# aleju/face-generator

Measured on NVIDIA H100. Metric: 32x32 GAN train images/sec (1 D-iter + 1 G-iter per batch, batch 256/GPU), higher is better.
Workload: dtype f32

## Files before the change

### face_generator_b200/csrc/convl.cu

```cuda
#include "convl.h"

#include "k_conv_tc.h"
#include "k_misc.h"

int convl_dalloc(ConvLEnv& e, float** p, size_t elems) { return fg_dalloc(e.c, *e.allocs, p, elems); }

int ScalePairs::alloc(fg_ctx* c, std::vector<void*>& allocs, int pairs) {
  n = pairs;
  used = 0;
  return fg_dalloc(c, allocs, &base, 2 * (size_t)pairs);
}
int ScalePairs::take(float** pair) {
  if (used == n) {
    fg_set_error("a block of %d FP16 scale pairs is full", n);
    return FG_ERR_UNSUPPORTED;
  }
  *pair = base + 2 * used++;
  return FG_OK;
}
int ScalePairs::reset(fg_ctx* c) const {
  if (!tc_f16(c)) return FG_OK;
  FG_CUDA(cudaMemset2DAsync(base, 2 * sizeof(float), 0, sizeof(float), n, c->stream));
  return FG_OK;
}

namespace {
inline bool tc_f(const fg_ctx* c, const ConvL& L, int B) { return c->conv_impl != FG_CONV_SIMT && tc_conv_eligible(L.geom_k(B)); }
inline bool tc_d(const fg_ctx* c, const ConvL& L, int B) { return c->conv_impl != FG_CONV_SIMT && tc_conv_eligible(L.geom_d(B)); }
inline bool tc_w(const fg_ctx* c, const ConvL& L, int B) { return tc_f(c, L, B) && L.Cout % 128 == 0 && L.geom_k(B).Cin % 64 == 0; }
}

bool convl_tc_fwd(const fg_ctx* c, const ConvL& L) { return tc_f(c, L, 1); }
bool convl_tc_bwd(const fg_ctx* c, const ConvL& L) { return tc_f(c, L, 1) && tc_d(c, L, 1); }

int tc_op_split(fg_ctx* c, TcOp& op, const float* x, int64_t n, bool f16) {
  if (!f16) {
    if (op.split_ready) {
      op.split_ready = false;
      return FG_OK;
    }
    return tc_split(c, x, op.hi, op.lo, n);
  }
  if (op.amax_ready) op.amax_ready = false;
  else FG_TRY(tc_amax(c, x, n, op.s));
  return tc_split_h(c, x, op.hi, op.lo, n, op.s);
}

int convl_alloc(ConvLEnv& e, ConvL& L) {
  const size_t nw = (size_t)L.k * L.k * L.Cout * L.Cin;
  FG_TRY(convl_dalloc(e, &L.Wp, nw));
  FG_TRY(convl_dalloc(e, &L.Wpd, nw));
  if (L.nA) FG_TRY(convl_dalloc(e, &L.bp, L.Cout));
  if (!L.x.s) FG_TRY(convl_dalloc(e, &L.x.s, 2));
  if (!e.dy.s) FG_TRY(convl_dalloc(e, &e.dy.s, 2));
  if (tc_conv_eligible(L.geom_k(e.maxB))) {
    const int K = L.geom_k(e.maxB).Cin;
    const size_t nk = (size_t)L.k * L.k * L.Cout * K, nx = (size_t)e.maxB * L.H * L.H * K;
    FG_TRY(convl_dalloc(e, &L.Wf_hi, nk));
    FG_TRY(convl_dalloc(e, &L.Wf_lo, nk));
    FG_TRY(convl_dalloc(e, &L.x.hi, nx));
    FG_TRY(convl_dalloc(e, &L.x.lo, nx));
    if (L.kpad) {
      FG_TRY(convl_dalloc(e, &L.Wpad, nk));
      FG_TRY(convl_dalloc(e, &L.xpad, nx));
    }
  }
  if (L.need_dgrad && tc_conv_eligible(L.geom_d(e.maxB))) {
    FG_TRY(convl_dalloc(e, &L.Wd_hi, nw));
    FG_TRY(convl_dalloc(e, &L.Wd_lo, nw));
  }
  const int B = e.maxB;
  if (L.pad_out && !(tc_conv_eligible(ConvGeom{B, L.H, L.H, L.Cin, L.pad_out, L.k, 1}) &&
                     tc_conv_eligible(ConvGeom{B, L.H, L.H, L.pad_out, L.Cin, L.k, 1}) && L.Cin % 128 == 0))
    L.pad_out = 0;
  if (L.pad_dy && !(L.x.hi && tc_conv_eligible(ConvGeom{B, L.H, L.H, L.Cin, L.pad_dy, L.k, 1}) && L.Cin % 64 == 0))
    L.pad_dy = 0;
  if (L.pad_out) {
    const size_t nq = (size_t)L.k * L.k * L.pad_out * L.Cin;
    FG_TRY(convl_dalloc(e, &L.Wq_hi, nq));
    FG_TRY(convl_dalloc(e, &L.Wq_lo, nq));
    const size_t nx = (size_t)B * L.H * L.H * L.Cin;
    FG_TRY(convl_dalloc(e, &L.x.hi, nx));
    FG_TRY(convl_dalloc(e, &L.x.lo, nx));
  }
  return FG_OK;
}

int convl_pack(fg_ctx* c, ConvL& L, const float* P) {
  const int KK = L.k * L.k;
  const bool tc_on = c->conv_impl != FG_CONV_SIMT;
  const bool h = tc_on && tc_f16(c) && L.geom_k(1).Cin % 64 == 0 && (L.Cout % 64 == 0 || L.pad_out);
  L.packed_f16 = h;
  if (KK > 1 && tc_on && !L.nA && !L.cA && !L.pad_out && !L.kpad && L.Wf_hi && (L.Wd_hi || !L.need_dgrad) && tc_f(c, L, 1) &&
      (!L.need_dgrad || tc_d(c, L, 1))) {
    if (h) return tc_pack_split_h(c, P + L.w_off, L.Wf_hi, L.Wf_lo, L.Wd_hi, L.Wd_lo, L.Cout, L.Cin, KK);
    return tc_pack_split(c, P + L.w_off, L.Wf_hi, L.Wf_lo, L.Wd_hi, L.Wd_lo, L.Cout, L.Cin, KK);
  }
  FG_TRY(k_pack_weights(c, P + L.w_off, L.Wp, L.need_dgrad ? L.Wpd : nullptr, L.Cout, L.Cin, KK, L.nA, L.nS, L.cA, L.cS));
  if (L.bp) FG_TRY(k_pack_weights(c, P + L.b_off, L.bp, nullptr, L.Cout, 1, 1, L.nA, L.nS, 0, 0));
  if (!tc_on) return FG_OK;
  if (L.kpad && L.Wf_hi) {
    FG_CUDA(cudaMemcpy2DAsync(L.Wpad, L.kpad * sizeof(float), L.Wp, L.Cin * sizeof(float), L.Cin * sizeof(float), L.Cout,
                              cudaMemcpyDeviceToDevice, c->stream));
    if (h) return tc_split_h(c, L.Wpad, L.Wf_hi, L.Wf_lo, (int64_t)L.Cout * L.kpad);
    return tc_split(c, L.Wpad, L.Wf_hi, L.Wf_lo, (int64_t)L.Cout * L.kpad);
  }
  const int64_t nw = (int64_t)KK * L.Cout * L.Cin;
  if (h) {
    if (L.Wf_hi) FG_TRY(tc_split_h(c, L.Wp, L.Wf_hi, L.Wf_lo, nw));
    if (L.Wd_hi) FG_TRY(tc_split_h(c, L.Wpd, L.Wd_hi, L.Wd_lo, nw));
    if (L.pad_out) FG_TRY(k_pack_pad_split_h(c, P + L.w_off, L.Wq_hi, L.Wq_lo, L.Cout, L.pad_out, L.Cin, KK));
    return FG_OK;
  }
  if (L.Wf_hi) FG_TRY(tc_split(c, L.Wp, L.Wf_hi, L.Wf_lo, nw));
  if (L.Wd_hi) FG_TRY(tc_split(c, L.Wpd, L.Wd_hi, L.Wd_lo, nw));
  if (L.pad_out) FG_TRY(k_pack_pad_split(c, P + L.w_off, L.Wq_hi, L.Wq_lo, L.Cout, L.pad_out, L.Cin, KK));
  return FG_OK;
}

int convl_fwd(ConvLEnv& e, ConvL& L, const float* in, const float* P, float* out, int B) {
  fg_ctx* c = e.c;
  const ConvGeom g = L.geom(B);
  const float* bias = L.bp ? L.bp : P + L.b_off;
  const bool h = L.packed_f16;
  const float* os = h ? L.x.s + 1 : nullptr;
  if (L.pad_out && c->conv_impl != FG_CONV_SIMT) {
    FG_TRY(tc_op_split(c, L.x, in, (int64_t)B * L.H * L.H * L.Cin, h));
    {
      ScopedTimer t(c, L.tf);
      FG_TRY(tc_conv_fwd(c, L.x.hi, L.x.lo, L.Wq_hi, L.Wq_lo, nullptr, e.ga, ConvGeom{B, L.H, L.H, L.Cin, L.pad_out, L.k, 1}, 0,
                         nullptr, nullptr, h, os));
    }
    return k_compact_bias(c, e.ga, bias, out, (int64_t)B * L.H * L.H, L.Cout, L.pad_out);
  }
  if (tc_f(c, L, B)) {
    const ConvGeom gk = L.geom_k(B);
    if (L.kpad) {
      FG_CUDA(cudaMemcpy2DAsync(L.xpad, L.kpad * sizeof(float), in, L.Cin * sizeof(float), L.Cin * sizeof(float), (size_t)B * L.H * L.H,
                                cudaMemcpyDeviceToDevice, c->stream));
      in = L.xpad;
    }
    FG_TRY(tc_op_split(c, L.x, in, (int64_t)B * L.H * L.H * gk.Cin, h));
    ScopedTimer t(c, L.tf);
    return tc_conv_fwd(c, L.x.hi, L.x.lo, L.Wf_hi, L.Wf_lo, bias, out, gk, 0, nullptr, nullptr, h, os);
  }
  ScopedTimer t(c, L.tf);
  if (c->edge_impl && k_edge_eligible(g)) return k_conv_edge(c, in, L.Wp, bias, out, g);
  return k_small_eligible(g) ? k_conv_small(c, in, L.Wp, bias, out, g) : k_conv_simt(c, in, L.Wp, bias, out, g);
}

int convl_bwd(ConvLEnv& e, ConvL& L, const float* in, const float* dy, float* G, float* din, int B) {
  fg_ctx* c = e.c;
  const ConvGeom g = L.geom(B), gd = L.geom_d(B);
  const bool w_tc = G && tc_w(c, L, B), d_tc = din && tc_d(c, L, B);
  const bool h = L.packed_f16;
  float* sdy = L.sdy ? L.sdy : e.dy.s;
  const bool split_ready = e.dy.split_ready, amax_ready = e.dy.amax_ready, bias_ready = e.dy.bias_ready;
  e.dy.split_ready = e.dy.amax_ready = e.dy.bias_ready = false;
  const float *osy = h ? sdy + 1 : nullptr, *osx = h ? L.x.s + 1 : nullptr;
  const bool tc_on = c->conv_impl != FG_CONV_SIMT;
  const int64_t P = (int64_t)B * L.H * L.H;
  if (h && !amax_ready && (w_tc || d_tc || (G && tc_on && (L.pad_out || L.pad_dy)))) FG_TRY(tc_amax(c, dy, P * L.Cout, sdy));
  if (w_tc || d_tc) {
    if (h) FG_TRY(tc_split_h(c, dy, e.dy.hi, e.dy.lo, P * L.Cout, sdy));
    else if (!split_ready) FG_TRY(tc_split(c, dy, e.dy.hi, e.dy.lo, P * L.Cout));
  }
  if (G && tc_on && L.pad_out) {
    if (h) FG_TRY(k_pad_split_h(c, dy, e.pad.hi, e.pad.lo, P, L.Cout, L.pad_out, sdy));
    else FG_TRY(k_pad_split(c, dy, e.pad.hi, e.pad.lo, P, L.Cout, L.pad_out));
    {
      ScopedTimer t(c, L.tw);
      FG_TRY(tc_conv_wgrad(c, e.pad.hi, e.pad.lo, L.x.hi, L.x.lo, e.ws, ConvGeom{B, L.H, L.H, L.pad_out, L.Cin, L.k, 1}, h, osy, osx));
    }
    FG_TRY(k_unpack_wgrad_swapped(c, e.ws, G + L.w_off, L.Cout, L.pad_out, L.Cin, L.k * L.k));
    if (!bias_ready) FG_TRY(k_colsum_add(c, dy, G + L.b_off, P, L.Cout, 0, 0));
  } else if (G && tc_on && L.pad_dy && !w_tc) {
    if (h) FG_TRY(k_pad_split_h(c, dy, e.pad.hi, e.pad.lo, P, L.Cout, L.pad_dy, sdy));
    else FG_TRY(k_pad_split(c, dy, e.pad.hi, e.pad.lo, P, L.Cout, L.pad_dy));
    {
      ScopedTimer t(c, L.tw);
      FG_TRY(tc_conv_wgrad(c, L.x.hi, L.x.lo, e.pad.hi, e.pad.lo, e.ws, ConvGeom{B, L.H, L.H, L.Cin, L.pad_dy, L.k, 1}, h, osy, osx));
    }
    FG_TRY(k_unpack_wgrad_pad(c, e.ws, G + L.w_off, L.Cout, L.pad_dy, L.Cin, L.k * L.k));
    if (!bias_ready) FG_TRY(k_colsum_add(c, dy, G + L.b_off, P, L.Cout, 0, 0));
  } else if (G) {
    const int64_t koff = L.kpad && w_tc ? (int64_t)L.Cout * L.Cin : 0;
    {
      ScopedTimer t(c, L.tw);
      if (w_tc) FG_TRY(tc_conv_wgrad(c, L.x.hi, L.x.lo, e.dy.hi, e.dy.lo, e.ws + koff, L.geom_k(B), h, osy, osx));
      else if (k_small_eligible(g)) FG_TRY(k_wgrad_small(c, in, dy, e.ws, g));
      else FG_TRY(k_wgrad_simt(c, in, dy, e.ws, g));
    }
    if (koff)
      FG_CUDA(cudaMemcpy2DAsync(e.ws, L.Cin * sizeof(float), e.ws + koff, L.kpad * sizeof(float), L.Cin * sizeof(float), L.Cout,
                                cudaMemcpyDeviceToDevice, c->stream));
    FG_TRY(k_unpack_wgrad(c, e.ws, G + L.w_off, L.Cout, L.Cin, L.k * L.k, L.nA, L.nS, L.cA, L.cS));
    if (!bias_ready) FG_TRY(k_colsum_add(c, dy, G + L.b_off, P, L.Cout, L.nA, L.nS));
  }
  if (din) {
    ScopedTimer t(c, L.td);
    if (d_tc) return tc_conv_fwd(c, e.dy.hi, e.dy.lo, L.Wd_hi, L.Wd_lo, nullptr, din, gd, 0, nullptr, nullptr, h, osy);
    if (c->edge_impl && k_edge_eligible(gd)) return k_conv_edge(c, dy, L.Wpd, nullptr, din, gd);
    return k_small_eligible(gd) ? k_conv_small(c, dy, L.Wpd, nullptr, din, gd) : k_conv_simt(c, dy, L.Wpd, nullptr, din, gd);
  }
  return FG_OK;
}

bool upsl_tc(const fg_ctx* c, const UpsL& U) {
  return c->conv_impl != FG_CONV_SIMT && tc_conv_eligible(U.geom(1)) && U.Cout % 128 == 0 && U.Cin % 64 == 0;
}

int upsl_alloc(ConvLEnv& e, UpsL& U) {
  const size_t nw25 = (size_t)25 * U.Cout * U.Cin, nw36 = (size_t)36 * U.Cout * U.Cin;
  FG_TRY(convl_dalloc(e, &U.Wp, nw25));
  FG_TRY(convl_dalloc(e, &U.Wpd, nw25));
  FG_TRY(convl_dalloc(e, &U.Wf_hi, nw36));
  FG_TRY(convl_dalloc(e, &U.Wf_lo, nw36));
  FG_TRY(convl_dalloc(e, &U.Wd_hi, nw36));
  FG_TRY(convl_dalloc(e, &U.Wd_lo, nw36));
  FG_TRY(convl_dalloc(e, &U.Wx_hi, nw25));
  FG_TRY(convl_dalloc(e, &U.Wx_lo, nw25));
  const size_t nx = (size_t)e.maxB * (U.H / 2) * (U.H / 2) * U.Cin;
  FG_TRY(convl_dalloc(e, &U.x.hi, nx));
  FG_TRY(convl_dalloc(e, &U.x.lo, nx));
  if (!U.x.s) FG_TRY(convl_dalloc(e, &U.x.s, 2));
  return FG_OK;
}

int upsl_pack(fg_ctx* c, UpsL& U, const float* P) {
  const float* W = P + U.w_off;
  if (!upsl_tc(c, U)) return k_pack_weights(c, W, U.Wp, U.Wpd, U.Cout, U.Cin, 25, 0, 0, 0, 0);
  if (tc_f16(c)) FG_TRY(tc_pack_collapsed_h(c, W, U.Wf_hi, U.Wf_lo, U.Wd_hi, U.Wd_lo, U.Cout, U.Cin));
  else FG_TRY(tc_pack_collapsed(c, W, U.Wf_hi, U.Wf_lo, U.Wd_hi, U.Wd_lo, U.Cout, U.Cin));
  if (c->conv_impl == FG_CONV_TC_DENSE) FG_TRY(tc_pack_split(c, W, U.Wx_hi, U.Wx_lo, nullptr, nullptr, U.Cout, U.Cin, 25));
  return FG_OK;
}

int upsl_fwd(ConvLEnv& e, UpsL& U, const float* h, const float* P, float* z, int B, int* parts) {
  fg_ctx* c = e.c;
  const ConvGeom g = U.geom(B);
  const bool want = parts && *parts;
  if (parts) *parts = 0;
  const float* bias = P + U.b_off;
  if (!upsl_tc(c, U)) {
    ScopedTimer t(c, U.tf);
    return k_conv_simt(c, h, U.Wp, bias, z, g);
  }
  const bool f16 = tc_f16(c);
  FG_TRY(tc_op_split(c, U.x, h, (int64_t)B * (U.H / 2) * (U.H / 2) * U.Cin, f16));
  ScopedTimer t(c, U.tf);
  float* st = want && c->bn_epilogue ? c->bn_parts : nullptr;
  const bool dense = c->conv_impl == FG_CONV_TC_DENSE;
  return tc_conv_fwd(c, U.x.hi, U.x.lo, dense ? U.Wx_hi : U.Wf_hi, dense ? U.Wx_lo : U.Wf_lo, bias, z, g, dense ? 1 : 2, st,
                     st ? parts : nullptr, f16, f16 ? U.x.s + 1 : nullptr);
}

int upsl_bwd(ConvLEnv& e, UpsL& U, TcOp& dy, const float* h, const float* dz, float* G, float* dh, int B, bool* pooled) {
  fg_ctx* c = e.c;
  const ConvGeom g = U.geom(B);
  float* dW = G + U.w_off;
  *pooled = upsl_tc(c, U);
  if (!*pooled) {
    {
      ScopedTimer t(c, U.tw);
      FG_TRY(k_wgrad_simt(c, h, dz, e.ws, g));
    }
    FG_TRY(k_unpack_wgrad(c, e.ws, dW, U.Cout, U.Cin, 25, 0, 0, 0, 0));
    ScopedTimer t(c, U.td);
    return k_conv_simt(c, dz, U.Wpd, nullptr, dh, ConvGeom{B, U.H, U.H, U.Cout, U.Cin, 5, 1});
  }
  const bool f16 = tc_f16(c);
  FG_TRY(tc_op_split(c, dy, dz, (int64_t)B * U.H * U.H * U.Cout, f16));
  const float *sy = f16 ? dy.s + 1 : nullptr, *sx = f16 ? U.x.s + 1 : nullptr;
  if (f16 && U.tb && (c->bwd_merge == 2 ? tc_bwd_pair_eligible(c, g) : c->bwd_merge == 1 && tc_bwd_pair_pays(c, g))) {
    {
      ScopedTimer t(c, U.tb);
      FG_TRY(tc_conv_bwd_ups(c, U.x.hi, U.x.lo, dy.hi, dy.lo, U.Wd_hi, U.Wd_lo, e.ws, dh, g, sy, sx));
    }
    return tc_combine_collapsed_wgrad(c, e.ws, dW, U.Cout, U.Cin);
  }
  {
    ScopedTimer t(c, U.tw);
    FG_TRY(tc_conv_wgrad(c, U.x.hi, U.x.lo, dy.hi, dy.lo, e.ws, g, f16, sy, sx));
  }
  FG_TRY(tc_combine_collapsed_wgrad(c, e.ws, dW, U.Cout, U.Cin));
  ScopedTimer t(c, U.td);
  return tc_conv_dgrad_ups(c, dy.hi, dy.lo, U.Wd_hi, U.Wd_lo, dh, g, f16, sy);
}
```

### face_generator_b200/csrc/convl.h

```cpp
#pragma once
#include <vector>

#include "fg_internal.h"

inline bool tc_f16(const fg_ctx* c) { return c->mma_f16 && c->conv_impl == FG_CONV_TC_COLLAPSED; }

struct AmaxInto {
  fg_ctx* c;
  AmaxInto(fg_ctx* c_, TcOp& op) : AmaxInto(c_, op.s, &op.amax_ready) {}
  AmaxInto(fg_ctx* c_, float* pair, bool* done) : c(c_) {
    if (tc_f16(c)) {
      c->amax_out = reinterpret_cast<unsigned*>(pair);
      c->amax_done = done;
    }
  }
  ~AmaxInto() { c->amax_out = nullptr; }
};

inline unsigned* take_amax(fg_ctx* c) {
  unsigned* p = c->amax_out;
  if (p) *c->amax_done = true;
  return p;
}

int tc_op_split(fg_ctx* c, TcOp& op, const float* x, int64_t n, bool f16);

inline int pack_key(const fg_ctx* c) { return c->conv_impl | (c->mma_f16 << 4); }
int convl_dalloc(ConvLEnv& e, float** p, size_t elems);
int convl_alloc(ConvLEnv& e, ConvL& L);
bool convl_tc_fwd(const fg_ctx* c, const ConvL& L);
bool convl_tc_bwd(const fg_ctx* c, const ConvL& L);
int convl_pack(fg_ctx* c, ConvL& L, const float* P);
int convl_fwd(ConvLEnv& e, ConvL& L, const float* in, const float* P, float* out, int B);
int convl_bwd(ConvLEnv& e, ConvL& L, const float* in, const float* dy, float* G, float* din, int B);

bool upsl_tc(const fg_ctx* c, const UpsL& U);
int upsl_alloc(ConvLEnv& e, UpsL& U);
int upsl_pack(fg_ctx* c, UpsL& U, const float* P);
int upsl_fwd(ConvLEnv& e, UpsL& U, const float* h, const float* P, float* z, int B, int* parts = nullptr);
int upsl_bwd(ConvLEnv& e, UpsL& U, TcOp& dy, const float* h, const float* dz, float* G, float* dh, int B, bool* pooled);

int gen_alloc(ConvLEnv& e, UpsGen& G, const GenDesc& d);
int gen_pack(fg_ctx* c, UpsGen& G, NetPair& p);
int gen_forward(ConvLEnv& e, UpsGen& G, NetPair& p, const float* noise, int B, bool training);
int gen_backward(ConvLEnv& e, UpsGen& G, NetPair& p, const float* dy, float* dnoise);
void gen_debug_rows(const UpsGen& G, std::vector<DebugTensor>& rows);
```

### face_generator_b200/csrc/fg_internal.h

```cpp
#pragma once
#include <cuda_runtime.h>
#include <cstdint>
#include <cstdio>
#include <deque>
#include <functional>
#include <initializer_list>
#include <map>
#include <string>
#include <vector>

#include "fg_b200.h"

void fg_set_error(const char* fmt, ...);

#define FG_CUDA(call)                                                                               \
  do {                                                                                              \
    cudaError_t e__ = (call);                                                                       \
    if (e__ != cudaSuccess) {                                                                       \
      fg_set_error("%s:%d: %s -> %s", __FILE__, __LINE__, #call, cudaGetErrorString(e__));          \
      return FG_ERR_CUDA;                                                                           \
    }                                                                                               \
  } while (0)
#define FG_TRY(call)                  \
  do {                                \
    int r__ = (call);                 \
    if (r__ != FG_OK) return r__;     \
  } while (0)
#define FG_REQUIRE(cond, ...)         \
  do {                                \
    if (!(cond)) {                    \
      fg_set_error(__VA_ARGS__);      \
      return FG_ERR_INVALID;          \
    }                                 \
  } while (0)
#define LAUNCH_CHECK(c)                 \
  do {                                  \
    (c)->launches++;                    \
    FG_CUDA(cudaGetLastError());        \
  } while (0)
inline int grid_for(int64_t n, int block, int cap = 132 * 16) {
  int64_t g = (n + block - 1) / block;
  if (g > cap) g = cap;
  if (g < 1) g = 1;
  return (int)g;
}
#define GRID_STRIDE(i, n) \
  for (int64_t i = blockIdx.x * (int64_t)blockDim.x + threadIdx.x; i < (n); i += (int64_t)gridDim.x * blockDim.x)

constexpr int kMaskPerSample = 1984;
constexpr int kNoiseDim = 100;
constexpr int kSmallMaxParts = 2048;
constexpr int kGradTail = 8;
constexpr int kOptRedRows = 132 * 2;

struct ConvGeom {
  int B, H, W, Cin, Cout, k, ups;
};

struct GLayout {
  int64_t L1W, L1b, a1, C1W, C1b, g1, be1, a2, C2W, C2b, g2, be2, a3, C3W, C3b, total;
};
GLayout make_g_layout(int C, int side);

struct DeviceStats {
  float loss_D, loss_G;
  int conf[4];
  int trained_D;
  int t_D, t_G;
  float acc_D;
  int acc_count, acc_head;
  float step_D, step_G;
  int do_train_D, do_train_G;
};
constexpr int kAccHistMax = 1024;
constexpr int kMaxIters = 16;
constexpr int kBnState = 768;

struct StepGraph {
  std::vector<uint8_t> key;
  cudaGraphExec_t exec = nullptr;
  int64_t launches = 0;
  bool failed = false;
};

struct NetPair {
  int64_t nG = 0, nD = 0;
  float *PG = nullptr, *PD = nullptr, *gG = nullptr, *gD = nullptr;
  float *tailG = nullptr, *tailD = nullptr;
  float *mG = nullptr, *vG = nullptr, *mD = nullptr, *vD = nullptr;
  float* bnG = nullptr;
  DeviceStats* dstats = nullptr;
  DeviceStats* hstats = nullptr;
  float* acc_hist = nullptr;
  int G_pack = -1, D_pack = -1;
  std::vector<StepGraph> graphs;
  const char* optim_timer[2] = {nullptr, nullptr};
  struct Keep {
    const char* name;
    const float* src;
    int64_t per;
    float* copy = nullptr;
  };
  std::vector<Keep> keep;
  int keep_B = 0;
};

struct ScalePairs {
  float* base = nullptr;
  int n = 0, used = 0;
  int alloc(fg_ctx* c, std::vector<void*>& allocs, int pairs);
  int take(float** pair);
  int reset(fg_ctx* c) const;
};

struct TcOp {
  float *hi = nullptr, *lo = nullptr;
  float* s = nullptr;
  bool split_ready = false, amax_ready = false, bias_ready = false;
};
struct ConvL {
  int Cin = 0, Cout = 0, k = 1, H = 1;
  int64_t w_off = 0, b_off = 0;
  int cA = 0, cS = 0;
  int nA = 0, nS = 0;
  float *Wp = nullptr, *Wpd = nullptr;
  float* bp = nullptr;
  float *Wf_hi = nullptr, *Wf_lo = nullptr, *Wd_hi = nullptr, *Wd_lo = nullptr;
  TcOp x;
  float* sdy = nullptr;
  int kpad = 0;
  float *xpad = nullptr, *Wpad = nullptr;
  bool packed_f16 = false;
  int pad_out = 0, pad_dy = 0;
  float *Wq_hi = nullptr, *Wq_lo = nullptr;
  bool need_dgrad = true;
  const char *tf = "", *td = "", *tw = "";
  ConvGeom geom(int B) const { return ConvGeom{B, H, H, Cin, Cout, k, 1}; }
  ConvGeom geom_k(int B) const { return ConvGeom{B, H, H, kpad ? kpad : Cin, Cout, k, 1}; }
  ConvGeom geom_d(int B) const { return ConvGeom{B, H, H, Cout, Cin, k, 1}; }
};

struct UpsL {
  int Cin = 0, Cout = 0, H = 0;
  int64_t w_off = 0, b_off = 0;
  float *Wp = nullptr, *Wpd = nullptr;
  float *Wf_hi = nullptr, *Wf_lo = nullptr, *Wd_hi = nullptr, *Wd_lo = nullptr;
  float *Wx_hi = nullptr, *Wx_lo = nullptr;
  TcOp x;
  const char *tf = "", *td = "", *tw = "", *tb = nullptr;
  ConvGeom geom(int B) const { return ConvGeom{B, H, H, Cin, Cout, 5, 2}; }
};

struct ConvLEnv {
  fg_ctx* c = nullptr;
  int maxB = 0;
  std::vector<void*>* allocs = nullptr;
  float *ga = nullptr;
  TcOp dy;
  TcOp pad;
  float* ws = nullptr;
};

struct GenDesc {
  int side;
  const char* prefix;
  int l1_kpad;
  bool bwd_merge;
};

struct UpsGen {
  int S = 32, C = 3;
  GLayout gl;
  ConvL GL1, GC3;
  UpsL GU[2];
  ScalePairs pairs;
  float* sdz[2] = {nullptr, nullptr};
  float *noise = nullptr, *z0 = nullptr, *h0 = nullptr, *z1 = nullptr, *h1 = nullptr, *z2 = nullptr, *h2 = nullptr,
        *z3 = nullptr, *y = nullptr;
  float *dz3 = nullptr, *dfull = nullptr, *dz2 = nullptr, *dz1 = nullptr, *dz0 = nullptr;
  float *bn_mean[2] = {nullptr, nullptr}, *bn_istd[2] = {nullptr, nullptr}, *bn_mg = nullptr;
  int B = 0;
  bool train = true, valid = false;
  std::deque<std::string> names;
  const char *t_bn2_finalize = nullptr, *t_bn2_stats = nullptr, *t_bn2_apply = nullptr, *t_bn2_bwd_reduce = nullptr,
             *t_bn2_bwd_apply = nullptr;
};

struct TimerRec {
  double ms = 0;
  int64_t launches = 0;
  std::vector<std::pair<cudaEvent_t, cudaEvent_t>> pending;
};

struct IterStage {
  float* p[8] = {};
  size_t cap[8] = {};
  int reserve(fg_ctx* c, std::vector<void*>& allocs, int k, size_t n);
  int in(fg_ctx* c, std::vector<void*>& allocs, int k, const float* p, size_t n, size_t cap_n, const float** out);
};

struct Net32;

struct fg_ctx {
  int device = 0, maxB = 0, C = 3;
  cudaStream_t stream = nullptr;
  bool own_stream = true;
  int64_t launches = 0;
  int conv_impl = FG_CONV_TC_COLLAPSED;
  int sm_count = 132;
  int opt_D = 0, opt_G = 0;
  float sgd_mom_D = 0.f, sgd_mom_G = 0.f;
  std::vector<void*> allocs;
  Net32* n32 = nullptr;
  float* small_ws = nullptr;
  float* splitk_ws = nullptr;
  size_t splitk_ws_elems = 0;
  double* red_ws = nullptr;
  size_t red_ws_elems = 0;
  double* red_ws_opt = nullptr;
  unsigned* red_ticket = nullptr;
  double* bn_slice_acc = nullptr;
  float* bn_parts = nullptr;
  int edge_impl = 1;
  int bn_epilogue = 1;
  int mma_f16 = 1;
  float* lop_sx = nullptr;
  float* lop_sy = nullptr;
  unsigned* amax_out = nullptr;
  bool* amax_done = nullptr;
  double* bn_acc = nullptr;
  float* io_dev = nullptr;
  size_t io_dev_elems = 0;
  float* scratch[8] = {nullptr, nullptr, nullptr, nullptr, nullptr, nullptr, nullptr, nullptr};
  size_t scratch_elems[8] = {0, 0, 0, 0, 0, 0, 0, 0};
  void* nccl_comm = nullptr;
  int world = 1, rank = 0;
  int dp_overlap = 1;
  int reserve_sms = 0;
  int last_conv_kind = 0, last_conv_tile_m = 0, last_conv_tile_n = 0, last_conv_format = 0, last_conv_splits = 0;
  int bwd_merge = 1, bwd_merge_ctas = 0;
  int* bwd_claim = nullptr;
  int use_graph = 1, graph_epoch = 0;
  uint64_t* seed_dev = nullptr;
  cudaStream_t comm_stream = nullptr;
  cudaEvent_t ev_fork = nullptr, ev_join = nullptr;
  bool debug_keep = false;
  cudaEvent_t events[16] = {};
  bool timing = false;
  std::map<std::string, TimerRec> timers;
};

inline void note_conv(fg_ctx* c, int kind, int tile_m, int tile_n, int format, int splits) {
  c->last_conv_kind = kind;
  c->last_conv_tile_m = tile_m;
  c->last_conv_tile_n = tile_n;
  c->last_conv_format = format;
  c->last_conv_splits = splits;
}

struct ScopedTimer {
  fg_ctx* c;
  TimerRec* rec = nullptr;
  cudaEvent_t e0 = nullptr, e1 = nullptr;
  ScopedTimer(fg_ctx* c_, const char* name) : c(c_) {
    if (c->timing && name) {
      rec = &c->timers[name];
      cudaEventCreate(&e0);
      cudaEventCreate(&e1);
      cudaEventRecord(e0, c->stream);
    }
  }
  ~ScopedTimer() {
    if (rec) {
      cudaEventRecord(e1, c->stream);
      rec->pending.emplace_back(e0, e1);
    }
  }
};

int k_fill(fg_ctx* c, float* p, float v, int64_t n);
int k_nchw_to_nhwc(fg_ctx* c, const float* src, float* dst, int B, int C, int HW);
int k_nhwc_to_nchw(fg_ctx* c, const float* src, float* dst, int B, int C, int HW);
int k_pack_weights(fg_ctx* c, const float* W, float* Wp, float* Wpd, int N, int Cc, int KK, int nA, int nS, int cA,
                   int cS);
int k_unpack_wgrad(fg_ctx* c, const float* dWp, float* dW, int N, int Cc, int KK, int nA, int nS, int cA, int cS);
int k_colsum_add(fg_ctx* c, const float* X, float* out, int64_t P, int N, int nA, int nS);
int k_prelu_fwd(fg_ctx* c, const float* z, const float* slope, float* h, int64_t n);
int k_prelu_bwd(fg_ctx* c, const float* dh, const float* z, const float* slope, float* dz, float* dslope, int B, int H,
                int W, int C, int pool);
int k_bn_stats(fg_ctx* c, const float* z, double* acc2C, int64_t P, int C);
bool k_bn4_ok(int C);
int k_bn_stats4(fg_ctx* c, const float* z, double* acc, int64_t P, int C);
int k_bn_bwd_reduce4(fg_ctx* c, const float* dh, const float* z, const float* mean, const float* istd, const float* gamma,
                     const float* beta, const float* slope, double* acc, float* dslope, int64_t P, int C);
int k_bn_finalize(fg_ctx* c, double* acc2C, float* mean, float* istd, float* run_mean, float* run_var, int64_t P,
                  int C);
int k_bn_finalize_parts(fg_ctx* c, const float* part, int nparts, int nphase, float* mean, float* istd, float* run_mean,
                        float* run_var, int64_t P, int C);
int k_bn_eval_prep(fg_ctx* c, const float* run_mean, const float* run_var, float* mean, float* istd, int C);
int k_bn_prelu_apply(fg_ctx* c, const float* z, const float* mean, const float* istd, const float* gamma,
                     const float* beta, const float* slope, float* h, int64_t P, int C, float* hi = nullptr,
                     float* lo = nullptr);
int k_bn_prelu_bwd_reduce(fg_ctx* c, const float* dh, const float* z, const float* mean, const float* istd,
                          const float* gamma, const float* beta, const float* slope, double* acc2C, float* dslope,
                          int B, int H, int W, int C, int pool);
int k_bn_bwd_finalize(fg_ctx* c, double* acc2C, float* mg2C, float* dgamma, float* dbeta, int64_t P, int C);
int k_bn_prelu_bwd_apply(fg_ctx* c, const float* dh, const float* z, const float* mean, const float* istd,
                         const float* gamma, const float* beta, const float* slope, const float* mg2C, float* dz,
                         int B, int H, int W, int C, int pool, float* hi = nullptr, float* lo = nullptr,
                         float* dbias = nullptr);
int k_sigmoid_fwd(fg_ctx* c, const float* z, float* y, int64_t n);
int k_sigmoid_bwd(fg_ctx* c, const float* dy, const float* y, float* dz, int64_t n);
int k_masks_generate(fg_ctx* c, float* masks, int B, uint64_t seed, float p_spatial, float p_drop,
                     const uint64_t* seed_dev = nullptr);
int k_set_u64(fg_ctx* c, uint64_t* dst, uint64_t v);
int k_seed_roots(fg_ctx* c, uint64_t* roots, int n);
int k_d_act_pool_fwd(fg_ctx* c, const float* z, const float* slope, const float* masks, int moff, float eval_scale,
                     float* p, int B, int H, int W, int C, float* hi = nullptr, float* lo = nullptr);
int k_d_act_pool_bwd(fg_ctx* c, const float* dp, const float* z, const float* slope, const float* masks, int moff,
                     float eval_scale, float* dz, float* dslope, int B, int H, int W, int C, float* hi = nullptr,
                     float* lo = nullptr, float* dbias = nullptr);
int k_lin_act_drop_fwd(fg_ctx* c, const float* z, const float* slope, const float* masks, int moff, float scale,
                       float* h, int B, int N);
int k_lin_act_drop_bwd(fg_ctx* c, const float* dh, const float* z, const float* slope, const float* masks, int moff,
                       float scale, float* dz, float* dslope, int B, int N);
int k_sigmoid_bce(fg_ctx* c, const float* logit, float* out, float* dlogit, float* loss_out, float* tail4, int B,
                  int n_ones);
int k_bce_fwd(fg_ctx* c, const float* x, const float* t, int n, float* loss_out);
int k_bce_bwd(fg_ctx* c, const float* x, const float* t, int n, float* dx);
int k_sigmoid_grad_mul(fg_ctx* c, const float* dout, const float* out, float* dlogit, int n);
int k_penalty_loss(fg_ctx* c, const float* p, int64_t n, float l1, float l2, float* loss_inout);
int k_gate_and_prep(fg_ctx* c, DeviceStats* st, float* acc_hist, int net, const fg_hyper* h, const float* tail4, int B,
                    float world, bool accumulate = false);
int k_optim_prep(fg_ctx* c, DeviceStats* st, int net, const fg_hyper* h);
int k_gemv_fwd(fg_ctx* c, const float* x, const float* w, const float* bias, float* out, int B, int K);
int k_gemv_dgrad(fg_ctx* c, const float* dy, const float* w, float* dx, int B, int K);
int k_gemv_wgrad_add(fg_ctx* c, const float* x, const float* dy, float* dw, float* db, int B, int K);
int k_adam(fg_ctx* c, float* p, const float* g, float* m, float* v, int64_t n, float beta1, float beta2, float eps,
           float l1_grad, float l2, float clampv, float grad_scale, const float* step_dev, const int* flag_dev,
           float step_host, float* g_out);
int k_optim_update(fg_ctx* c, int mode, float* p, float* g, float* m, float* v, int64_t n, float beta1, float beta2, float eps,
                   float mom, float l1_grad, float l2, float clampv, float grad_scale, const float* step_dev,
                   const int* flag_dev, const int* t_dev);

int k_conv_simt(fg_ctx* c, const float* in, const float* Wp, const float* bias, float* out, ConvGeom g);
int k_wgrad_simt(fg_ctx* c, const float* in, const float* dY, float* dWp, ConvGeom g);
bool k_small_eligible(const ConvGeom& g);
int k_conv_small(fg_ctx* c, const float* in, const float* Wp, const float* bias, float* out, ConvGeom g);
int k_wgrad_small(fg_ctx* c, const float* in, const float* dY, float* dWp, ConvGeom g);

bool k_edge_eligible(const ConvGeom& g);
int k_conv_edge(fg_ctx* c, const float* in, const float* Wp, const float* bias, float* out, ConvGeom g);

inline int red_check(fg_ctx* c, int64_t rows, int64_t n) {
  if (rows * n > (int64_t)c->red_ws_elems) {
    fg_set_error("ordered reduction of %lld x %lld partials exceeds its workspace", (long long)rows, (long long)n);
    return FG_ERR_UNSUPPORTED;
  }
  return FG_OK;
}
int k_splitk_reduce(fg_ctx* c, const float* parts, int splits, int64_t n, float* out);

int tc_init(fg_ctx* c);
void tc_destroy(fg_ctx* c);

int net32_alloc(fg_ctx* c);
void net32_free(fg_ctx* c);
NetPair& net32_pair(fg_ctx* c);

int net_allreduce(fg_ctx* c, float* buf, int64_t n);
int net_broadcast(fg_ctx* c, void* buf, size_t bytes);
int net_group(bool start);

int fg_dalloc(fg_ctx* c, std::vector<void*>& allocs, float** p, size_t n);
int pair_alloc(fg_ctx* c, std::vector<void*>& allocs, NetPair& p, int64_t nG, int64_t nD, bool bn);
void pair_clear_graphs(NetPair& p);
void pair_free(NetPair& p);
int pair_zero_grads(fg_ctx* c, NetPair& p, int net);
int pair_allreduce_grads(fg_ctx* c, NetPair& p, int net);
int pair_gate(fg_ctx* c, NetPair& p, int net, const fg_hyper* h, int B, float world, bool accumulate = false);
int pair_optim(fg_ctx* c, NetPair& p, int net, const fg_hyper* h, float grad_scale);
int k_adam_prep(fg_ctx* c, int* t_dev, float* step_dev, float lr, float beta1, float beta2);
int pair_broadcast(fg_ctx* c, NetPair& p);
int pair_step_stats(fg_ctx* c, const NetPair& p, fg_step_stats* stats);
int pair_set_params(fg_ctx* c, NetPair& p, int net, const float* src);
int pair_get_params(fg_ctx* c, const NetPair& p, int net, float* dst);
int pair_get_grads(fg_ctx* c, const NetPair& p, int net, float* dst);
int pair_set_adam_state(fg_ctx* c, NetPair& p, int net, const float* m, const float* v, int t);
int pair_get_adam_state(fg_ctx* c, const NetPair& p, int net, float* m, float* v, int* t);
int pair_set_bn_state(fg_ctx* c, NetPair& p, const float* src);
int pair_get_bn_state(fg_ctx* c, const NetPair& p, float* dst);
int net_graph_run(fg_ctx* c, NetPair& p, int B, const void* hyper, size_t hyper_bytes, std::initializer_list<const void*> inputs,
                  uint64_t seed, const std::function<int()>& body, int nd = 1, int ng = 1);

int step_check(fg_ctx* c, const char* what, int B, int nd, int ng, bool inputs, const fg_dataset* d = nullptr, bool fed = false);
struct StepNets {
  StepNets(fg_ctx* c, NetPair& pair, const fg_hyper* h, int B, float* logit, float* out, float* dlogit, float* masks,
           int64_t mask, bool gate, bool overlap)
      : c(c), pair(&pair), h(h), B(B), logit(logit), out(out), dlogit(dlogit), masks(masks), mask(mask), gate(gate),
        overlap(overlap) {}
  fg_ctx* c;
  NetPair* pair;
  const fg_hyper* h;
  int B;
  float *logit, *out, *dlogit;
  float* masks;
  int64_t mask;
  bool gate;
  bool overlap;
  virtual int g_forward(int j, bool d_iter) = 0;
  virtual int d_input(int j) = 0;
  virtual int draw_masks(int kind, const uint64_t* root) = 0;
  virtual int d_forward(bool on_g) = 0;
  virtual int d_backward(bool want_wgrad, bool want_dx) = 0;
  virtual int g_backward() = 0;
};
int pair_train_step(StepNets& s, int nd, int ng, const float* masksD, const float* masksG, uint64_t seed,
                    std::initializer_list<const void*> inputs, const std::function<int()>* feed, fg_step_stats* stats);
struct DebugTensor;
void pair_keep_rows(const NetPair& p, std::vector<DebugTensor>& ents);

int k_relu_fwd(fg_ctx* c, const float* z, float* h, int64_t n);
int k_relu_bwd(fg_ctx* c, const float* dh, const float* z, float* dz, int64_t n);
int k_tanh_dropout_fwd(fg_ctx* c, const float* z, const float* masks_in, const uint64_t* seed_dev, float p, float* code, float* h,
                       float* flags_out, int64_t n);
int k_tanh_dropout_bwd(fg_ctx* c, const float* dh, const float* masks, float p, const float* code, float* dz, int64_t n);
int k_abs_criterion(fg_ctx* c, bool sigmoid, const float* z, const float* t, float* y, float* dz, int64_t n, float* loss);

bool fg_is_dev(const void* p);
int fg_to_dev(fg_ctx* c, const float* p, size_t n, float* staging, const float** out);
int fg_to_user(fg_ctx* c, float* dst, const float* src_dev, size_t n);
struct DebugTensor {
  const char* name;
  const float* p;
  int64_t per;
  int B;
};
int64_t debug_tensor_copy(fg_ctx* c, const char* what, const DebugTensor* ents, size_t n_ents, const char* name, float* dst,
                          int64_t max_elems);

struct JpegScratch;
void jpeg_scratch_free(JpegScratch* s);
struct JpegEncScratch;
void jpeg_enc_scratch_free(JpegEncScratch* s);
struct fg_dataset {
  fg_ctx* c = nullptr;
  int64_t N = 0;
  int Cs = 3, Hs = 64, Ws = 64;
  uint8_t* data = nullptr;
  int32_t* idx = nullptr;
  JpegScratch* jpeg = nullptr;
  JpegEncScratch* jpeg_enc = nullptr;
};
int dataset_check_feed(const fg_dataset* d, const fg_ctx* c, const char* what);
int dataset_draw_gather(fg_dataset* d, uint64_t seed, int B, int size, float* out_dev, const uint64_t* root = nullptr,
                        uint64_t kinds = 0);
int dataset_draw_gather_c2f(fg_dataset* d, uint64_t seed, int B, int fine_size, int coarse_size, float* fine, float* coarse,
                            float* diff, const uint64_t* root = nullptr, uint64_t kinds = 0);
int noise_uniform_dev(fg_ctx* c, uint64_t seed, int64_t n, float* out_dev, const uint64_t* root = nullptr, uint64_t kinds = 0);
```

### face_generator_b200/csrc/gen.cu

```cuda
#include "convl.h"

GLayout make_g_layout(int C, int side) {
  const int64_t n0 = 128 * (side / 4) * (side / 4);
  GLayout L;
  int64_t o = 0;
  L.L1W = o; o += n0 * kNoiseDim;
  L.L1b = o; o += n0;
  L.a1 = o; o += 1;
  L.C1W = o; o += 256 * 128 * 25;
  L.C1b = o; o += 256;
  L.g1 = o; o += 256;
  L.be1 = o; o += 256;
  L.a2 = o; o += 1;
  L.C2W = o; o += 128 * 256 * 25;
  L.C2b = o; o += 128;
  L.g2 = o; o += 128;
  L.be2 = o; o += 128;
  L.a3 = o; o += 1;
  L.C3W = o; o += (int64_t)C * 128 * 9;
  L.C3b = o; o += C;
  L.total = o;
  return L;
}

int gen_alloc(ConvLEnv& e, UpsGen& G, const GenDesc& d) {
  fg_ctx* c = e.c;
  const int S = d.side, C = c->C;
  G.S = S;
  G.C = C;
  G.gl = make_g_layout(C, S);
  const GLayout& gl = G.gl;
  auto timer = [&](const char* name) {
    G.names.push_back(std::string(d.prefix) + name);
    return G.names.back().c_str();
  };
  FG_TRY(G.pairs.alloc(c, *e.allocs, 8));
  ConvL& L1 = G.GL1;
  L1.Cin = kNoiseDim; L1.Cout = 128 * (S / 4) * (S / 4); L1.k = 1; L1.H = 1;
  L1.w_off = gl.L1W; L1.b_off = gl.L1b;
  L1.nA = 128; L1.nS = (S / 4) * (S / 4);
  L1.kpad = d.l1_kpad;
  L1.tf = timer("G.L1.fwd"); L1.td = timer("G.L1.dgrad"); L1.tw = timer("G.L1.wgrad");
  ConvL& C3 = G.GC3;
  C3.Cin = 128; C3.Cout = C; C3.k = 3; C3.H = S;
  C3.w_off = gl.C3W; C3.b_off = gl.C3b;
  C3.tf = timer("G.C3.fwd"); C3.td = timer("G.C3.dgrad"); C3.tw = timer("G.C3.wgrad");
  for (ConvL* L : {&L1, &C3}) {
    FG_TRY(G.pairs.take(&L->x.s));
    FG_TRY(G.pairs.take(&L->sdy));
    FG_TRY(convl_alloc(e, *L));
  }
  static const char* uf[2] = {"G.C1.fwd", "G.C2.fwd"};
  static const char* ud[2] = {"G.C1.dgrad", "G.C2.dgrad"};
  static const char* uw[2] = {"G.C1.wgrad", "G.C2.wgrad"};
  static const char* ub[2] = {"G.C1.wgrad+dgrad", "G.C2.wgrad+dgrad"};
  const int ci[2] = {128, 256}, co[2] = {256, 128}, hs[2] = {S / 2, S};
  const int64_t wo[2] = {gl.C1W, gl.C2W}, bo[2] = {gl.C1b, gl.C2b};
  for (int i = 0; i < 2; ++i) {
    UpsL& U = G.GU[i];
    U.Cin = ci[i]; U.Cout = co[i]; U.H = hs[i];
    U.w_off = wo[i]; U.b_off = bo[i];
    U.tf = timer(uf[i]); U.td = timer(ud[i]); U.tw = timer(uw[i]);
    U.tb = d.bwd_merge ? timer(ub[i]) : nullptr;
    FG_TRY(G.pairs.take(&U.x.s));
    FG_TRY(G.pairs.take(&G.sdz[i]));
    FG_TRY(upsl_alloc(e, U));
  }
  G.t_bn2_finalize = timer("G.bn2.finalize");
  G.t_bn2_stats = timer("hbm.G.bn2.stats");
  G.t_bn2_apply = timer("hbm.G.bn2.apply");
  G.t_bn2_bwd_reduce = timer("hbm.G.bn2.bwd_reduce");
  G.t_bn2_bwd_apply = timer("hbm.G.bn2.bwd_apply");
  const size_t B = e.maxB, n0 = L1.Cout, n1 = (size_t)256 * (S / 2) * (S / 2), n2 = (size_t)128 * S * S, n3 = (size_t)C * S * S;
  for (auto [p, n] : {std::pair<float**, size_t>{&G.noise, kNoiseDim}, {&G.z0, n0}, {&G.h0, n0}, {&G.z1, n1}, {&G.h1, n1},
                      {&G.z2, n2}, {&G.h2, n2}, {&G.z3, n3}, {&G.y, n3}, {&G.dz3, n3},
                      {&G.dfull, (size_t)256 * S * S},
                      {&G.dz2, n2}, {&G.dz1, n1}, {&G.dz0, n0}})
    FG_TRY(convl_dalloc(e, p, B * n));
  for (int i = 0; i < 2; ++i) {
    FG_TRY(convl_dalloc(e, &G.bn_mean[i], co[i]));
    FG_TRY(convl_dalloc(e, &G.bn_istd[i], co[i]));
  }
  return convl_dalloc(e, &G.bn_mg, 512);
}

int gen_pack(fg_ctx* c, UpsGen& G, NetPair& p) {
  if (p.G_pack == pack_key(c)) return FG_OK;
  FG_TRY(convl_pack(c, G.GL1, p.PG));
  for (int i = 0; i < 2; ++i) FG_TRY(upsl_pack(c, G.GU[i], p.PG));
  FG_TRY(convl_pack(c, G.GC3, p.PG));
  p.G_pack = pack_key(c);
  return FG_OK;
}

namespace {
int bn_stats(fg_ctx* c, UpsGen& G, NetPair& p, int i, const float* z, int B, bool training, int parts, const char* t_finalize,
             const char* t_stats) {
  const int Cc = G.GU[i].Cout;
  const int64_t P = (int64_t)B * G.GU[i].H * G.GU[i].H;
  float *rm = p.bnG + (i == 0 ? 0 : 512), *rv = rm + Cc;
  if (!training) return k_bn_eval_prep(c, rm, rv, G.bn_mean[i], G.bn_istd[i], Cc);
  if (parts) {
    ScopedTimer tm(c, t_finalize);
    return k_bn_finalize_parts(c, c->bn_parts, parts, 4, G.bn_mean[i], G.bn_istd[i], rm, rv, P, Cc);
  }
  {
    ScopedTimer tm(c, t_stats);
    FG_TRY(k_bn_stats(c, z, c->bn_acc, P, Cc));
  }
  return k_bn_finalize(c, c->bn_acc, G.bn_mean[i], G.bn_istd[i], rm, rv, P, Cc);
}
}

int gen_forward(ConvLEnv& e, UpsGen& G, NetPair& p, const float* noise, int B, bool training) {
  fg_ctx* c = e.c;
  FG_REQUIRE(B >= 1 && B <= e.maxB, "G forward: batch %d out of range [1,%d]", B, e.maxB);
  FG_TRY(gen_pack(c, G, p));
  const GLayout& L = G.gl;
  const float* P = p.PG;
  const int S = G.S;
  if (noise != G.noise)
    FG_CUDA(cudaMemcpyAsync(G.noise, noise, sizeof(float) * B * kNoiseDim, cudaMemcpyDeviceToDevice, c->stream));
  G.B = B;
  G.train = training;
  FG_TRY(G.pairs.reset(c));
  FG_TRY(convl_fwd(e, G.GL1, G.noise, P, G.z0, B));
  {
    AmaxInto am(c, G.GU[0].x);
    FG_TRY(k_prelu_fwd(c, G.z0, P + L.a1, G.h0, (int64_t)B * G.GL1.Cout));
  }
  int parts = training ? 1 : 0;
  FG_TRY(upsl_fwd(e, G.GU[0], G.h0, P, G.z1, B, &parts));
  FG_TRY(bn_stats(c, G, p, 0, G.z1, B, training, parts, nullptr, nullptr));
  UpsL& C2 = G.GU[1];
  C2.x.split_ready = training && upsl_tc(c, C2) && !tc_f16(c);
  {
    AmaxInto am(c, C2.x);
    FG_TRY(k_bn_prelu_apply(c, G.z1, G.bn_mean[0], G.bn_istd[0], P + L.g1, P + L.be1, P + L.a2, G.h1,
                            (int64_t)B * (S / 2) * (S / 2), 256, C2.x.split_ready ? C2.x.hi : nullptr,
                            C2.x.split_ready ? C2.x.lo : nullptr));
  }
  parts = training ? 1 : 0;
  FG_TRY(upsl_fwd(e, C2, G.h1, P, G.z2, B, &parts));
  FG_TRY(bn_stats(c, G, p, 1, G.z2, B, training, parts, G.t_bn2_finalize, G.t_bn2_stats));
  {
    ScopedTimer tm(c, G.t_bn2_apply);
    FG_TRY(k_bn_prelu_apply(c, G.z2, G.bn_mean[1], G.bn_istd[1], P + L.g2, P + L.be2, P + L.a3, G.h2, (int64_t)B * S * S, 128));
  }
  FG_TRY(convl_fwd(e, G.GC3, G.h2, P, G.z3, B));
  FG_TRY(k_sigmoid_fwd(c, G.z3, G.y, (int64_t)B * S * S * G.C));
  G.valid = true;
  return FG_OK;
}

int gen_backward(ConvLEnv& e, UpsGen& G, NetPair& p, const float* dy, float* dnoise) {
  fg_ctx* c = e.c;
  if (!G.valid || !G.train) {
    fg_set_error("G backward needs a preceding training-mode G forward");
    return FG_ERR_STATE;
  }
  const GLayout& L = G.gl;
  const float* P = p.PG;
  float* g = p.gG;
  const int B = G.B, S = G.S, h = S / 2;
  FG_TRY(G.pairs.reset(c));
  FG_TRY(k_sigmoid_bwd(c, dy, G.y, G.dz3, (int64_t)B * S * S * G.C));
  FG_TRY(convl_bwd(e, G.GC3, G.h2, G.dz3, g, G.dfull, B));
  {
    ScopedTimer tm(c, G.t_bn2_bwd_reduce);
    FG_TRY(k_bn_prelu_bwd_reduce(c, G.dfull, G.z2, G.bn_mean[1], G.bn_istd[1], P + L.g2, P + L.be2, P + L.a3, c->bn_acc,
                                 g + L.a3, B, S, S, 128, 0));
  }
  FG_TRY(k_bn_bwd_finalize(c, c->bn_acc, G.bn_mg, g + L.g2, g + L.be2, (int64_t)B * S * S, 128));
  const bool tf32 = !tc_f16(c);
  TcOp dz2{e.dy.hi, e.dy.lo, G.sdz[1]};
  dz2.split_ready = upsl_tc(c, G.GU[1]) && tf32;
  {
    ScopedTimer tm(c, G.t_bn2_bwd_apply);
    AmaxInto am(c, dz2);
    FG_TRY(k_bn_prelu_bwd_apply(c, G.dfull, G.z2, G.bn_mean[1], G.bn_istd[1], P + L.g2, P + L.be2, P + L.a3, G.bn_mg, G.dz2,
                                B, S, S, 128, 0, dz2.split_ready ? dz2.hi : nullptr, dz2.split_ready ? dz2.lo : nullptr,
                                g + L.C2b));
  }
  bool pooled = false;
  FG_TRY(upsl_bwd(e, G.GU[1], dz2, G.h1, G.dz2, g, G.dfull, B, &pooled));
  FG_TRY(k_bn_prelu_bwd_reduce(c, G.dfull, G.z1, G.bn_mean[0], G.bn_istd[0], P + L.g1, P + L.be1, P + L.a2, c->bn_acc,
                               g + L.a2, B, h, h, 256, pooled ? 0 : 1));
  FG_TRY(k_bn_bwd_finalize(c, c->bn_acc, G.bn_mg, g + L.g1, g + L.be1, (int64_t)B * h * h, 256));
  TcOp dz1{e.dy.hi, e.dy.lo, G.sdz[0]};
  dz1.split_ready = upsl_tc(c, G.GU[0]) && tf32 && pooled;
  {
    AmaxInto am(c, dz1);
    FG_TRY(k_bn_prelu_bwd_apply(c, G.dfull, G.z1, G.bn_mean[0], G.bn_istd[0], P + L.g1, P + L.be1, P + L.a2, G.bn_mg, G.dz1,
                                B, h, h, 256, pooled ? 0 : 1, dz1.split_ready ? dz1.hi : nullptr,
                                dz1.split_ready ? dz1.lo : nullptr, g + L.C1b));
  }
  FG_TRY(upsl_bwd(e, G.GU[0], dz1, G.h0, G.dz1, g, G.dfull, B, &pooled));
  {
    AmaxInto am(c, G.GL1.sdy, &e.dy.amax_ready);
    FG_TRY(k_prelu_bwd(c, G.dfull, G.z0, P + L.a1, G.dz0, g + L.a1, B, S / 4, S / 4, 128, pooled ? 0 : 1));
  }
  return convl_bwd(e, G.GL1, G.noise, G.dz0, g, dnoise, B);
}

void gen_debug_rows(const UpsGen& G, std::vector<DebugTensor>& rows) {
  const int64_t n0 = G.GL1.Cout, n1 = 256 * (G.S / 2) * (G.S / 2), n2 = 128 * G.S * G.S, n3 = (int64_t)G.C * G.S * G.S;
  const int B = G.B;
  for (const DebugTensor& r : {DebugTensor{"G.z0", G.z0, n0, B}, {"G.h0", G.h0, n0, B}, {"G.z1", G.z1, n1, B},
                               {"G.h1", G.h1, n1, B}, {"G.z2", G.z2, n2, B}, {"G.h2", G.h2, n2, B}, {"G.z3", G.z3, n3, B},
                               {"G.y", G.y, n3, B}, {"G.dz2", G.dz2, n2, B}, {"G.dz1", G.dz1, n1, B}, {"G.dz0", G.dz0, n0, B},
                               {"G.bn_mean1", G.bn_mean[0], 256, 1}, {"G.bn_istd1", G.bn_istd[0], 256, 1},
                               {"G.bn_mean2", G.bn_mean[1], 128, 1}, {"G.bn_istd2", G.bn_istd[1], 128, 1}})
    rows.push_back({r.name, G.valid ? r.p : nullptr, r.per, r.B});
}
```

### face_generator_b200/csrc/k_conv_edge.cu

```cuda
#include <cuda.h>

#include <algorithm>

#include "fg_internal.h"
#include "k_conv_tc.h"

namespace {
constexpr int kW = 32;

__device__ __forceinline__ uint32_t smem_u32(const void* p) { return (uint32_t)__cvta_generic_to_shared(p); }
__device__ __forceinline__ void mbar_init(uint64_t* bar, uint32_t count) {
  asm volatile("mbarrier.init.shared::cta.b64 [%0], %1;" ::"r"(smem_u32(bar)), "r"(count));
}
__device__ __forceinline__ void mbar_expect_tx(uint64_t* bar, uint32_t bytes) {
  asm volatile("mbarrier.arrive.expect_tx.shared::cta.b64 _, [%0], %1;" ::"r"(smem_u32(bar)), "r"(bytes) : "memory");
}
__device__ __forceinline__ void mbar_wait(uint64_t* bar, uint32_t parity) {
  const uint32_t addr = smem_u32(bar);
  uint32_t ok;
  do {
    asm volatile(
        "{\n\t.reg .pred p;\n\t"
        "mbarrier.try_wait.parity.shared::cta.b64 p, [%1], %2;\n\t"
        "selp.b32 %0, 1, 0, p;\n\t}"
        : "=r"(ok)
        : "r"(addr), "r"(parity)
        : "memory");
  } while (!ok);
}
__device__ __forceinline__ float4 lds128(uint32_t addr) {
  float4 v;
  asm volatile("ld.shared.v4.f32 {%0, %1, %2, %3}, [%4];" : "=f"(v.x), "=f"(v.y), "=f"(v.z), "=f"(v.w) : "r"(addr));
  return v;
}
__device__ __forceinline__ float2 lds64(uint32_t addr) {
  float2 v;
  asm volatile("ld.shared.v2.f32 {%0, %1}, [%2];" : "=f"(v.x), "=f"(v.y) : "r"(addr));
  return v;
}
__device__ __forceinline__ void tma_load_4d(void* dst, const CUtensorMap* map, uint64_t* bar, int c0, int c1, int c2, int c3) {
  asm volatile(
      "cp.async.bulk.tensor.4d.shared::cluster.global.mbarrier::complete_tx::bytes [%0], [%1, {%3, %4, %5, %6}], [%2];"
      ::"r"(smem_u32(dst)), "l"(map), "r"(smem_u32(bar)), "r"(c0), "r"(c1), "r"(c2), "r"(c3)
      : "memory");
}

constexpr int kRedRows = 4;
template <int VEC>
constexpr uint32_t red_tile_bytes() { return (kRedRows + 2) * (kW + 2) * 32 * VEC * 4; }

template <int NS, int VEC>
__global__ void __launch_bounds__(256, 1) conv_reduce_kernel(const __grid_constant__ CUtensorMap tmap, const float* __restrict__ Wp,
                                                             const float* __restrict__ bias, float* __restrict__ out, int H,
                                                             int nunits) {
  constexpr int C = 32 * VEC;
  constexpr int PX = NS == 1 ? 16 : 4;
  constexpr uint32_t kTile = red_tile_bytes<VEC>();
  extern __shared__ uint8_t smem_raw[];
  uint8_t* smem = reinterpret_cast<uint8_t*>((reinterpret_cast<uintptr_t>(smem_raw) + 127) & ~(uintptr_t)127);
  uint64_t* full = reinterpret_cast<uint64_t*>(smem + 2 * kTile);
  const int warp = threadIdx.x >> 5, lane = threadIdx.x & 31;
  const int strips = H / kRedRows;
  if (threadIdx.x == 0) {
    mbar_init(full + 0, 1);
    mbar_init(full + 1, 1);
    asm volatile("fence.mbarrier_init.release.cluster;" ::: "memory");
  }
  __syncthreads();
  auto issue = [&](int unit, int buf) {
    const int b = unit / strips, y0 = (unit - b * strips) * kRedRows;
    asm volatile("fence.proxy.async.shared::cta;" ::: "memory");
    mbar_expect_tx(full + buf, kTile);
    tma_load_4d(smem + buf * kTile, &tmap, full + buf, 0, -1, y0 - 1, b);
  };
  if (threadIdx.x == 0 && (int)blockIdx.x < nunits) issue(blockIdx.x, 0);
  float w[9][NS][VEC];
#pragma unroll
  for (int t = 0; t < 9; ++t)
#pragma unroll
    for (int n = 0; n < NS; ++n)
#pragma unroll
      for (int j = 0; j < VEC; ++j) w[t][n][j] = Wp[(t * NS + n) * C + lane * VEC + j];
  float bv = 0.f;
  if (bias && (lane & 15) < PX * NS) bv = bias[(lane & 15) % NS];
  const int row = warp >> 1, xh = (warp & 1) * 16;
  int it = 0;
  for (int unit = blockIdx.x; unit < nunits; unit += gridDim.x, ++it) {
    const int buf = it & 1;
    if (threadIdx.x == 0 && unit + (int)gridDim.x < nunits) issue(unit + gridDim.x, buf ^ 1);
    mbar_wait(full + buf, (it >> 1) & 1);
    const uint32_t tile = smem_u32(smem + buf * kTile) + (uint32_t)lane * VEC * 4;
    const int b = unit / strips, y = (unit - b * strips) * kRedRows + row;
#pragma unroll 1
    for (int g = 0; g < 16 / PX; ++g) {
      const int x0 = xh + g * PX;
      float acc[PX][NS];
#pragma unroll
      for (int i = 0; i < PX; ++i)
#pragma unroll
        for (int n = 0; n < NS; ++n) acc[i][n] = 0.f;
#pragma unroll
      for (int j = 0; j < PX + 2; ++j) {
        float v[3][VEC];
#pragma unroll
        for (int dy = 0; dy < 3; ++dy) {
          const uint32_t ad = tile + (uint32_t)(((row + dy) * (kW + 2) + x0 + j) * C) * 4;
          if (VEC == 4) {
            const float4 q = lds128(ad);
            v[dy][0] = q.x; v[dy][1 % VEC] = q.y; v[dy][2 % VEC] = q.z; v[dy][3 % VEC] = q.w;
          } else {
            const float2 q = lds64(ad);
            v[dy][0] = q.x; v[dy][1 % VEC] = q.y;
          }
        }
#pragma unroll
        for (int dy = 0; dy < 3; ++dy)
#pragma unroll
          for (int k = 0; k < VEC; ++k)
#pragma unroll
            for (int dx = 0; dx < 3; ++dx) {
              const int i = j - dx;
              if (i < 0 || i >= PX) continue;
#pragma unroll
              for (int n = 0; n < NS; ++n) acc[i][n] = fmaf(v[dy][k], w[dy * 3 + dx][n][k], acc[i][n]);
            }
      }
      float r[16];
#pragma unroll
      for (int k = 0; k < 16; ++k) r[k] = k < PX * NS ? acc[k / NS][k % NS] : 0.f;
#pragma unroll
      for (int sft = 8; sft >= 1; sft >>= 1) {
        const bool up = (lane & sft) != 0;
#pragma unroll
        for (int k = 0; k < sft; ++k) {
          const float send = up ? r[k] : r[k + sft], keep = up ? r[k + sft] : r[k];
          r[k] = keep + __shfl_xor_sync(0xffffffffu, send, sft);
        }
      }
      const float tot = r[0] + __shfl_xor_sync(0xffffffffu, r[0], 16);
      if (lane < PX * NS) out[((size_t)(b * H + y) * kW + x0) * NS + lane] = tot + bv;
    }
    __syncthreads();
  }
}

constexpr int kExpRows = 8;
template <int CS, int N>
__global__ void __launch_bounds__(256, 1) conv_expand_kernel(const float* __restrict__ in, const float* __restrict__ Wp,
                                                             const float* __restrict__ bias, float* __restrict__ out, int H,
                                                             int nunits) {
  constexpr int RW = (kW + 2) * 4;
  constexpr int ROWF = kW * CS;
  constexpr int NPF = ((kExpRows + 2) * ROWF + 255) / 256;
  __shared__ __align__(16) float tile[2][(kExpRows + 2) * RW];
  const int warp = threadIdx.x >> 5, lane = threadIdx.x & 31;
  const int strips = H / kExpRows;
  for (int i = threadIdx.x; i < 2 * (kExpRows + 2) * RW; i += 256) (&tile[0][0])[i] = 0.f;
  const int n4 = (N == 128 ? lane : (lane & 15)) * 4;
  float w[9][CS][4];
#pragma unroll
  for (int t = 0; t < 9; ++t)
#pragma unroll
    for (int c = 0; c < CS; ++c)
#pragma unroll
      for (int j = 0; j < 4; ++j) w[t][c][j] = Wp[((size_t)t * N + n4 + j) * CS + c];
  float4 b4 = make_float4(0.f, 0.f, 0.f, 0.f);
  if (bias) b4 = make_float4(bias[n4], bias[n4 + 1], bias[n4 + 2], bias[n4 + 3]);
  float pf[NPF];
  auto prefetch = [&](int unit) {
    const int b = unit / strips, y0 = (unit - b * strips) * kExpRows;
#pragma unroll
    for (int i = 0; i < NPF; ++i) {
      const int idx = threadIdx.x + 256 * i;
      const int r = idx / ROWF, off = idx - r * ROWF, gy = y0 - 1 + r;
      pf[i] = (r < kExpRows + 2 && gy >= 0 && gy < H) ? in[((size_t)(b * H + gy) * kW) * CS + off] : 0.f;
    }
  };
  auto stash = [&](int buf) {
#pragma unroll
    for (int i = 0; i < NPF; ++i) {
      const int idx = threadIdx.x + 256 * i;
      const int r = idx / ROWF, off = idx - r * ROWF;
      if (r < kExpRows + 2) tile[buf][r * RW + (off / CS + 1) * 4 + off % CS] = pf[i];
    }
  };
  __syncthreads();
  if ((int)blockIdx.x < nunits) {
    prefetch(blockIdx.x);
    stash(0);
  }
  __syncthreads();
  constexpr int STEP = N == 128 ? 2 : 4;
  const int xoff = N == 128 ? 0 : 2 * (lane >> 4);
  int it = 0;
  for (int unit = blockIdx.x; unit < nunits; unit += gridDim.x, ++it) {
    const int buf = it & 1;
    const bool more = unit + (int)gridDim.x < nunits;
    if (more) prefetch(unit + gridDim.x);
    const int b = unit / strips, y = (unit - b * strips) * kExpRows + warp;
    const float4* t0 = reinterpret_cast<const float4*>(&tile[buf][warp * RW]);
    float* orow = out + ((size_t)(b * H + y) * kW) * N + n4;
#pragma unroll 1
    for (int xb = 0; xb < kW; xb += STEP) {
      const int x = xb + xoff;
      float4 a0 = b4, a1 = b4;
#pragma unroll
      for (int dy = 0; dy < 3; ++dy) {
        float4 col[4];
#pragma unroll
        for (int j = 0; j < 4; ++j) col[j] = t0[dy * (kW + 2) + x + j];
#pragma unroll
        for (int dx = 0; dx < 3; ++dx)
#pragma unroll
          for (int c = 0; c < CS; ++c) {
            const float v0 = c == 0 ? col[dx].x : (c == 1 ? col[dx].y : (c == 2 ? col[dx].z : col[dx].w));
            const float v1 = c == 0 ? col[dx + 1].x : (c == 1 ? col[dx + 1].y : (c == 2 ? col[dx + 1].z : col[dx + 1].w));
            const float* wp = w[dy * 3 + dx][c];
            a0.x = fmaf(v0, wp[0], a0.x); a1.x = fmaf(v1, wp[0], a1.x);
            a0.y = fmaf(v0, wp[1], a0.y); a1.y = fmaf(v1, wp[1], a1.y);
            a0.z = fmaf(v0, wp[2], a0.z); a1.z = fmaf(v1, wp[2], a1.z);
            a0.w = fmaf(v0, wp[3], a0.w); a1.w = fmaf(v1, wp[3], a1.w);
          }
      }
      *reinterpret_cast<float4*>(orow + (size_t)x * N) = a0;
      *reinterpret_cast<float4*>(orow + (size_t)(x + 1) * N) = a1;
    }
    if (more) stash(buf ^ 1);
    __syncthreads();
  }
}

template <int NS, int VEC>
int launch_reduce(fg_ctx* c, const float* in, const float* Wp, const float* bias, float* out, const ConvGeom& g) {
  CUtensorMap tmap;
  FG_TRY(tc_encode_nhwc_box(&tmap, in, 32 * VEC, g.W, g.H, g.B, 32 * VEC, kW + 2, kRedRows + 2, 1));
  const int nunits = g.B * (g.H / kRedRows);
  const size_t smem = 2 * (size_t)red_tile_bytes<VEC>() + 64 + 128;
  static bool attr_done = false;
  if (!attr_done) {
    FG_CUDA(cudaFuncSetAttribute(conv_reduce_kernel<NS, VEC>, cudaFuncAttributeMaxDynamicSharedMemorySize, (int)smem));
    attr_done = true;
  }
  note_conv(c, FG_KERNEL_EDGE_REDUCE, NS, VEC, 0, 1);
  conv_reduce_kernel<NS, VEC><<<std::min(nunits, c->sm_count), 256, smem, c->stream>>>(tmap, Wp, bias, out, g.H, nunits);
  LAUNCH_CHECK(c);
  return FG_OK;
}
template <int CS, int N>
int launch_expand(fg_ctx* c, const float* in, const float* Wp, const float* bias, float* out, const ConvGeom& g) {
  const int nunits = g.B * (g.H / kExpRows);
  note_conv(c, FG_KERNEL_EDGE_EXPAND, CS, N, 0, 1);
  conv_expand_kernel<CS, N><<<std::min(nunits, c->sm_count), 256, 0, c->stream>>>(in, Wp, bias, out, g.H, nunits);
  LAUNCH_CHECK(c);
  return FG_OK;
}
}

bool k_edge_eligible(const ConvGeom& g) {
  if (!(g.ups == 1 && g.k == 3 && g.W == kW && g.H % 8 == 0 && g.H >= 8)) return false;
  const bool reduce = (g.Cout == 1 || g.Cout == 3) && (g.Cin == 64 || g.Cin == 128);
  const bool expand = (g.Cin == 1 || g.Cin == 3 || g.Cin == 4) && (g.Cout == 64 || g.Cout == 128);
  return reduce || expand;
}

int k_conv_edge(fg_ctx* c, const float* in, const float* Wp, const float* bias, float* out, ConvGeom g) {
  if (g.Cout <= 3) {
    if (g.Cout == 3 && g.Cin == 128) return launch_reduce<3, 4>(c, in, Wp, bias, out, g);
    if (g.Cout == 3 && g.Cin == 64) return launch_reduce<3, 2>(c, in, Wp, bias, out, g);
    if (g.Cout == 1 && g.Cin == 128) return launch_reduce<1, 4>(c, in, Wp, bias, out, g);
    if (g.Cout == 1 && g.Cin == 64) return launch_reduce<1, 2>(c, in, Wp, bias, out, g);
  } else {
#define EXP(CS_)                                                                 \
  if (g.Cin == CS_) {                                                            \
    if (g.Cout == 128) return launch_expand<CS_, 128>(c, in, Wp, bias, out, g); \
    if (g.Cout == 64) return launch_expand<CS_, 64>(c, in, Wp, bias, out, g);   \
  }
    EXP(1) EXP(3) EXP(4)
#undef EXP
  }
  fg_set_error("k_conv_edge: unsupported shape %d -> %d", g.Cin, g.Cout);
  return FG_ERR_UNSUPPORTED;
}
```

### face_generator_b200/csrc/k_conv_small.cu

```cuda
#include "fg_internal.h"

namespace {
constexpr int kMaxSmallW = 36 * 128;

template <int NS, int VEC>
__global__ void __launch_bounds__(256) conv_smalln_kernel(const float* __restrict__ in, const float* __restrict__ Wp,
                                                          const float* __restrict__ bias, float* __restrict__ out, int B,
                                                          int H, int W) {
  constexpr int C = 32 * VEC;
  __shared__ __align__(16) float ws[9 * NS * C];
  for (int i = threadIdx.x; i < 9 * NS * C; i += blockDim.x) ws[i] = Wp[i];
  __syncthreads();
  constexpr int RL = 8;
  const int lane = threadIdx.x & 31;
  const uint32_t runs_per_row = (uint32_t)W / RL;
  const uint32_t nruns = (uint32_t)B * H * runs_per_row;
  const uint32_t warps = (gridDim.x * blockDim.x) >> 5;
  for (uint32_t run = (blockIdx.x * blockDim.x + threadIdx.x) >> 5; run < nruns; run += warps) {
    const int x0 = (int)(run % runs_per_row) * RL;
    const uint32_t row = run / runs_per_row;
    const int y = (int)(row % (uint32_t)H);
    const float* rowbase = in + (size_t)row * W * C + lane * VEC;
    float col[3][3][VEC];
    auto load_col = [&](int slot, int xx) {
#pragma unroll
      for (int dy = 0; dy < 3; ++dy) {
        const bool ok = (unsigned)(y + dy - 1) < (unsigned)H && (unsigned)xx < (unsigned)W;
        const float* ip = rowbase + ((dy - 1) * W + xx) * C;
        if (VEC == 4) {
          const float4 q = ok ? *reinterpret_cast<const float4*>(ip) : make_float4(0.f, 0.f, 0.f, 0.f);
          col[slot][dy][0] = q.x; col[slot][dy][1 % VEC] = q.y; col[slot][dy][2 % VEC] = q.z; col[slot][dy][3 % VEC] = q.w;
        } else if (VEC == 2) {
          const float2 q = ok ? *reinterpret_cast<const float2*>(ip) : make_float2(0.f, 0.f);
          col[slot][dy][0] = q.x; col[slot][dy][1 % VEC] = q.y;
        } else {
          col[slot][dy][0] = ok ? ip[0] : 0.f;
        }
      }
    };
    load_col(0, x0 - 1);
    load_col(1, x0);
#pragma unroll
    for (int i = 0; i < RL; ++i) {
      load_col((i + 2) % 3, x0 + i + 1);
      float acc[NS];
#pragma unroll
      for (int n = 0; n < NS; ++n) acc[n] = 0.f;
#pragma unroll
      for (int dy = 0; dy < 3; ++dy)
#pragma unroll
        for (int dx = 0; dx < 3; ++dx) {
          const int t = dy * 3 + dx, slot = (i + dx) % 3;
#pragma unroll
          for (int n = 0; n < NS; ++n) {
            const float* wp = ws + (t * NS + n) * C + lane * VEC;
#pragma unroll
            for (int j = 0; j < VEC; ++j) acc[n] = fmaf(col[slot][dy][j], wp[j], acc[n]);
          }
        }
#pragma unroll
      for (int n = 0; n < NS; ++n) {
#pragma unroll
        for (int o = 16; o > 0; o >>= 1) acc[n] += __shfl_xor_sync(0xffffffffu, acc[n], o);
      }
      if (lane == 0) {
        float* op = out + ((size_t)row * W + x0 + i) * NS;
#pragma unroll
        for (int n = 0; n < NS; ++n) op[n] = acc[n] + (bias ? bias[n] : 0.f);
      }
    }
  }
}

template <int CS>
__global__ void __launch_bounds__(256) conv_smallk4_kernel(const float* __restrict__ in, const float* __restrict__ Wp,
                                                           const float* __restrict__ bias, float* __restrict__ out, int B,
                                                           int H, int W, int N) {
  __shared__ __align__(16) float ws[9 * CS * 128];
  for (int i = threadIdx.x; i < 9 * CS * N; i += blockDim.x) {
    const int n = i % N, c = (i / N) % CS, t = i / (N * CS);
    ws[i] = Wp[((size_t)t * N + n) * CS + c];
  }
  __syncthreads();
  const uint32_t N4 = (uint32_t)N >> 2;
  const uint32_t total = (uint32_t)B * H * W * N4;
  for (uint32_t i = blockIdx.x * blockDim.x + threadIdx.x; i < total; i += gridDim.x * blockDim.x) {
    const uint32_t n4 = i % N4, p = i / N4;
    const int x = (int)(p % (uint32_t)W), y = (int)((p / (uint32_t)W) % (uint32_t)H);
    float4 acc = bias ? make_float4(bias[n4 * 4], bias[n4 * 4 + 1], bias[n4 * 4 + 2], bias[n4 * 4 + 3])
                      : make_float4(0.f, 0.f, 0.f, 0.f);
    const float* base = in + (size_t)p * CS;
#pragma unroll
    for (int t = 0; t < 9; ++t) {
      const int dy = t / 3 - 1, dx = t % 3 - 1;
      if ((unsigned)(y + dy) >= (unsigned)H || (unsigned)(x + dx) >= (unsigned)W) continue;
      const float* ip = base + (dy * W + dx) * CS;
#pragma unroll
      for (int c = 0; c < CS; ++c) {
        const float v = __ldg(ip + c);
        const float4 w = *reinterpret_cast<const float4*>(ws + (t * CS + c) * N + n4 * 4);
        acc.x = fmaf(v, w.x, acc.x);
        acc.y = fmaf(v, w.y, acc.y);
        acc.z = fmaf(v, w.z, acc.z);
        acc.w = fmaf(v, w.w, acc.w);
      }
    }
    *reinterpret_cast<float4*>(out + (size_t)i * 4) = acc;
  }
}

template <int CS, int XS>
__global__ void __launch_bounds__(128) wgrad_smallbig_kernel(const float* __restrict__ big, const float* __restrict__ small,
                                                             float* __restrict__ part, int B, int H, int W, int Cb,
                                                             int rows_per_block) {
  __shared__ float4 sm[3][68];
  const int lanes = 128 / Cb;
  const int cb = threadIdx.x % Cb, pl = threadIdx.x / Cb;
  const int x_begin = pl * XS;
  float acc[9][CS];
#pragma unroll
  for (int t = 0; t < 9; ++t)
#pragma unroll
    for (int c = 0; c < CS; ++c) acc[t][c] = 0.f;
  const int BH = B * H;
  const int r0 = blockIdx.x * rows_per_block, r1 = min(BH, r0 + rows_per_block);
  for (int r = r0; r < r1; ++r) {
    const int b = r / H, y = r - b * H;
    __syncthreads();
    for (int i = threadIdx.x; i < 3 * (W + 2); i += 128) {
      const int rr = i / (W + 2), cc = i - rr * (W + 2);
      const int yy = y + rr - 1, xx = cc - 1;
      float4 v = make_float4(0.f, 0.f, 0.f, 0.f);
      if (yy >= 0 && yy < H && xx >= 0 && xx < W) {
        const float* sp = small + (((size_t)b * H + yy) * W + xx) * CS;
        v.x = sp[0];
        if (CS > 1) v.y = sp[1 % CS];
        if (CS > 2) v.z = sp[2 % CS];
        if (CS > 3) v.w = sp[3 % CS];
      }
      sm[rr][cc] = v;
    }
    __syncthreads();
    const float* bp = big + ((size_t)r * W + x_begin) * Cb + cb;
    float bv[XS];
#pragma unroll
    for (int i = 0; i < XS; ++i) bv[i] = bp[(size_t)i * Cb];
    float4 w0[3], w1[3], w2[3];
#pragma unroll
    for (int rr = 0; rr < 3; ++rr) {
      w0[rr] = sm[rr][x_begin];
      w1[rr] = sm[rr][x_begin + 1];
    }
#pragma unroll
    for (int i = 0; i < XS; ++i) {
#pragma unroll
      for (int rr = 0; rr < 3; ++rr) {
        w2[rr] = sm[rr][x_begin + i + 2];
        const float4 q[3] = {w0[rr], w1[rr], w2[rr]};
#pragma unroll
        for (int cc = 0; cc < 3; ++cc) {
          acc[rr * 3 + cc][0] = fmaf(bv[i], q[cc].x, acc[rr * 3 + cc][0]);
          if (CS > 1) acc[rr * 3 + cc][1 % CS] = fmaf(bv[i], q[cc].y, acc[rr * 3 + cc][1 % CS]);
          if (CS > 2) acc[rr * 3 + cc][2 % CS] = fmaf(bv[i], q[cc].z, acc[rr * 3 + cc][2 % CS]);
          if (CS > 3) acc[rr * 3 + cc][3 % CS] = fmaf(bv[i], q[cc].w, acc[rr * 3 + cc][3 % CS]);
        }
        w0[rr] = w1[rr];
        w1[rr] = w2[rr];
      }
    }
  }
  float* dst = part + ((size_t)blockIdx.x * lanes + pl) * (9 * CS * Cb);
#pragma unroll
  for (int t = 0; t < 9; ++t)
#pragma unroll
    for (int c = 0; c < CS; ++c) dst[(t * CS + c) * Cb + cb] = acc[t][c];
}
__global__ void wgrad_small_reduce_kernel(const float* __restrict__ part, float* __restrict__ out, int nparts, int CS, int Cb,
                                          int sign, int transposed) {
  const int total = 9 * CS * Cb;
  const int j = blockIdx.x * blockDim.x + threadIdx.x;
  if (j >= total) return;
  const int per = (nparts + gridDim.y - 1) / gridDim.y;
  const int i0 = blockIdx.y * per, i1 = min(nparts, i0 + per);
  float s0 = 0.f, s1 = 0.f, s2 = 0.f, s3 = 0.f;
  int i = i0;
  for (; i + 3 < i1; i += 4) {
    s0 += part[(size_t)i * total + j];
    s1 += part[(size_t)(i + 1) * total + j];
    s2 += part[(size_t)(i + 2) * total + j];
    s3 += part[(size_t)(i + 3) * total + j];
  }
  for (; i < i1; ++i) s0 += part[(size_t)i * total + j];
  const int idx = j / (CS * Cb), cs = (j / Cb) % CS, cb = j % Cb;
  const int t = sign > 0 ? idx : 8 - idx;
  out[(size_t)blockIdx.y * total + (transposed ? ((size_t)t * Cb + cb) * CS + cs : ((size_t)t * CS + cs) * Cb + cb)] =
      (s0 + s1) + (s2 + s3);
}
}

bool k_small_eligible(const ConvGeom& g) {
  const int cs = g.Cin < g.Cout ? g.Cin : g.Cout, cb = g.Cin < g.Cout ? g.Cout : g.Cin;
  if (!(g.ups == 1 && g.k == 3 && cs >= 1 && cs <= 4 && (cb == 32 || cb == 64 || cb == 128))) return false;
  const int xs = g.W / (128 / cb);
  return g.W <= 64 && g.W % (128 / cb) == 0 && (xs == 8 || xs == 16 || xs == 32) &&
         (int64_t)g.B * g.H * g.W * cb < ((int64_t)1 << 31);
}

int k_conv_small(fg_ctx* c, const float* in, const float* Wp, const float* bias, float* out, ConvGeom g) {
  const int64_t P = (int64_t)g.B * g.H * g.W;
  if (g.Cin <= 4) {
    const int64_t total = P * (g.Cout / 4);
    int grid = (int)std::min<int64_t>((total + 255) / 256, c->sm_count * 16);
    switch (g.Cin) {
      case 1: conv_smallk4_kernel<1><<<grid, 256, 0, c->stream>>>(in, Wp, bias, out, g.B, g.H, g.W, g.Cout); break;
      case 2: conv_smallk4_kernel<2><<<grid, 256, 0, c->stream>>>(in, Wp, bias, out, g.B, g.H, g.W, g.Cout); break;
      case 3: conv_smallk4_kernel<3><<<grid, 256, 0, c->stream>>>(in, Wp, bias, out, g.B, g.H, g.W, g.Cout); break;
      default: conv_smallk4_kernel<4><<<grid, 256, 0, c->stream>>>(in, Wp, bias, out, g.B, g.H, g.W, g.Cout); break;
    }
    LAUNCH_CHECK(c);
    return FG_OK;
  }
  if (g.Cout > 4 || 9 * g.Cout * g.Cin > kMaxSmallW) {
    fg_set_error("k_conv_small: expects Cout <= 4");
    return FG_ERR_UNSUPPORTED;
  }
  if (g.W % 8) {
    fg_set_error("k_conv_small: W must be a multiple of 8");
    return FG_ERR_UNSUPPORTED;
  }
  int grid = (int)std::min<int64_t>((P / 8 * 32 + 255) / 256, c->sm_count * 8);
#define SN(NS_, VEC_) conv_smalln_kernel<NS_, VEC_><<<grid, 256, 0, c->stream>>>(in, Wp, bias, out, g.B, g.H, g.W)
  const int vec = g.Cin / 32;
  if (vec == 4) {
    if (g.Cout == 1) SN(1, 4); else if (g.Cout == 2) SN(2, 4); else if (g.Cout == 3) SN(3, 4); else SN(4, 4);
  } else if (vec == 2) {
    if (g.Cout == 1) SN(1, 2); else if (g.Cout == 2) SN(2, 2); else if (g.Cout == 3) SN(3, 2); else SN(4, 2);
  } else {
    if (g.Cout == 1) SN(1, 1); else if (g.Cout == 2) SN(2, 1); else if (g.Cout == 3) SN(3, 1); else SN(4, 1);
  }
#undef SN
  LAUNCH_CHECK(c);
  return FG_OK;
}

int k_wgrad_small(fg_ctx* c, const float* in, const float* dY, float* dWp, ConvGeom g) {
  const bool small_out = g.Cout <= 4;
  const float* big = small_out ? in : dY;
  const float* small = small_out ? dY : in;
  const int Cb = small_out ? g.Cin : g.Cout, Cs = small_out ? g.Cout : g.Cin;
  const int lanes = 128 / Cb, xs = g.W / lanes;
  const int BH = g.B * g.H;
  int rpb = 8;
  int nblocks = (BH + rpb - 1) / rpb;
  while (nblocks * lanes > kSmallMaxParts) {
    rpb *= 2;
    nblocks = (BH + rpb - 1) / rpb;
  }
  const int sign = small_out ? -1 : 1, transposed = small_out ? 0 : 1;
#define WG(CS_, XS_) \
  wgrad_smallbig_kernel<CS_, XS_><<<nblocks, 128, 0, c->stream>>>(big, small, c->small_ws, g.B, g.H, g.W, Cb, rpb)
#define WGX(CS_)                 \
  do {                           \
    if (xs == 8) WG(CS_, 8);     \
    else if (xs == 16) WG(CS_, 16); \
    else WG(CS_, 32);            \
  } while (0)
  switch (Cs) {
    case 1: WGX(1); break;
    case 2: WGX(2); break;
    case 3: WGX(3); break;
    default: WGX(4); break;
  }
#undef WGX
#undef WG
  LAUNCH_CHECK(c);
  const int total = 9 * Cs * Cb;
  constexpr int kSlices = 32;
  wgrad_small_reduce_kernel<<<dim3((total + 127) / 128, kSlices), 128, 0, c->stream>>>(c->small_ws, c->splitk_ws, nblocks * lanes,
                                                                                     Cs, Cb, sign, transposed);
  LAUNCH_CHECK(c);
  return k_splitk_reduce(c, c->splitk_ws, kSlices, total, dWp);
}
```

### face_generator_b200/csrc/k_elem.cu

```cuda
#include <cmath>

#include "convl.h"
#include "fg_internal.h"
#include "k_f16split.cuh"
#include "k_ordered.cuh"

__device__ __forceinline__ int perm_idx(int j, int A, int S) {
  if (A == 0) return j;
  return (j % S) * A + (j / S);
}

__device__ __forceinline__ double warp_sum(double v) {
#pragma unroll
  for (int o = 16; o > 0; o >>= 1) v += __shfl_xor_sync(0xffffffffu, v, o);
  return v;
}
__device__ __forceinline__ double block_sum(double v) {
  __shared__ double red[32];
  __syncthreads();
  v = warp_sum(v);
  if ((threadIdx.x & 31) == 0) red[threadIdx.x >> 5] = v;
  __syncthreads();
  if (threadIdx.x < 32) {
    v = threadIdx.x < (blockDim.x + 31) / 32 ? red[threadIdx.x] : 0.0;
    v = warp_sum(v);
  }
  return v;
}

__global__ void fill_kernel(float* p, float v, int64_t n) {
  for (int64_t i = blockIdx.x * (int64_t)blockDim.x + threadIdx.x; i < n; i += (int64_t)gridDim.x * blockDim.x) p[i] = v;
}
int k_fill(fg_ctx* c, float* p, float v, int64_t n) {
  if (n <= 0) return FG_OK;
  fill_kernel<<<grid_for(n, 256), 256, 0, c->stream>>>(p, v, n);
  LAUNCH_CHECK(c);
  return FG_OK;
}

__global__ void nchw_to_nhwc_kernel(const float* __restrict__ src, float* __restrict__ dst, int B, int C, int HW) {
  const int64_t n = (int64_t)B * C * HW;
  for (int64_t i = blockIdx.x * (int64_t)blockDim.x + threadIdx.x; i < n; i += (int64_t)gridDim.x * blockDim.x) {
    const int ch = (int)(i % C);
    const int64_t r = i / C;
    const int p = (int)(r % HW);
    const int b = (int)(r / HW);
    dst[i] = src[((int64_t)b * C + ch) * HW + p];
  }
}
__global__ void nhwc_to_nchw_kernel(const float* __restrict__ src, float* __restrict__ dst, int B, int C, int HW) {
  const int64_t n = (int64_t)B * C * HW;
  for (int64_t i = blockIdx.x * (int64_t)blockDim.x + threadIdx.x; i < n; i += (int64_t)gridDim.x * blockDim.x) {
    const int p = (int)(i % HW);
    const int64_t r = i / HW;
    const int ch = (int)(r % C);
    const int b = (int)(r / C);
    dst[i] = src[((int64_t)b * HW + p) * C + ch];
  }
}
int k_nchw_to_nhwc(fg_ctx* c, const float* src, float* dst, int B, int C, int HW) {
  nchw_to_nhwc_kernel<<<grid_for((int64_t)B * C * HW, 256), 256, 0, c->stream>>>(src, dst, B, C, HW);
  LAUNCH_CHECK(c);
  return FG_OK;
}
int k_nhwc_to_nchw(fg_ctx* c, const float* src, float* dst, int B, int C, int HW) {
  nhwc_to_nchw_kernel<<<grid_for((int64_t)B * C * HW, 256), 256, 0, c->stream>>>(src, dst, B, C, HW);
  LAUNCH_CHECK(c);
  return FG_OK;
}

__global__ void pack_weights_kernel(const float* __restrict__ W, float* __restrict__ Wp, float* __restrict__ Wpd, int N,
                                    int Cc, int KK, int nA, int nS, int cA, int cS) {
  const int64_t total = (int64_t)N * Cc * KK;
  for (int64_t i = blockIdx.x * (int64_t)blockDim.x + threadIdx.x; i < total; i += (int64_t)gridDim.x * blockDim.x) {
    const int t = (int)(i % KK);
    const int64_t r = i / KK;
    const int ch = (int)(r % Cc);
    const int n = (int)(r / Cc);
    const int n2 = perm_idx(n, nA, nS), c2 = perm_idx(ch, cA, cS);
    const float w = W[i];
    if (Wp) Wp[((int64_t)t * N + n2) * Cc + c2] = w;
    if (Wpd) Wpd[((int64_t)(KK - 1 - t) * Cc + c2) * N + n2] = w;
  }
}
int k_pack_weights(fg_ctx* c, const float* W, float* Wp, float* Wpd, int N, int Cc, int KK, int nA, int nS, int cA,
                   int cS) {
  pack_weights_kernel<<<grid_for((int64_t)N * Cc * KK, 256), 256, 0, c->stream>>>(W, Wp, Wpd, N, Cc, KK, nA, nS, cA, cS);
  LAUNCH_CHECK(c);
  return FG_OK;
}
__global__ void unpack_wgrad_kernel(const float* __restrict__ dWp, float* __restrict__ dW, int N, int Cc, int KK, int nA,
                                    int nS, int cA, int cS) {
  const int64_t total = (int64_t)N * Cc * KK;
  for (int64_t i = blockIdx.x * (int64_t)blockDim.x + threadIdx.x; i < total; i += (int64_t)gridDim.x * blockDim.x) {
    const int t = (int)(i % KK);
    const int64_t r = i / KK;
    const int ch = (int)(r % Cc);
    const int n = (int)(r / Cc);
    const int n2 = perm_idx(n, nA, nS), c2 = perm_idx(ch, cA, cS);
    dW[i] += dWp[((int64_t)t * N + n2) * Cc + c2];
  }
}
int k_unpack_wgrad(fg_ctx* c, const float* dWp, float* dW, int N, int Cc, int KK, int nA, int nS, int cA, int cS) {
  unpack_wgrad_kernel<<<grid_for((int64_t)N * Cc * KK, 256), 256, 0, c->stream>>>(dWp, dW, N, Cc, KK, nA, nS, cA, cS);
  LAUNCH_CHECK(c);
  return FG_OK;
}

__global__ void colsum_kernel(const float* __restrict__ X, float* __restrict__ out, int64_t P, int N, int nA, int nS,
                              int64_t rows_per_block, double* __restrict__ ws, unsigned* __restrict__ ticket) {
  __shared__ double sm[8][33];
  const int col = blockIdx.x * 32 + threadIdx.x;
  const int64_t r0 = blockIdx.y * rows_per_block;
  const int64_t r1 = min(P, r0 + rows_per_block);
  double s = 0;
  if (col < N)
    for (int64_t r = r0 + threadIdx.y; r < r1; r += 8) s += X[r * N + col];
  sm[threadIdx.y][threadIdx.x] = s;
  __syncthreads();
  if (threadIdx.y == 0 && col < N) {
    double t = 0;
#pragma unroll
    for (int i = 0; i < 8; ++i) t += sm[i][threadIdx.x];
    const int j = nA == 0 ? col : (col % nA) * nS + (col / nA);
    ws[(int64_t)blockIdx.y * N + j] = t;
  }
  if (ordered_last_block(ticket)) {
    for (int j = threadIdx.y * blockDim.x + threadIdx.x; j < N; j += blockDim.x * blockDim.y)
      out[j] += (float)ordered_sum(ws, gridDim.y, N, j);
    ordered_release(ticket);
  }
}
int k_colsum_add(fg_ctx* c, const float* X, float* out, int64_t P, int N, int nA, int nS) {
  int gy = (int)std::min<int64_t>(256, (P + 255) / 256);
  if (gy < 1) gy = 1;
  const int64_t rpb = (P + gy - 1) / gy;
  dim3 grid((N + 31) / 32, gy), block(32, 8);
  FG_TRY(red_check(c, gy, N));
  colsum_kernel<<<grid, block, 0, c->stream>>>(X, out, P, N, nA, nS, rpb, c->red_ws, c->red_ticket);
  LAUNCH_CHECK(c);
  return FG_OK;
}

__global__ void prelu_fwd_kernel(const float* __restrict__ z, const float* __restrict__ slope, float* __restrict__ h,
                                 int64_t n, unsigned* __restrict__ amax) {
  const float a = *slope;
  float am = 0.f;
  for (int64_t i = blockIdx.x * (int64_t)blockDim.x + threadIdx.x; i < n; i += (int64_t)gridDim.x * blockDim.x) {
    const float v = z[i];
    const float o = v > 0.f ? v : a * v;
    h[i] = o;
    am = fmaxf(am, finite_abs(o));
  }
  amax_commit(amax, am);
}
int k_prelu_fwd(fg_ctx* c, const float* z, const float* slope, float* h, int64_t n) {
  prelu_fwd_kernel<<<grid_for(n, 256), 256, 0, c->stream>>>(z, slope, h, n, take_amax(c));
  LAUNCH_CHECK(c);
  return FG_OK;
}

__device__ __forceinline__ float load_dh(const float* __restrict__ dh, int b, int y, int x, int ch, int H, int W, int C,
                                         int pool) {
  if (!pool) return dh[(((int64_t)b * H + y) * W + x) * C + ch];
  const int64_t base = (((int64_t)b * 2 * H + 2 * y) * 2 * W + 2 * x) * C + ch;
  const int64_t rs = (int64_t)2 * W * C;
  return (dh[base] + dh[base + C]) + (dh[base + rs] + dh[base + rs + C]);
}

__global__ void prelu_bwd_kernel(const float* __restrict__ dh, const float* __restrict__ z,
                                 const float* __restrict__ slope, float* __restrict__ dz, float* __restrict__ dslope, int B,
                                 int H, int W, int C, int pool, unsigned* __restrict__ amax, double* __restrict__ ws,
                                 unsigned* __restrict__ ticket) {
  const float a = *slope;
  const int64_t n = (int64_t)B * H * W * C;
  double s = 0;
  float am = 0.f;
  for (int64_t i = blockIdx.x * (int64_t)blockDim.x + threadIdx.x; i < n; i += (int64_t)gridDim.x * blockDim.x) {
    const int ch = (int)(i % C);
    int64_t r = i / C;
    const int x = (int)(r % W);
    r /= W;
    const int y = (int)(r % H);
    const int b = (int)(r / H);
    const float g = load_dh(dh, b, y, x, ch, H, W, C, pool);
    const float v = z[i];
    if (v > 0.f) {
      dz[i] = g;
      am = fmaxf(am, finite_abs(g));
    } else {
      dz[i] = a * g;
      am = fmaxf(am, finite_abs(a * g));
      s += (double)g * (double)v;
    }
  }
  amax_commit(amax, am);
  s = block_sum(s);
  if (!dslope) return;
  if (threadIdx.x == 0) ws[blockIdx.x] = s;
  if (ordered_last_block(ticket)) {
    if (threadIdx.x == 0) *dslope += (float)ordered_sum(ws, gridDim.x, 1, 0);
    ordered_release(ticket);
  }
}
int k_prelu_bwd(fg_ctx* c, const float* dh, const float* z, const float* slope, float* dz, float* dslope, int B, int H,
                int W, int C, int pool) {
  const int64_t n = (int64_t)B * H * W * C;
  prelu_bwd_kernel<<<grid_for(n, 256, 132 * 8), 256, 0, c->stream>>>(dh, z, slope, dz, dslope, B, H, W, C, pool, take_amax(c),
                                                                    c->red_ws, c->red_ticket);
  LAUNCH_CHECK(c);
  return FG_OK;
}

__global__ void bn_stats_kernel(const float* __restrict__ z, double* __restrict__ acc, int64_t P, int C,
                                int64_t rows_per_block, double* __restrict__ ws, unsigned* __restrict__ ticket) {
  extern __shared__ double sm[];
  const int lanes = blockDim.x / C;
  const int ch = threadIdx.x % C, lane = threadIdx.x / C;
  const int64_t r0 = blockIdx.x * rows_per_block, r1 = min(P, r0 + rows_per_block);
  double s = 0, s2 = 0;
  for (int64_t r = r0 + lane; r < r1; r += lanes) {
    const double v = z[r * C + ch];
    s += v;
    s2 += v * v;
  }
  sm[threadIdx.x] = s;
  sm[blockDim.x + threadIdx.x] = s2;
  __syncthreads();
  if (lane == 0) {
    for (int l = 1; l < lanes; ++l) {
      s += sm[l * C + ch];
      s2 += sm[blockDim.x + l * C + ch];
    }
    ws[(int64_t)blockIdx.x * 2 * C + ch] = s;
    ws[(int64_t)blockIdx.x * 2 * C + C + ch] = s2;
  }
  if (ordered_last_block(ticket)) {
    for (int i = threadIdx.x; i < 2 * C; i += blockDim.x) acc[i] += ordered_sum(ws, gridDim.x, 2 * C, i);
    ordered_release(ticket);
  }
}
static inline int bn_block(int C) {
  int lanes = 256 / C;
  if (lanes < 1) lanes = 1;
  return C * lanes;
}
int k_bn_stats(fg_ctx* c, const float* z, double* acc, int64_t P, int C) {
  if (k_bn4_ok(C)) return k_bn_stats4(c, z, acc, P, C);
  if (C > 1024) {
    fg_set_error("BatchNorm with C=%d > 1024 unsupported", C);
    return FG_ERR_UNSUPPORTED;
  }
  FG_CUDA(cudaMemsetAsync(acc, 0, sizeof(double) * 2 * C, c->stream));
  const int block = bn_block(C);
  int grid = (int)std::min<int64_t>(c->sm_count * 4, (P + 63) / 64);
  if (grid < 1) grid = 1;
  const int64_t rpb = (P + grid - 1) / grid;
  FG_TRY(red_check(c, grid, 2 * C));
  bn_stats_kernel<<<grid, block, sizeof(double) * 2 * block, c->stream>>>(z, acc, P, C, rpb, c->red_ws, c->red_ticket);
  LAUNCH_CHECK(c);
  return FG_OK;
}
__global__ void bn_finalize_kernel(const double* __restrict__ acc, float* __restrict__ mean, float* __restrict__ istd,
                                   float* __restrict__ run_mean, float* __restrict__ run_var, int64_t P, int C) {
  const int ch = blockIdx.x * blockDim.x + threadIdx.x;
  if (ch >= C) return;
  const double n = (double)P;
  const double m = acc[ch] / n;
  double var = acc[C + ch] / n - m * m;
  if (var < 0) var = 0;
  mean[ch] = (float)m;
  istd[ch] = (float)(1.0 / sqrt(var + 1e-5));
  if (run_mean) run_mean[ch] = 0.9f * run_mean[ch] + 0.1f * (float)m;
  if (run_var) run_var[ch] = 0.9f * run_var[ch] + 0.1f * (float)(P > 1 ? var * n / (n - 1.0) : var);
}
int k_bn_finalize(fg_ctx* c, double* acc, float* mean, float* istd, float* run_mean, float* run_var, int64_t P, int C) {
  bn_finalize_kernel<<<(C + 127) / 128, 128, 0, c->stream>>>(acc, mean, istd, run_mean, run_var, P, C);
  LAUNCH_CHECK(c);
  return FG_OK;
}
constexpr int kBnSlices = 32;
constexpr double kBnOnePassRatio = 16.0;
__device__ __forceinline__ double bn_tile_count(int i, int nphase, int64_t phase_pixels) {
  return (double)min((int64_t)128, phase_pixels - (int64_t)(i / nphase) * 128);
}
__global__ void __launch_bounds__(256) bn_finalize_parts_kernel(const float* __restrict__ part, int nparts, int nphase,
                                                                double* __restrict__ slice_acc,
                                                                unsigned int* __restrict__ ticket, float* __restrict__ mean,
                                                                float* __restrict__ istd, float* __restrict__ run_mean,
                                                                float* __restrict__ run_var, int64_t P, int C) {
  __shared__ double sm[4][8][32];
  __shared__ bool last;
  const int lane = threadIdx.x & 31, g = threadIdx.x >> 5;
  const int ch = blockIdx.x * 32 + lane;
  const int per = (nparts + kBnSlices - 1) / kBnSlices;
  const int i0 = blockIdx.y * per, i1 = min(nparts, i0 + per);
  const int64_t pp = P / nphase;
  const double r = ch < C ? (double)part[ch] / bn_tile_count(0, nphase, pp) : 0.0;
  double s = 0, q = 0, ds = 0, dq = 0;
  if (ch < C)
    for (int i = i0 + g; i < i1; i += 8) {
      const double si = (double)part[((int64_t)i * 3 + 0) * C + ch];
      s += si;
      q += (double)part[((int64_t)i * 3 + 1) * C + ch];
      const double n = bn_tile_count(i, nphase, pp), d = si - n * r;
      ds += d;
      dq += (double)part[((int64_t)i * 3 + 2) * C + ch] + d * d * (n == 128.0 ? 1.0 / 128 : 1.0 / n);
    }
  sm[0][g][lane] = s;
  sm[1][g][lane] = q;
  sm[2][g][lane] = ds;
  sm[3][g][lane] = dq;
  __syncthreads();
  if (g == 0 && ch < C) {
    for (int k = 1; k < 8; ++k) {
      s += sm[0][k][lane];
      q += sm[1][k][lane];
      ds += sm[2][k][lane];
      dq += sm[3][k][lane];
    }
    slice_acc[((int64_t)blockIdx.y * 4 + 0) * C + ch] = s;
    slice_acc[((int64_t)blockIdx.y * 4 + 1) * C + ch] = q;
    slice_acc[((int64_t)blockIdx.y * 4 + 2) * C + ch] = ds;
    slice_acc[((int64_t)blockIdx.y * 4 + 3) * C + ch] = dq;
  }
  __threadfence();
  __syncthreads();
  if (threadIdx.x == 0) last = atomicAdd(ticket + blockIdx.x, 1u) == (unsigned)kBnSlices - 1;
  __syncthreads();
  if (!last) return;
  __threadfence();
  if (threadIdx.x == 0) ticket[blockIdx.x] = 0;
  if (g != 0 || ch >= C) return;
  s = q = ds = dq = 0;
  for (int k = 0; k < kBnSlices; ++k) {
    s += slice_acc[((int64_t)k * 4 + 0) * C + ch];
    q += slice_acc[((int64_t)k * 4 + 1) * C + ch];
    ds += slice_acc[((int64_t)k * 4 + 2) * C + ch];
    dq += slice_acc[((int64_t)k * 4 + 3) * C + ch];
  }
  const double n = (double)P;
  const double m = s / n;
  double var = q / n - m * m;
  if (var < 0) var = 0;
  if (q / n > kBnOnePassRatio * (var + 1e-5)) var = fmax(0.0, (dq - ds * (ds / n)) / n);
  mean[ch] = (float)m;
  istd[ch] = (float)(1.0 / sqrt(var + 1e-5));
  if (run_mean) run_mean[ch] = 0.9f * run_mean[ch] + 0.1f * (float)m;
  if (run_var) run_var[ch] = 0.9f * run_var[ch] + 0.1f * (float)(P > 1 ? var * n / (n - 1.0) : var);
}
int k_bn_finalize_parts(fg_ctx* c, const float* part, int nparts, int nphase, float* mean, float* istd, float* run_mean,
                        float* run_var, int64_t P, int C) {
  double* acc = c->bn_slice_acc;
  unsigned int* ticket = reinterpret_cast<unsigned int*>(acc + (size_t)kBnSlices * 4 * 256);
  bn_finalize_parts_kernel<<<dim3((C + 31) / 32, kBnSlices), 256, 0, c->stream>>>(part, nparts, nphase, acc, ticket, mean, istd,
                                                                                run_mean, run_var, P, C);
  LAUNCH_CHECK(c);
  return FG_OK;
}
__global__ void bn_eval_prep_kernel(const float* __restrict__ rm, const float* __restrict__ rv, float* __restrict__ mean,
                                    float* __restrict__ istd, int C) {
  const int ch = blockIdx.x * blockDim.x + threadIdx.x;
  if (ch >= C) return;
  mean[ch] = rm[ch];
  istd[ch] = 1.0f / sqrtf(rv[ch] + 1e-5f);
}
int k_bn_eval_prep(fg_ctx* c, const float* rm, const float* rv, float* mean, float* istd, int C) {
  bn_eval_prep_kernel<<<(C + 127) / 128, 128, 0, c->stream>>>(rm, rv, mean, istd, C);
  LAUNCH_CHECK(c);
  return FG_OK;
}
__global__ void bn_prelu_apply_kernel(const float* __restrict__ z, const float* __restrict__ mean,
                                      const float* __restrict__ istd, const float* __restrict__ gamma,
                                      const float* __restrict__ beta, const float* __restrict__ slope,
                                      float* __restrict__ h, float* __restrict__ hi, float* __restrict__ lo, int64_t n4,
                                      int C, unsigned* __restrict__ amax) {
  float am = 0.f;
  const bool act = slope != nullptr;
  const float a = act ? *slope : 1.f;
  const float4* z4 = reinterpret_cast<const float4*>(z);
  float4* h4 = reinterpret_cast<float4*>(h);
  float4* hi4 = reinterpret_cast<float4*>(hi);
  float4* lo4 = reinterpret_cast<float4*>(lo);
  for (int64_t i = blockIdx.x * (int64_t)blockDim.x + threadIdx.x; i < n4; i += (int64_t)gridDim.x * blockDim.x) {
    const int ch = (int)((i * 4) % C);
    const float4 v = z4[i];
    const float4 m = *reinterpret_cast<const float4*>(mean + ch);
    const float4 s = *reinterpret_cast<const float4*>(istd + ch);
    const float4 g = make_float4(gamma[ch], gamma[ch + 1], gamma[ch + 2], gamma[ch + 3]);
    const float4 b = make_float4(beta[ch], beta[ch + 1], beta[ch + 2], beta[ch + 3]);
    float4 o;
    o.x = g.x * ((v.x - m.x) * s.x) + b.x;
    o.y = g.y * ((v.y - m.y) * s.y) + b.y;
    o.z = g.z * ((v.z - m.z) * s.z) + b.z;
    o.w = g.w * ((v.w - m.w) * s.w) + b.w;
    if (act) {
      o.x = o.x > 0.f ? o.x : a * o.x;
      o.y = o.y > 0.f ? o.y : a * o.y;
      o.z = o.z > 0.f ? o.z : a * o.z;
      o.w = o.w > 0.f ? o.w : a * o.w;
    }
    if (h) h4[i] = o;
    am = amax4(am, o.x, o.y, o.z, o.w);
    if (hi) {
      float4 vh, vl;
      vh.x = __uint_as_float((__float_as_uint(o.x) + 0x1000u) & 0xFFFFE000u);
      vh.y = __uint_as_float((__float_as_uint(o.y) + 0x1000u) & 0xFFFFE000u);
      vh.z = __uint_as_float((__float_as_uint(o.z) + 0x1000u) & 0xFFFFE000u);
      vh.w = __uint_as_float((__float_as_uint(o.w) + 0x1000u) & 0xFFFFE000u);
      vl = make_float4(o.x - vh.x, o.y - vh.y, o.z - vh.z, o.w - vh.w);
      hi4[i] = vh;
      lo4[i] = vl;
    }
  }
  amax_commit(amax, am);
}
__global__ void bn_prelu_apply_scalar_kernel(const float* __restrict__ z, const float* __restrict__ mean,
                                             const float* __restrict__ istd, const float* __restrict__ gamma,
                                             const float* __restrict__ beta, const float* __restrict__ slope,
                                             float* __restrict__ h, int64_t n, int C) {
  const bool act = slope != nullptr;
  const float a = act ? *slope : 1.f;
  for (int64_t i = blockIdx.x * (int64_t)blockDim.x + threadIdx.x; i < n; i += (int64_t)gridDim.x * blockDim.x) {
    const int ch = (int)(i % C);
    float o = gamma[ch] * ((z[i] - mean[ch]) * istd[ch]) + beta[ch];
    if (act) o = o > 0.f ? o : a * o;
    h[i] = o;
  }
}
int k_bn_prelu_apply(fg_ctx* c, const float* z, const float* mean, const float* istd, const float* gamma,
                     const float* beta, const float* slope, float* h, int64_t P, int C, float* hi, float* lo) {
  const int64_t n = P * C;
  if (C % 4 == 0) {
    bn_prelu_apply_kernel<<<grid_for(n / 4, 256), 256, 0, c->stream>>>(z, mean, istd, gamma, beta, slope, h, hi, lo, n / 4, C,
                                                                       take_amax(c));
  } else {
    if (hi || !h) {
      fg_set_error("bn_prelu_apply: hi/lo outputs need C %% 4 == 0");
      return FG_ERR_UNSUPPORTED;
    }
    bn_prelu_apply_scalar_kernel<<<grid_for(n, 256), 256, 0, c->stream>>>(z, mean, istd, gamma, beta, slope, h, n, C);
  }
  LAUNCH_CHECK(c);
  return FG_OK;
}

__global__ void bn_prelu_bwd_reduce_kernel(const float* __restrict__ dh, const float* __restrict__ z,
                                           const float* __restrict__ mean, const float* __restrict__ istd,
                                           const float* __restrict__ gamma, const float* __restrict__ beta,
                                           const float* __restrict__ slope, double* __restrict__ acc,
                                           float* __restrict__ dslope, int B, int H, int W, int C, int pool,
                                           int64_t rows_per_block, double* __restrict__ ws, unsigned* __restrict__ ticket) {
  extern __shared__ double sm[];
  const int lanes = blockDim.x / C;
  const int ch = threadIdx.x % C, lane = threadIdx.x / C;
  const int64_t P = (int64_t)B * H * W;
  const int64_t r0 = blockIdx.x * rows_per_block, r1 = min(P, r0 + rows_per_block);
  const bool act = slope != nullptr;
  const float a = act ? *slope : 1.f;
  const float m = mean[ch], is = istd[ch], ga = gamma[ch], be = beta[ch];
  double sg = 0, sgx = 0, ss = 0;
  for (int64_t r = r0 + lane; r < r1; r += lanes) {
    float d;
    if (pool) {
      const uint32_t ru = (uint32_t)r;
      const int x = (int)(ru % (uint32_t)W);
      const uint32_t q = ru / (uint32_t)W;
      d = load_dh(dh, (int)(q / (uint32_t)H), (int)(q % (uint32_t)H), x, ch, H, W, C, 1);
    } else {
      d = dh[r * C + ch];
    }
    const float xh = (z[r * C + ch] - m) * is;
    float g = d;
    if (act) {
      const float u = ga * xh + be;
      if (!(u > 0.f)) {
        g = a * d;
        ss += (double)d * (double)u;
      }
    }
    sg += g;
    sgx += (double)g * (double)xh;
  }
  sm[threadIdx.x] = sg;
  sm[blockDim.x + threadIdx.x] = sgx;
  __syncthreads();
  if (lane == 0) {
    for (int l = 1; l < lanes; ++l) {
      sg += sm[l * C + ch];
      sgx += sm[blockDim.x + l * C + ch];
    }
    ws[(int64_t)blockIdx.x * (2 * C + 1) + ch] = sg;
    ws[(int64_t)blockIdx.x * (2 * C + 1) + C + ch] = sgx;
  }
  if (act) ss = block_sum(ss);
  if (threadIdx.x == 0) ws[(int64_t)blockIdx.x * (2 * C + 1) + 2 * C] = ss;
  if (ordered_last_block(ticket)) {
    for (int i = threadIdx.x; i < 2 * C; i += blockDim.x) acc[i] += ordered_sum(ws, gridDim.x, 2 * C + 1, i);
    if (act && dslope && threadIdx.x == 0) *dslope += (float)ordered_sum(ws, gridDim.x, 2 * C + 1, 2 * C);
    ordered_release(ticket);
  }
}
int k_bn_prelu_bwd_reduce(fg_ctx* c, const float* dh, const float* z, const float* mean, const float* istd,
                          const float* gamma, const float* beta, const float* slope, double* acc, float* dslope, int B,
                          int H, int W, int C, int pool) {
  if (!pool && k_bn4_ok(C))
    return k_bn_bwd_reduce4(c, dh, z, mean, istd, gamma, beta, slope, acc, dslope, (int64_t)B * H * W, C);
  if (C > 1024) return FG_ERR_UNSUPPORTED;
  FG_CUDA(cudaMemsetAsync(acc, 0, sizeof(double) * 2 * C, c->stream));
  const int64_t P = (int64_t)B * H * W;
  const int block = bn_block(C);
  int grid = (int)std::min<int64_t>(c->sm_count * 4, (P + 63) / 64);
  if (grid < 1) grid = 1;
  const int64_t rpb = (P + grid - 1) / grid;
  FG_TRY(red_check(c, grid, 2 * C + 1));
  bn_prelu_bwd_reduce_kernel<<<grid, block, sizeof(double) * 2 * block, c->stream>>>(dh, z, mean, istd, gamma, beta, slope,
                                                                                  acc, dslope, B, H, W, C, pool, rpb, c->red_ws,
                                                                                  c->red_ticket);
  LAUNCH_CHECK(c);
  return FG_OK;
}
__global__ void bn_bwd_finalize_kernel(const double* __restrict__ acc, float* __restrict__ mg, float* __restrict__ dgamma,
                                       float* __restrict__ dbeta, int64_t P, int C) {
  const int ch = blockIdx.x * blockDim.x + threadIdx.x;
  if (ch >= C) return;
  mg[ch] = (float)(acc[ch] / (double)P);
  mg[C + ch] = (float)(acc[C + ch] / (double)P);
  if (dgamma) dgamma[ch] += (float)acc[C + ch];
  if (dbeta) dbeta[ch] += (float)acc[ch];
}
int k_bn_bwd_finalize(fg_ctx* c, double* acc, float* mg, float* dgamma, float* dbeta, int64_t P, int C) {
  bn_bwd_finalize_kernel<<<(C + 127) / 128, 128, 0, c->stream>>>(acc, mg, dgamma, dbeta, P, C);
  LAUNCH_CHECK(c);
  return FG_OK;
}
__global__ void bn_prelu_bwd_apply_kernel(const float* __restrict__ dh, const float* __restrict__ z,
                                          const float* __restrict__ mean, const float* __restrict__ istd,
                                          const float* __restrict__ gamma, const float* __restrict__ beta,
                                          const float* __restrict__ slope, const float* __restrict__ mg,
                                          float* __restrict__ dz, int B, int H, int W, int C, int pool) {
  const bool act = slope != nullptr;
  const float a = act ? *slope : 1.f;
  const int64_t n = (int64_t)B * H * W * C;
  for (int64_t i = blockIdx.x * (int64_t)blockDim.x + threadIdx.x; i < n; i += (int64_t)gridDim.x * blockDim.x) {
    const int ch = (int)(i % C);
    int64_t r = i / C;
    const int x = (int)(r % W);
    r /= W;
    const int y = (int)(r % H);
    const int b = (int)(r / H);
    const float d = load_dh(dh, b, y, x, ch, H, W, C, pool);
    const float is = istd[ch], ga = gamma[ch];
    const float xh = (z[i] - mean[ch]) * is;
    float g = d;
    if (act) {
      const float u = ga * xh + beta[ch];
      if (!(u > 0.f)) g = a * d;
    }
    dz[i] = ga * is * (g - mg[ch] - xh * mg[C + ch]);
  }
}
__device__ void block_colsum_rows(const float (&bs)[4], int C, int n, double* ws, unsigned* ticket, float* dst,
                                  float* extra_dst, double extra = 0.0) {
  __shared__ float tb[256][4];
#pragma unroll
  for (int j = 0; j < 4; ++j) tb[threadIdx.x][j] = bs[j];
  __syncthreads();
  const int C4 = C / 4;
  double* row = ws + (int64_t)blockIdx.x * n;
  for (int i = threadIdx.x; i < C; i += blockDim.x) {
    double s = 0;
    for (int t = i / 4; t < (int)blockDim.x; t += C4) s += tb[t][i & 3];
    row[i] = s;
  }
  if (n > C && threadIdx.x == 0) row[C] = extra;
  if (ordered_last_block(ticket)) {
    if (dst)
      for (int i = threadIdx.x; i < C; i += blockDim.x) dst[i] += (float)ordered_sum(ws, gridDim.x, n, i);
    if (extra_dst && threadIdx.x == 0) *extra_dst += (float)ordered_sum(ws, gridDim.x, n, C);
    ordered_release(ticket);
  }
}

__global__ void bn_prelu_bwd_apply4_kernel(const float* __restrict__ dh, const float* __restrict__ z,
                                           const float* __restrict__ mean, const float* __restrict__ istd,
                                           const float* __restrict__ gamma, const float* __restrict__ beta,
                                           const float* __restrict__ slope, const float* __restrict__ mg,
                                           float* __restrict__ dz, float* __restrict__ hi, float* __restrict__ lo,
                                           float* __restrict__ dbias, int64_t n4, int C, unsigned* __restrict__ amax,
                                           double* __restrict__ ws, unsigned* __restrict__ ticket) {
  float am = 0.f;
  float bs[4] = {0.f, 0.f, 0.f, 0.f};
  const bool act = slope != nullptr;
  const float a = act ? *slope : 1.f;
  const float4* dh4 = reinterpret_cast<const float4*>(dh);
  const float4* z4 = reinterpret_cast<const float4*>(z);
  float4* dz4 = reinterpret_cast<float4*>(dz);
  float4* hi4 = reinterpret_cast<float4*>(hi);
  float4* lo4 = reinterpret_cast<float4*>(lo);
  const int C4 = C / 4;
  for (int64_t i = blockIdx.x * (int64_t)blockDim.x + threadIdx.x; i < n4; i += (int64_t)gridDim.x * blockDim.x) {
    const int ch = (int)(i % C4) * 4;
    const float4 d = dh4[i], v = z4[i];
    const float dv[4] = {d.x, d.y, d.z, d.w}, zv[4] = {v.x, v.y, v.z, v.w};
    float o[4];
#pragma unroll
    for (int j = 0; j < 4; ++j) {
      const float is = istd[ch + j], ga = gamma[ch + j];
      const float xh = (zv[j] - mean[ch + j]) * is;
      float g = dv[j];
      if (act) {
        const float u = ga * xh + beta[ch + j];
        if (!(u > 0.f)) g = a * g;
      }
      o[j] = ga * is * (g - mg[ch + j] - xh * mg[C + ch + j]);
    }
    dz4[i] = make_float4(o[0], o[1], o[2], o[3]);
    am = amax4(am, o[0], o[1], o[2], o[3]);
    bs[0] += o[0]; bs[1] += o[1]; bs[2] += o[2]; bs[3] += o[3];
    if (hi) {
      float h[4];
#pragma unroll
      for (int j = 0; j < 4; ++j) h[j] = __uint_as_float((__float_as_uint(o[j]) + 0x1000u) & 0xFFFFE000u);
      hi4[i] = make_float4(h[0], h[1], h[2], h[3]);
      lo4[i] = make_float4(o[0] - h[0], o[1] - h[1], o[2] - h[2], o[3] - h[3]);
    }
  }
  amax_commit(amax, am);
  if (dbias) block_colsum_rows(bs, C, C, ws, ticket, dbias, nullptr);
}
int k_bn_prelu_bwd_apply(fg_ctx* c, const float* dh, const float* z, const float* mean, const float* istd,
                         const float* gamma, const float* beta, const float* slope, const float* mg, float* dz, int B,
                         int H, int W, int C, int pool, float* hi, float* lo, float* dbias) {
  const int64_t n = (int64_t)B * H * W * C;
  if (!pool && C % 4 == 0 && C <= 1024 && 256 % (C / 4) == 0) {
    const int grid = grid_for(n / 4, 256);
    FG_TRY(red_check(c, grid, C));
    bn_prelu_bwd_apply4_kernel<<<grid, 256, 0, c->stream>>>(dh, z, mean, istd, gamma, beta, slope, mg, dz, hi, lo, dbias, n / 4,
                                                           C, take_amax(c), c->red_ws, c->red_ticket);
    LAUNCH_CHECK(c);
    return FG_OK;
  }
  if (hi) {
    fg_set_error("bn_prelu_bwd_apply: hi/lo outputs need the un-pooled float4 path");
    return FG_ERR_UNSUPPORTED;
  }
  bn_prelu_bwd_apply_kernel<<<grid_for(n, 256), 256, 0, c->stream>>>(dh, z, mean, istd, gamma, beta, slope, mg, dz, B, H,
                                                                    W, C, pool);
  LAUNCH_CHECK(c);
  if (dbias) return k_colsum_add(c, dz, dbias, (int64_t)B * H * W, C, 0, 0);
  return FG_OK;
}

__device__ __forceinline__ float sigmoidf_(float x) { return 1.0f / (1.0f + expf(-x)); }
__global__ void sigmoid_fwd_kernel(const float* __restrict__ z, float* __restrict__ y, int64_t n) {
  for (int64_t i = blockIdx.x * (int64_t)blockDim.x + threadIdx.x; i < n; i += (int64_t)gridDim.x * blockDim.x)
    y[i] = sigmoidf_(z[i]);
}
int k_sigmoid_fwd(fg_ctx* c, const float* z, float* y, int64_t n) {
  sigmoid_fwd_kernel<<<grid_for(n, 256), 256, 0, c->stream>>>(z, y, n);
  LAUNCH_CHECK(c);
  return FG_OK;
}
__global__ void sigmoid_bwd_kernel(const float* __restrict__ dy, const float* __restrict__ y, float* __restrict__ dz,
                                   int64_t n) {
  for (int64_t i = blockIdx.x * (int64_t)blockDim.x + threadIdx.x; i < n; i += (int64_t)gridDim.x * blockDim.x) {
    const float v = y[i];
    dz[i] = dy[i] * v * (1.0f - v);
  }
}
int k_sigmoid_bwd(fg_ctx* c, const float* dy, const float* y, float* dz, int64_t n) {
  sigmoid_bwd_kernel<<<grid_for(n, 256), 256, 0, c->stream>>>(dy, y, dz, n);
  LAUNCH_CHECK(c);
  return FG_OK;
}
int k_sigmoid_grad_mul(fg_ctx* c, const float* dout, const float* out, float* dlogit, int n) {
  return k_sigmoid_bwd(c, dout, out, dlogit, n);
}

__device__ __forceinline__ uint64_t splitmix64(uint64_t x) {
  x += 0x9E3779B97F4A7C15ull;
  x = (x ^ (x >> 30)) * 0xBF58476D1CE4E5B9ull;
  x = (x ^ (x >> 27)) * 0x94D049BB133111EBull;
  return x ^ (x >> 31);
}
__global__ void masks_generate_kernel(float* __restrict__ masks, int B, uint64_t seed, float p_spatial, float p_drop,
                                      const uint64_t* __restrict__ seed_dev) {
  if (seed_dev) seed += *seed_dev * 2;
  const int64_t n = (int64_t)B * kMaskPerSample;
  for (int64_t i = blockIdx.x * (int64_t)blockDim.x + threadIdx.x; i < n; i += (int64_t)gridDim.x * blockDim.x) {
    const int j = (int)(i % kMaskPerSample);
    const uint64_t r = splitmix64(seed * 0x100000001B3ull + (uint64_t)i);
    const float u = (float)(r >> 40) * (1.0f / 16777216.0f);
    masks[i] = u >= (j < 960 ? p_spatial : p_drop) ? 1.f : 0.f;
  }
}
__global__ void set_u64_kernel(uint64_t* dst, uint64_t v) { *dst = v; }
int k_set_u64(fg_ctx* c, uint64_t* dst, uint64_t v) {
  set_u64_kernel<<<1, 1, 0, c->stream>>>(dst, v);
  LAUNCH_CHECK(c);
  return FG_OK;
}
__global__ void seed_roots_kernel(uint64_t* roots, int n) {
  const int j = threadIdx.x;
  if (j >= 1 && j < n) roots[j] = (1ull << 60) | (roots[0] << 8) | (uint64_t)j;
}
int k_seed_roots(fg_ctx* c, uint64_t* roots, int n) {
  seed_roots_kernel<<<1, 32, 0, c->stream>>>(roots, n);
  LAUNCH_CHECK(c);
  return FG_OK;
}
int k_masks_generate(fg_ctx* c, float* masks, int B, uint64_t seed, float p_spatial, float p_drop, const uint64_t* seed_dev) {
  masks_generate_kernel<<<grid_for((int64_t)B * kMaskPerSample, 256), 256, 0, c->stream>>>(masks, B, seed, p_spatial,
                                                                                          p_drop, seed_dev);
  LAUNCH_CHECK(c);
  return FG_OK;
}

__device__ __forceinline__ float4 prelu4(float4 v, float a) {
  v.x = v.x > 0.f ? v.x : a * v.x;
  v.y = v.y > 0.f ? v.y : a * v.y;
  v.z = v.z > 0.f ? v.z : a * v.z;
  v.w = v.w > 0.f ? v.w : a * v.w;
  return v;
}
__device__ __forceinline__ void split4(const float4& o, float4* hi, float4* lo, uint32_t i) {
  float4 h;
  h.x = __uint_as_float((__float_as_uint(o.x) + 0x1000u) & 0xFFFFE000u);
  h.y = __uint_as_float((__float_as_uint(o.y) + 0x1000u) & 0xFFFFE000u);
  h.z = __uint_as_float((__float_as_uint(o.z) + 0x1000u) & 0xFFFFE000u);
  h.w = __uint_as_float((__float_as_uint(o.w) + 0x1000u) & 0xFFFFE000u);
  hi[i] = h;
  lo[i] = make_float4(o.x - h.x, o.y - h.y, o.z - h.z, o.w - h.w);
}
__global__ void d_act_pool_fwd_kernel(const float* __restrict__ z, const float* __restrict__ slope,
                                      const float* __restrict__ masks, int moff, float eval_scale, float* __restrict__ p,
                                      float4* __restrict__ hi, float4* __restrict__ lo, int B, int H, int W, int C,
                                      unsigned* __restrict__ amax) {
  float am = 0.f;
  const float a = *slope;
  const uint32_t Ho = H / 2, Wo = W / 2, C4 = C / 4;
  const uint32_t n = (uint32_t)B * Ho * Wo * C4;
  const float4* z4 = reinterpret_cast<const float4*>(z);
  float4* p4 = reinterpret_cast<float4*>(p);
  for (uint32_t i = blockIdx.x * blockDim.x + threadIdx.x; i < n; i += gridDim.x * blockDim.x) {
    const uint32_t c4 = i % C4;
    uint32_t r = i / C4;
    const uint32_t xo = r % Wo;
    r /= Wo;
    const uint32_t yo = r % Ho, b = r / Ho;
    float4 m = make_float4(eval_scale, eval_scale, eval_scale, eval_scale);
    if (masks) m = *reinterpret_cast<const float4*>(masks + (size_t)b * kMaskPerSample + moff + c4 * 4);
    const uint32_t base = ((b * H + 2 * yo) * W + 2 * xo) * C4 + c4, rs = (uint32_t)W * C4;
    const float4 v0 = prelu4(z4[base], a), v1 = prelu4(z4[base + C4], a), v2 = prelu4(z4[base + rs], a),
                 v3 = prelu4(z4[base + rs + C4], a);
    float4 o;
    o.x = (v0.x * m.x + v1.x * m.x + v2.x * m.x + v3.x * m.x) * 0.25f;
    o.y = (v0.y * m.y + v1.y * m.y + v2.y * m.y + v3.y * m.y) * 0.25f;
    o.z = (v0.z * m.z + v1.z * m.z + v2.z * m.z + v3.z * m.z) * 0.25f;
    o.w = (v0.w * m.w + v1.w * m.w + v2.w * m.w + v3.w * m.w) * 0.25f;
    p4[i] = o;
    am = amax4(am, o.x, o.y, o.z, o.w);
    if (hi) split4(o, hi, lo, i);
  }
  amax_commit(amax, am);
}
int k_d_act_pool_fwd(fg_ctx* c, const float* z, const float* slope, const float* masks, int moff, float eval_scale,
                     float* p, int B, int H, int W, int C, float* hi, float* lo) {
  const int64_t n = (int64_t)B * (H / 2) * (W / 2) * C / 4;
  if (C % 4 || (moff % 4) || (int64_t)B * H * W * C >= ((int64_t)1 << 31)) {
    fg_set_error("d_act_pool_fwd: unsupported shape (C %% 4, size)");
    return FG_ERR_UNSUPPORTED;
  }
  d_act_pool_fwd_kernel<<<grid_for(n, 256), 256, 0, c->stream>>>(z, slope, masks, moff, eval_scale, p, reinterpret_cast<float4*>(hi),
                                                                 reinterpret_cast<float4*>(lo), B, H, W, C, take_amax(c));
  LAUNCH_CHECK(c);
  return FG_OK;
}
__global__ void d_act_pool_bwd_kernel(const float* __restrict__ dp, const float* __restrict__ z,
                                      const float* __restrict__ slope, const float* __restrict__ masks, int moff,
                                      float eval_scale, float* __restrict__ dz, float* __restrict__ dslope,
                                      float4* __restrict__ hi, float4* __restrict__ lo, float* __restrict__ dbias, int B,
                                      int H, int W, int C, unsigned* __restrict__ amax, double* __restrict__ ws,
                                      unsigned* __restrict__ ticket) {
  float am = 0.f;
  float bs[4] = {0.f, 0.f, 0.f, 0.f};
  const float a = *slope;
  const uint32_t Ho = H / 2, Wo = W / 2, C4 = C / 4;
  const uint32_t n = (uint32_t)B * Ho * Wo * C4;
  const float4* z4 = reinterpret_cast<const float4*>(z);
  const float4* dp4 = reinterpret_cast<const float4*>(dp);
  float4* dz4 = reinterpret_cast<float4*>(dz);
  float s = 0.f;
  double sd = 0;
  for (uint32_t i = blockIdx.x * blockDim.x + threadIdx.x; i < n; i += gridDim.x * blockDim.x) {
    const uint32_t c4 = i % C4;
    uint32_t r = i / C4;
    const uint32_t xo = r % Wo;
    r /= Wo;
    const uint32_t yo = r % Ho, b = r / Ho;
    float4 m = make_float4(eval_scale, eval_scale, eval_scale, eval_scale);
    if (masks) m = *reinterpret_cast<const float4*>(masks + (size_t)b * kMaskPerSample + moff + c4 * 4);
    const float4 d = dp4[i];
    const float4 g = make_float4(d.x * 0.25f * m.x, d.y * 0.25f * m.y, d.z * 0.25f * m.z, d.w * 0.25f * m.w);
    const uint32_t base = ((b * H + 2 * yo) * W + 2 * xo) * C4 + c4, rs = (uint32_t)W * C4;
    s = 0.f;
#pragma unroll
    for (int q = 0; q < 4; ++q) {
      const uint32_t idx = base + (q & 1) * C4 + (q >> 1) * rs;
      const float4 v = z4[idx];
      float4 o;
      o.x = v.x > 0.f ? g.x : a * g.x;
      o.y = v.y > 0.f ? g.y : a * g.y;
      o.z = v.z > 0.f ? g.z : a * g.z;
      o.w = v.w > 0.f ? g.w : a * g.w;
      if (!(v.x > 0.f)) s = fmaf(g.x, v.x, s);
      if (!(v.y > 0.f)) s = fmaf(g.y, v.y, s);
      if (!(v.z > 0.f)) s = fmaf(g.z, v.z, s);
      if (!(v.w > 0.f)) s = fmaf(g.w, v.w, s);
      dz4[idx] = o;
      am = amax4(am, o.x, o.y, o.z, o.w);
      bs[0] += o.x; bs[1] += o.y; bs[2] += o.z; bs[3] += o.w;
      if (hi) split4(o, hi, lo, idx);
    }
    sd += (double)s;
  }
  amax_commit(amax, am);
  sd = block_sum(sd);
  if (dbias || dslope) block_colsum_rows(bs, dbias ? (int)C : 0, (dbias ? (int)C : 0) + 1, ws, ticket, dbias, dslope, sd);
}
int k_d_act_pool_bwd(fg_ctx* c, const float* dp, const float* z, const float* slope, const float* masks, int moff,
                     float eval_scale, float* dz, float* dslope, int B, int H, int W, int C, float* hi, float* lo,
                     float* dbias) {
  const int64_t n = (int64_t)B * (H / 2) * (W / 2) * C / 4;
  if (C % 4 || (moff % 4) || (int64_t)B * H * W * C >= ((int64_t)1 << 31)) {
    fg_set_error("d_act_pool_bwd: unsupported shape (C %% 4, size)");
    return FG_ERR_UNSUPPORTED;
  }
  const bool fuse = dbias && C <= 512 && 256 % (C / 4) == 0;
  const int grid = grid_for(n, 256, 132 * 8);
  FG_TRY(red_check(c, grid, C + 1));
  d_act_pool_bwd_kernel<<<grid, 256, 0, c->stream>>>(dp, z, slope, masks, moff, eval_scale, dz, dslope,
                                                    reinterpret_cast<float4*>(hi), reinterpret_cast<float4*>(lo),
                                                    fuse ? dbias : nullptr, B, H, W, C, take_amax(c), c->red_ws, c->red_ticket);
  LAUNCH_CHECK(c);
  if (dbias && !fuse) return k_colsum_add(c, dz, dbias, (int64_t)B * H * W, C, 0, 0);
  return FG_OK;
}
__global__ void lin_act_drop_fwd_kernel(const float* __restrict__ z, const float* __restrict__ slope,
                                        const float* __restrict__ masks, int moff, float scale, float* __restrict__ h,
                                        int B, int N, unsigned* __restrict__ amax) {
  float am = 0.f;
  const float a = *slope;
  const int64_t n = (int64_t)B * N;
  for (int64_t i = blockIdx.x * (int64_t)blockDim.x + threadIdx.x; i < n; i += (int64_t)gridDim.x * blockDim.x) {
    const int j = (int)(i % N);
    const int b = (int)(i / N);
    const float v = z[i];
    const float act = v > 0.f ? v : a * v;
    const float o = masks ? act * masks[(int64_t)b * kMaskPerSample + moff + j] * scale : act;
    h[i] = o;
    am = fmaxf(am, finite_abs(o));
  }
  amax_commit(amax, am);
}
int k_lin_act_drop_fwd(fg_ctx* c, const float* z, const float* slope, const float* masks, int moff, float scale,
                       float* h, int B, int N) {
  lin_act_drop_fwd_kernel<<<grid_for((int64_t)B * N, 256), 256, 0, c->stream>>>(z, slope, masks, moff, scale, h, B, N, take_amax(c));
  LAUNCH_CHECK(c);
  return FG_OK;
}
__global__ void lin_act_drop_bwd_kernel(const float* __restrict__ dh, const float* __restrict__ z,
                                        const float* __restrict__ slope, const float* __restrict__ masks, int moff,
                                        float scale, float* __restrict__ dz, float* __restrict__ dslope, int B, int N,
                                        unsigned* __restrict__ amax, double* __restrict__ ws, unsigned* __restrict__ ticket) {
  float am = 0.f;
  const float a = *slope;
  const int64_t n = (int64_t)B * N;
  double s = 0;
  for (int64_t i = blockIdx.x * (int64_t)blockDim.x + threadIdx.x; i < n; i += (int64_t)gridDim.x * blockDim.x) {
    const int j = (int)(i % N);
    const int b = (int)(i / N);
    const float g = masks ? dh[i] * masks[(int64_t)b * kMaskPerSample + moff + j] * scale : dh[i];
    const float v = z[i];
    if (v > 0.f) {
      dz[i] = g;
      am = fmaxf(am, finite_abs(g));
    } else {
      dz[i] = a * g;
      am = fmaxf(am, finite_abs(a * g));
      s += (double)g * (double)v;
    }
  }
  amax_commit(amax, am);
  s = block_sum(s);
  if (!dslope) return;
  if (threadIdx.x == 0) ws[blockIdx.x] = s;
  if (ordered_last_block(ticket)) {
    if (threadIdx.x == 0) *dslope += (float)ordered_sum(ws, gridDim.x, 1, 0);
    ordered_release(ticket);
  }
}
int k_lin_act_drop_bwd(fg_ctx* c, const float* dh, const float* z, const float* slope, const float* masks, int moff,
                       float scale, float* dz, float* dslope, int B, int N) {
  lin_act_drop_bwd_kernel<<<grid_for((int64_t)B * N, 256, 132), 256, 0, c->stream>>>(dh, z, slope, masks, moff, scale, dz,
                                                                                   dslope, B, N, take_amax(c), c->red_ws,
                                                                                   c->red_ticket);
  LAUNCH_CHECK(c);
  return FG_OK;
}

__device__ __forceinline__ float bce_term(float x, float t) {
  const float eps = 1e-12f;
  return t * logf(x + eps) + (1.0f - t) * logf(1.0f - x + eps);
}
__device__ __forceinline__ float bce_grad(float x, float t, float invN) {
  const float eps = 1e-12f;
  return -(t - x) / (x * (1.0f - x + eps) + eps) * invN;
}
__global__ void sigmoid_bce_kernel(const float* __restrict__ logit, float* __restrict__ out, float* __restrict__ dlogit,
                                   float* __restrict__ loss_out, float* __restrict__ tail4, int B, int n_ones) {
  double s = 0;
  int c0 = 0, c1 = 0, c2 = 0, c3 = 0;
  const float invN = 1.0f / (float)B;
  for (int i = threadIdx.x; i < B; i += blockDim.x) {
    const float y = sigmoidf_(logit[i]);
    const float t = i < n_ones ? 1.f : 0.f;
    out[i] = y;
    s += (double)bce_term(y, t);
    dlogit[i] = bce_grad(y, t, invN) * y * (1.0f - y);
    const bool pred1 = y > 0.5f;
    if (t > 0.5f) {
      if (pred1) c0++; else c1++;
    } else {
      if (pred1) c2++; else c3++;
    }
  }
  s = block_sum(s);
  const double d0 = block_sum((double)c0), d1 = block_sum((double)c1), d2 = block_sum((double)c2),
               d3 = block_sum((double)c3);
  if (threadIdx.x == 0) {
    *loss_out = (float)(-s / (double)B);
    if (tail4) {
      tail4[0] = (float)d0;
      tail4[1] = (float)d1;
      tail4[2] = (float)d2;
      tail4[3] = (float)d3;
    }
  }
}
int k_sigmoid_bce(fg_ctx* c, const float* logit, float* out, float* dlogit, float* loss_out, float* tail4, int B,
                  int n_ones) {
  sigmoid_bce_kernel<<<1, 256, 0, c->stream>>>(logit, out, dlogit, loss_out, tail4, B, n_ones);
  LAUNCH_CHECK(c);
  return FG_OK;
}
__global__ void bce_fwd_kernel(const float* __restrict__ x, const float* __restrict__ t, int n, float* __restrict__ loss) {
  double s = 0;
  for (int i = threadIdx.x; i < n; i += blockDim.x) s += (double)bce_term(x[i], t[i]);
  s = block_sum(s);
  if (threadIdx.x == 0) *loss = (float)(-s / (double)n);
}
__global__ void bce_bwd_kernel(const float* __restrict__ x, const float* __restrict__ t, int n, float* __restrict__ dx) {
  const float invN = 1.0f / (float)n;
  for (int i = blockIdx.x * blockDim.x + threadIdx.x; i < n; i += gridDim.x * blockDim.x) dx[i] = bce_grad(x[i], t[i], invN);
}
int k_bce_fwd(fg_ctx* c, const float* x, const float* t, int n, float* loss_out) {
  bce_fwd_kernel<<<1, 256, 0, c->stream>>>(x, t, n, loss_out);
  LAUNCH_CHECK(c);
  return FG_OK;
}
int k_bce_bwd(fg_ctx* c, const float* x, const float* t, int n, float* dx) {
  bce_bwd_kernel<<<grid_for(n, 256), 256, 0, c->stream>>>(x, t, n, dx);
  LAUNCH_CHECK(c);
  return FG_OK;
}

__global__ void penalty_loss_kernel(const float* __restrict__ p, int64_t n, float l1, float l2, float* __restrict__ loss,
                                    double* __restrict__ ws, unsigned* __restrict__ ticket) {
  double s1 = 0, s2 = 0;
  for (int64_t i = blockIdx.x * (int64_t)blockDim.x + threadIdx.x; i < n; i += (int64_t)gridDim.x * blockDim.x) {
    const double v = p[i];
    s1 += fabs(v);
    s2 += v * v;
  }
  s1 = block_sum(s1);
  s2 = block_sum(s2);
  if (threadIdx.x == 0) ws[blockIdx.x] = l1 * s1 + l2 * s2 * 0.5;
  if (ordered_last_block(ticket)) {
    if (threadIdx.x == 0) *loss += (float)ordered_sum(ws, gridDim.x, 1, 0);
    ordered_release(ticket);
  }
}
int k_penalty_loss(fg_ctx* c, const float* p, int64_t n, float l1, float l2, float* loss_inout) {
  penalty_loss_kernel<<<grid_for(n, 256, kOptRedRows), 256, 0, c->stream>>>(p, n, l1, l2, loss_inout, c->red_ws_opt,
                                                                           c->red_ticket + 1);
  LAUNCH_CHECK(c);
  return FG_OK;
}
__device__ __forceinline__ float step_size(const fg_hyper& h, int opt, float lr, double t) {
  if (opt != FG_OPT_ADAM) return lr;
  return (float)((double)lr * sqrt(1.0 - pow((double)h.beta2, t)) / (1.0 - pow((double)h.beta1, t)));
}
__global__ void gate_prep_kernel(DeviceStats* st, float* acc_hist, int net, fg_hyper h, const float* tail4, float total, int opt,
                                 int accumulate) {
  if (threadIdx.x != 0 || blockIdx.x != 0) return;
  if (net == FG_NET_D) {
    int interval = h.accs_interval;
    if (interval < 1) interval = 1;
    if (interval > kAccHistMax) interval = kAccHistMax;
    const float correct = tail4[0] + tail4[3];
    const float tV = correct / total;
    for (int i = 0; i < 4; ++i) st->conf[i] = (accumulate ? st->conf[i] : 0) + (int)(tail4[i] + 0.5f);
    st->acc_D = tV;
    acc_hist[st->acc_head] = tV;
    st->acc_head = (st->acc_head + 1) % interval;
    if (st->acc_count < interval) st->acc_count++;
    double m = 0;
    for (int i = 0; i < st->acc_count; ++i) m += acc_hist[i];
    m /= st->acc_count;
    const int go = m < (double)h.D_maxAcc ? 1 : 0;
    st->do_train_D = go;
    st->trained_D = (accumulate ? st->trained_D : 0) + go;
    if (go) {
      st->t_D += 1;
      st->step_D = step_size(h, opt, h.lr_D, (double)st->t_D);
    }
  } else {
    st->do_train_G = 1;
    st->t_G += 1;
    st->step_G = step_size(h, opt, h.lr_G, (double)st->t_G);
  }
}
int k_gate_and_prep(fg_ctx* c, DeviceStats* st, float* acc_hist, int net, const fg_hyper* h, const float* tail4, int B,
                    float world, bool accumulate) {
  gate_prep_kernel<<<1, 32, 0, c->stream>>>(st, acc_hist, net, *h, tail4, (float)B * world, net == FG_NET_D ? c->opt_D : c->opt_G,
                                            accumulate ? 1 : 0);
  LAUNCH_CHECK(c);
  return FG_OK;
}
__global__ void optim_prep_kernel(DeviceStats* st, int net, fg_hyper h, int opt) {
  if (threadIdx.x != 0 || blockIdx.x != 0) return;
  if (net == FG_NET_D) {
    st->do_train_D = 1;
    st->t_D += 1;
    st->step_D = step_size(h, opt, h.lr_D, (double)st->t_D);
  } else {
    st->do_train_G = 1;
    st->t_G += 1;
    st->step_G = step_size(h, opt, h.lr_G, (double)st->t_G);
  }
}
int k_optim_prep(fg_ctx* c, DeviceStats* st, int net, const fg_hyper* h) {
  optim_prep_kernel<<<1, 32, 0, c->stream>>>(st, net, *h, net == FG_NET_D ? c->opt_D : c->opt_G);
  LAUNCH_CHECK(c);
  return FG_OK;
}
__global__ void adam_kernel(float* __restrict__ p, float* __restrict__ g, float* __restrict__ m, float* __restrict__ v,
                            int64_t n, float beta1, float beta2, float eps, float l1_grad, float l2, float clampv,
                            float grad_scale, const float* __restrict__ step_dev, const int* __restrict__ flag_dev,
                            float step_host, int update, int mode, float mom, const int* __restrict__ t_dev) {
  if (flag_dev && *flag_dev == 0) update = 0;
  const float step = step_dev ? *step_dev : step_host;
  const bool first = t_dev ? *t_dev == 1 : false;
  const bool pen = (l1_grad != 0.f) || (l2 != 0.f);
  for (int64_t i = blockIdx.x * (int64_t)blockDim.x + threadIdx.x; i < n; i += (int64_t)gridDim.x * blockDim.x) {
    const float pv = p[i];
    float gv = g[i] * grad_scale;
    if (pen) {
      const float sg = pv > 0.f ? 1.f : (pv < 0.f ? -1.f : 0.f);
      gv += sg * l1_grad + pv * l2;
    }
    if (clampv != 0.f) gv = fminf(fmaxf(gv, -clampv), clampv);
    g[i] = gv;
    if (!update) continue;
    if (mode == FG_OPT_ADAM) {
      const float mv = m[i] * beta1 + (1.0f - beta1) * gv;
      const float vv = v[i] * beta2 + (1.0f - beta2) * gv * gv;
      m[i] = mv;
      v[i] = vv;
      p[i] = pv - step * mv / (sqrtf(vv) + eps);
    } else if (mode == FG_OPT_ADAGRAD) {
      const float vv = v[i] + gv * gv;
      v[i] = vv;
      p[i] = pv - step * gv / (sqrtf(vv) + 1e-10f);
    } else {
      float ge = gv;
      if (mom != 0.f) {
        ge = first ? gv : m[i] * mom + (1.0f - mom) * gv;
        m[i] = ge;
      }
      p[i] = pv - step * ge;
    }
  }
}
__global__ void gemv_fwd_kernel(const float* __restrict__ x, const float* __restrict__ w, const float* __restrict__ bias,
                                float* __restrict__ out, int B, int K) {
  const int row = (blockIdx.x * blockDim.x + threadIdx.x) >> 5, lane = threadIdx.x & 31;
  if (row >= B) return;
  float s = 0.f;
  for (int k = lane; k < K; k += 32) s = fmaf(x[(size_t)row * K + k], w[k], s);
#pragma unroll
  for (int o = 16; o > 0; o >>= 1) s += __shfl_xor_sync(0xffffffffu, s, o);
  if (lane == 0) out[row] = s + (bias ? bias[0] : 0.f);
}
__global__ void gemv_dgrad_kernel(const float* __restrict__ dy, const float* __restrict__ w, float* __restrict__ dx, int B,
                                  int K) {
  const int n = B * K;
  for (int i = blockIdx.x * blockDim.x + threadIdx.x; i < n; i += gridDim.x * blockDim.x) dx[i] = dy[i / K] * w[i % K];
}
__global__ void gemv_wgrad_kernel(const float* __restrict__ x, const float* __restrict__ dy, float* __restrict__ dw,
                                  float* __restrict__ db, int B, int K) {
  const int k = blockIdx.x * blockDim.x + threadIdx.x;
  if (k < K) {
    float s = 0.f;
    for (int b = 0; b < B; ++b) s = fmaf(dy[b], x[(size_t)b * K + k], s);
    dw[k] += s;
  }
  if (k == 0 && db) {
    float s = 0.f;
    for (int b = 0; b < B; ++b) s += dy[b];
    db[0] += s;
  }
}
int k_gemv_fwd(fg_ctx* c, const float* x, const float* w, const float* bias, float* out, int B, int K) {
  gemv_fwd_kernel<<<(B * 32 + 255) / 256, 256, 0, c->stream>>>(x, w, bias, out, B, K);
  LAUNCH_CHECK(c);
  return FG_OK;
}
int k_gemv_dgrad(fg_ctx* c, const float* dy, const float* w, float* dx, int B, int K) {
  gemv_dgrad_kernel<<<grid_for((int64_t)B * K, 256), 256, 0, c->stream>>>(dy, w, dx, B, K);
  LAUNCH_CHECK(c);
  return FG_OK;
}
int k_gemv_wgrad_add(fg_ctx* c, const float* x, const float* dy, float* dw, float* db, int B, int K) {
  gemv_wgrad_kernel<<<(K + 127) / 128, 128, 0, c->stream>>>(x, dy, dw, db, B, K);
  LAUNCH_CHECK(c);
  return FG_OK;
}

int k_adam(fg_ctx* c, float* p, const float* g, float* m, float* v, int64_t n, float beta1, float beta2, float eps,
           float l1_grad, float l2, float clampv, float grad_scale, const float* step_dev, const int* flag_dev,
           float step_host, float* g_out) {
  (void)g_out;
  adam_kernel<<<grid_for(n, 256, 132 * 8), 256, 0, c->stream>>>(p, const_cast<float*>(g), m, v, n, beta1, beta2, eps,
                                                               l1_grad, l2, clampv, grad_scale, step_dev, flag_dev,
                                                               step_host, 1, FG_OPT_ADAM, 0.f, nullptr);
  LAUNCH_CHECK(c);
  return FG_OK;
}
int k_optim_update(fg_ctx* c, int mode, float* p, float* g, float* m, float* v, int64_t n, float beta1, float beta2, float eps,
                   float mom, float l1_grad, float l2, float clampv, float grad_scale, const float* step_dev,
                   const int* flag_dev, const int* t_dev) {
  adam_kernel<<<grid_for(n, 256, 132 * 8), 256, 0, c->stream>>>(p, g, m, v, n, beta1, beta2, eps, l1_grad, l2, clampv, grad_scale,
                                                               step_dev, flag_dev, 0.f, 1, mode, mom, t_dev);
  LAUNCH_CHECK(c);
  return FG_OK;
}
```

### face_generator_b200/csrc/nets.cu

```cuda
#include <algorithm>

#include "fg_internal.h"
#include "k_conv_tc.h"
#include "ups_gan.h"

namespace {
struct DLayout {
  int64_t cW[4], cb[4], ca[4], L1W, L1b, a5, L2W, L2b, a6, L3W, L3b, total;
};

DLayout make_d_layout(int C) {
  DLayout L;
  const int cin[4] = {C, 64, 128, 256}, cout[4] = {64, 128, 256, 512};
  int64_t o = 0;
  for (int i = 0; i < 4; ++i) {
    L.cW[i] = o; o += (int64_t)cout[i] * cin[i] * 9;
    L.cb[i] = o; o += cout[i];
    L.ca[i] = o; o += 1;
  }
  L.L1W = o; o += 512 * 2048;
  L.L1b = o; o += 512;
  L.a5 = o; o += 1;
  L.L2W = o; o += 512 * 512;
  L.L2b = o; o += 512;
  L.a6 = o; o += 1;
  L.L3W = o; o += 512;
  L.L3b = o; o += 1;
  L.total = o;
  return L;
}

const int kDcin[4] = {0 , 64, 128, 256}, kDcout[4] = {64, 128, 256, 512}, kDhw[4] = {32, 16, 8, 4};
const int kDmoff[4] = {0, 64, 192, 448};
inline int dcin(const fg_ctx* c, int i) { return i == 0 ? c->C : kDcin[i]; }

struct D32 final : GanD {
  DLayout dl;
  ConvL Dc[4], DL1, DL2;
  ScalePairs pairs;
  bool train = true, fwd_valid = false;
  float *z[4] = {nullptr, nullptr, nullptr, nullptr}, *p[4] = {nullptr, nullptr, nullptr, nullptr};
  float *zl1 = nullptr, *hl1 = nullptr, *zl2 = nullptr, *hl2 = nullptr;
  float drop_scale = 2.0f, spatial_eval = 0.8f;
  float *dh = nullptr, *dzl = nullptr, *dz = nullptr, *dp = nullptr;
  std::vector<NetPair::Keep> bwd_keep;
  int bwd_keep_B = 0;

  ~D32() override {
    for (NetPair::Keep& k : bwd_keep)
      if (k.copy) cudaFree(k.copy);
  }
  int64_t layout(int C) override {
    dl = make_d_layout(C);
    return dl.total;
  }
  int dalloc(float** q, size_t elems) { return convl_dalloc(n->env, q, elems); }
  int alloc() override;
  int forward(const float* x, int B, bool training, const fg_hyper* h) override;
  int keep_bwd(int k, const float* src, int B);
  int backward(bool want_wgrad, bool want_dx) override;
  int draw_masks(int B, uint64_t seed, const fg_hyper* h, const uint64_t* root) override {
    return k_masks_generate(n->c, masks, B, seed, h->p_spatial, h->p_drop, root);
  }
  void debug_rows(std::vector<DebugTensor>& ents) const override;
};

int D32::alloc() {
  fg_ctx* c = n->c;
  ConvLEnv& e = n->env;
  const size_t B = c->maxB, C = c->C;
  FG_TRY(dalloc(&e.ws, std::max<size_t>(9 * 512 * 256, 8192 * (128 + kNoiseDim))));
  FG_TRY(dalloc(&x, B * 1024 * C));
  for (int i = 0; i < 4; ++i) {
    const size_t n_z = B * (size_t)kDhw[i] * kDhw[i] * kDcout[i];
    FG_TRY(dalloc(&z[i], n_z));
    FG_TRY(dalloc(&p[i], n_z / 4));
  }
  FG_TRY(dalloc(&zl1, B * 512));
  FG_TRY(dalloc(&hl1, B * 512));
  FG_TRY(dalloc(&zl2, B * 512));
  FG_TRY(dalloc(&hl2, B * 512));
  FG_TRY(dalloc(&logit, B));
  FG_TRY(dalloc(&out, B));
  FG_TRY(dalloc(&masks, B * kMaskPerSample));
  FG_TRY(dalloc(&dlogit, B));
  FG_TRY(dalloc(&dh, B * 512));
  FG_TRY(dalloc(&dzl, B * 512));
  FG_TRY(dalloc(&dz, B * 65536));
  FG_TRY(dalloc(&dp, B * 16384));
  FG_TRY(dalloc(&dx, B * 1024 * C));
  FG_TRY(dalloc(&e.dy.hi, B * 131072));
  FG_TRY(dalloc(&e.dy.lo, B * 131072));
  FG_TRY(pairs.alloc(c, n->allocs, 1 + 2 * 6));
  FG_TRY(pairs.take(&e.dy.s));
  auto conv = [&](ConvL& L, int Cin, int Cout, int k, int H, int64_t w_off, int64_t b_off, const char* tf, const char* td,
                  const char* tw) {
    L.Cin = Cin; L.Cout = Cout; L.k = k; L.H = H;
    L.w_off = w_off; L.b_off = b_off;
    L.tf = tf; L.td = td; L.tw = tw;
  };
  static const char* tf[4] = {"D.C1.fwd", "D.C2.fwd", "D.C3.fwd", "D.C4.fwd"};
  static const char* td[4] = {"D.C1.dgrad", "D.C2.dgrad", "D.C3.dgrad", "D.C4.dgrad"};
  static const char* tw[4] = {"D.C1.wgrad", "D.C2.wgrad", "D.C3.wgrad", "D.C4.wgrad"};
  for (int i = 0; i < 4; ++i) conv(Dc[i], dcin(c, i), kDcout[i], 3, kDhw[i], dl.cW[i], dl.cb[i], tf[i], td[i], tw[i]);
  conv(DL1, 2048, 512, 1, 1, dl.L1W, dl.L1b, "D.L1.fwd", "D.L1.dgrad", "D.L1.wgrad");
  DL1.cA = 512; DL1.cS = 4;
  conv(DL2, 512, 512, 1, 1, dl.L2W, dl.L2b, "D.L2.fwd", "D.L2.dgrad", "D.L2.wgrad");
  for (ConvL* L : {&Dc[0], &Dc[1], &Dc[2], &Dc[3], &DL1, &DL2}) {
    FG_TRY(pairs.take(&L->x.s));
    FG_TRY(pairs.take(&L->sdy));
    FG_TRY(convl_alloc(e, *L));
  }
  n->net.keep = {{"Dstep.z1", z[0], 65536}, {"Dstep.z2", z[1], 32768}, {"Dstep.z3", z[2], 16384},
                 {"Dstep.z4", z[3], 8192},  {"Dstep.zl1", zl1, 512},    {"Dstep.zl2", zl2, 512},
                 {"Dstep.logit", logit, 1}, {"Dstep.out", out, 1}};
  bwd_keep = {{"Dbwd.dh3", nullptr, 512},    {"Dbwd.dzl2", nullptr, 512},  {"Dbwd.dh2", nullptr, 512},
              {"Dbwd.dzl1", nullptr, 512},   {"Dbwd.dp4", nullptr, 2048},  {"Dbwd.dz4", nullptr, 8192},
              {"Dbwd.dp3", nullptr, 4096},   {"Dbwd.dz3", nullptr, 16384}, {"Dbwd.dp2", nullptr, 8192},
              {"Dbwd.dz2", nullptr, 32768},  {"Dbwd.dp1", nullptr, 16384}, {"Dbwd.dz1", nullptr, 65536}};
  return FG_OK;
}

int D32::forward(const float* xin, int Bn, bool training, const fg_hyper* h) {
  fg_ctx* c = n->c;
  FG_REQUIRE(Bn >= 1 && Bn <= c->maxB, "D forward: batch %d out of range [1,%d]", Bn, c->maxB);
  FG_TRY(gan_pack_D(*n, {&Dc[0], &Dc[1], &Dc[2], &Dc[3], &DL1, &DL2}));
  FG_TRY(pairs.reset(c));
  const DLayout& L = dl;
  float* P = n->net.PD;
  ConvLEnv& e = n->env;
  if (xin != x) FG_CUDA(cudaMemcpyAsync(x, xin, sizeof(float) * (size_t)Bn * 1024 * c->C, cudaMemcpyDeviceToDevice, c->stream));
  B = Bn;
  train = training;
  const float* m = training ? masks : nullptr;
  const float* cur = x;
  for (int i = 0; i < 4; ++i) {
    const int H = kDhw[i];
    FG_TRY(convl_fwd(e, Dc[i], cur, P, z[i], B));
    TcOp& nx = (i < 3 ? Dc[i + 1] : DL1).x;
    nx.split_ready = convl_tc_fwd(c, i < 3 ? Dc[i + 1] : DL1) && !tc_f16(c);
    {
      AmaxInto am(c, nx);
      FG_TRY(k_d_act_pool_fwd(c, z[i], P + L.ca[i], m, kDmoff[i], 1.0f - h->p_spatial, p[i], B, H, H, kDcout[i],
                              nx.split_ready ? nx.hi : nullptr, nx.split_ready ? nx.lo : nullptr));
    }
    cur = p[i];
  }
  const float scale = 1.0f / (1.0f - h->p_drop);
  drop_scale = scale;
  spatial_eval = 1.0f - h->p_spatial;
  FG_TRY(convl_fwd(e, DL1, p[3], P, zl1, B));
  {
    AmaxInto am(c, DL2.x);
    FG_TRY(k_lin_act_drop_fwd(c, zl1, P + L.a5, m, 960, scale, hl1, B, 512));
  }
  FG_TRY(convl_fwd(e, DL2, hl1, P, zl2, B));
  FG_TRY(k_lin_act_drop_fwd(c, zl2, P + L.a6, m, 1472, scale, hl2, B, 512));
  {
    ScopedTimer tm(c, "D.L3.fwd");
    FG_TRY(k_gemv_fwd(c, hl2, P + L.L3W, P + L.L3b, logit, B, 512));
  }
  fwd_valid = true;
  return FG_OK;
}

int D32::keep_bwd(int k, const float* src, int Bn) {
  fg_ctx* c = n->c;
  if (!c->debug_keep) return FG_OK;
  NetPair::Keep& e = bwd_keep[k];
  if (!e.copy) FG_CUDA(cudaMalloc((void**)&e.copy, sizeof(float) * c->maxB * e.per));
  FG_CUDA(cudaMemcpyAsync(e.copy, src, sizeof(float) * Bn * e.per, cudaMemcpyDeviceToDevice, c->stream));
  bwd_keep_B = Bn;
  return FG_OK;
}

int D32::backward(bool want_wgrad, bool want_dx) {
  fg_ctx* c = n->c;
  if (!fwd_valid) {
    fg_set_error("D backward needs a preceding D forward");
    return FG_ERR_STATE;
  }
  const DLayout& L = dl;
  float *P = n->net.PD, *G = n->net.gD;
  const float* m = train ? masks : nullptr;
  const float scale = drop_scale, eval_scale = spatial_eval;
  ConvLEnv& e = n->env;
  FG_TRY(pairs.reset(c));
  if (want_wgrad) {
    ScopedTimer tm(c, "D.L3.wgrad");
    FG_TRY(k_gemv_wgrad_add(c, hl2, dlogit, G + L.L3W, G + L.L3b, B, 512));
  }
  {
    ScopedTimer tm(c, "D.L3.dgrad");
    FG_TRY(k_gemv_dgrad(c, dlogit, P + L.L3W, dh, B, 512));
  }
  FG_TRY(keep_bwd(0, dh, B));
  TcOp& dy = e.dy;
  float* GD = want_wgrad ? G : nullptr;
  {
    AmaxInto am(c, DL2.sdy, &dy.amax_ready);
    FG_TRY(k_lin_act_drop_bwd(c, dh, zl2, P + L.a6, m, 1472, scale, dzl, want_wgrad ? G + L.a6 : nullptr, B, 512));
  }
  FG_TRY(keep_bwd(1, dzl, B));
  FG_TRY(convl_bwd(e, DL2, hl1, dzl, GD, dh, B));
  FG_TRY(keep_bwd(2, dh, B));
  {
    AmaxInto am(c, DL1.sdy, &dy.amax_ready);
    FG_TRY(k_lin_act_drop_bwd(c, dh, zl1, P + L.a5, m, 960, scale, dzl, want_wgrad ? G + L.a5 : nullptr, B, 512));
  }
  FG_TRY(keep_bwd(3, dzl, B));
  FG_TRY(convl_bwd(e, DL1, p[3], dzl, GD, dp, B));
  for (int i = 3; i >= 0; --i) {
    const int H = kDhw[i];
    FG_TRY(keep_bwd(4 + 2 * (3 - i), dp, B));
    dy.split_ready = convl_tc_bwd(c, Dc[i]) && !tc_f16(c);
    dy.bias_ready = want_wgrad;
    {
      AmaxInto am(c, Dc[i].sdy, &dy.amax_ready);
      FG_TRY(k_d_act_pool_bwd(c, dp, z[i], P + L.ca[i], m, kDmoff[i], eval_scale, dz, want_wgrad ? G + L.ca[i] : nullptr, B,
                              H, H, kDcout[i], dy.split_ready ? dy.hi : nullptr, dy.split_ready ? dy.lo : nullptr,
                              want_wgrad ? G + L.cb[i] : nullptr));
    }
    FG_TRY(keep_bwd(5 + 2 * (3 - i), dz, B));
    float* din = i > 0 ? dp : want_dx ? dx : nullptr;
    FG_TRY(convl_bwd(e, Dc[i], i == 0 ? x : p[i - 1], dz, GD, din, B));
  }
  return FG_OK;
}

void D32::debug_rows(std::vector<DebugTensor>& ents) const {
  const int db = B;
  ents.insert(ents.end(), {{"D.z1", z[0], 65536, db}, {"D.z2", z[1], 32768, db}, {"D.z3", z[2], 16384, db},
                           {"D.z4", z[3], 8192, db}, {"D.p1", p[0], 16384, db}, {"D.p2", p[1], 8192, db},
                           {"D.p3", p[2], 4096, db}, {"D.p4", p[3], 2048, db}, {"D.logit", logit, 1, db},
                           {"D.out", out, 1, db}, {"D.dx", dx, 1024 * n->c->C, db}, {"D.masks", masks, kMaskPerSample, db},
                           {"D.zl1", zl1, 512, db}, {"D.hl1", hl1, 512, db}, {"D.zl2", zl2, 512, db},
                           {"D.hl2", hl2, 512, db}, {"D.dlogit", dlogit, 1, db}});
  for (const NetPair::Keep& k : bwd_keep) ents.push_back({k.name, k.copy, k.per, bwd_keep_B});
}
}

struct Net32 : UpsGan {
  float *ownPG = nullptr, *ownPD = nullptr, *ownGG = nullptr, *ownGD = nullptr;
  float* tail_sep = nullptr;
};

int net32_alloc(fg_ctx* c) {
  Net32* n = c->n32 = new Net32();
  static const GanDesc k32{{32, "", 128, true}, kMaskPerSample, true};
  FG_TRY(gan_alloc(*n, c, k32, std::make_unique<D32>(), c->io_dev));
  NetPair& p = n->net;
  p.optim_timer[0] = "hbm.optim.G";
  p.optim_timer[1] = "hbm.optim.D";
  n->ownPG = p.PG; n->ownPD = p.PD; n->ownGG = p.gG; n->ownGD = p.gD;
  FG_TRY(fg_dalloc(c, n->allocs, &n->tail_sep, 2 * kGradTail));
  FG_CUDA(cudaStreamSynchronize(c->stream));
  return FG_OK;
}
void net32_free(fg_ctx* c) {
  if (!c->n32) return;
  gan_free(*c->n32);
  delete c->n32;
  c->n32 = nullptr;
}
NetPair& net32_pair(fg_ctx* c) { return c->n32->net; }

#define ENTER(c)                                      \
  do {                                                \
    if (!(c)) {                                       \
      fg_set_error("null fg_ctx");                    \
      return FG_ERR_INVALID;                          \
    }                                                 \
    FG_CUDA(cudaSetDevice((c)->device));              \
  } while (0)

namespace {
int train_step_iters(fg_ctx* c, const char* what, const fg_hyper* h, int B, int d_iters, int g_iters, const float* real,
                     const float* noise_D, const float* noise_G, const float* masks_D, const float* masks_G, uint64_t seed,
                     fg_step_stats* stats) {
  ENTER(c);
  return gan_train_step_iters(*c->n32, what, h, B, d_iters, g_iters, real, noise_D, noise_G, masks_D, masks_G, seed, stats);
}

int train_step_dataset_iters(fg_ctx* c, fg_dataset* d, const char* what, const fg_hyper* h, int B, int d_iters, int g_iters,
                             uint64_t seed, fg_step_stats* stats) {
  if (!d || !d->c) {
    fg_set_error("null fg_dataset");
    return FG_ERR_INVALID;
  }
  FG_CUDA(cudaSetDevice(d->c->device));
  if (!c) return step_check(c, what, B, d_iters, g_iters, h, d, true);
  return gan_train_step_dataset_iters(*c->n32, d, what, h, B, d_iters, g_iters, seed, stats);
}
}

extern "C" {

int64_t fg_param_count(int net, int channels) {
  if (channels != 1 && channels != 3) return -1;
  return net == FG_NET_G ? make_g_layout(channels, 32).total : net == FG_NET_D ? make_d_layout(channels).total : -1;
}
int fg_set_params(fg_ctx* c, int net, const float* src) {
  ENTER(c);
  FG_REQUIRE(net == FG_NET_G || net == FG_NET_D, "net must be FG_NET_G or FG_NET_D");
  return pair_set_params(c, c->n32->net, net, src);
}
int fg_get_params(fg_ctx* c, int net, float* dst) {
  ENTER(c);
  FG_REQUIRE(net == FG_NET_G || net == FG_NET_D, "net must be FG_NET_G or FG_NET_D");
  return pair_get_params(c, c->n32->net, net, dst);
}
int fg_get_grads(fg_ctx* c, int net, float* dst) {
  ENTER(c);
  FG_REQUIRE(net == FG_NET_G || net == FG_NET_D, "net must be FG_NET_G or FG_NET_D");
  return pair_get_grads(c, c->n32->net, net, dst);
}
int fg_zero_grads(fg_ctx* c, int net) {
  ENTER(c);
  FG_REQUIRE(net == FG_NET_G || net == FG_NET_D, "net must be FG_NET_G or FG_NET_D");
  return pair_zero_grads(c, c->n32->net, net);
}
int fg_bind_params(fg_ctx* c, int net, float* params_dev, float* grads_dev) {
  ENTER(c);
  c->graph_epoch++;
  FG_REQUIRE(net == FG_NET_G || net == FG_NET_D, "net must be FG_NET_G or FG_NET_D");
  for (const float* p : {params_dev, grads_dev}) {
    if (!p) continue;
    FG_REQUIRE(fg_is_dev(p), "fg_bind_params: buffers must be DEVICE memory (CudaTensor:data())");
    FG_REQUIRE(reinterpret_cast<uintptr_t>(p) % 16 == 0, "fg_bind_params: buffers must be 16-byte aligned");
  }
  FG_CUDA(cudaStreamSynchronize(c->stream));
  Net32* n = c->n32;
  NetPair& np = n->net;
  const bool d = net == FG_NET_D;
  (d ? np.PD : np.PG) = params_dev ? params_dev : (d ? n->ownPD : n->ownPG);
  float* own_g = d ? n->ownGD : n->ownGG;
  const int64_t len = d ? np.nD : np.nG;
  (d ? np.gD : np.gG) = grads_dev ? grads_dev : own_g;
  (d ? np.tailD : np.tailG) = grads_dev ? n->tail_sep + (d ? kGradTail : 0) : own_g + len;
  np.G_pack = np.D_pack = -1;
  return FG_OK;
}
float* fg_params_ptr(fg_ctx* c, int net) {
  return !c ? nullptr : net == FG_NET_D ? c->n32->net.PD : net == FG_NET_G ? c->n32->net.PG : nullptr;
}
float* fg_grads_ptr(fg_ctx* c, int net) {
  return !c ? nullptr : net == FG_NET_D ? c->n32->net.gD : net == FG_NET_G ? c->n32->net.gG : nullptr;
}

int fg_set_adam_state(fg_ctx* c, int net, const float* m, const float* v, int t) {
  ENTER(c);
  FG_REQUIRE(net == FG_NET_G || net == FG_NET_D, "net must be FG_NET_G or FG_NET_D");
  return pair_set_adam_state(c, c->n32->net, net, m, v, t);
}
int fg_get_adam_state(fg_ctx* c, int net, float* m, float* v, int* t) {
  ENTER(c);
  FG_REQUIRE(net == FG_NET_G || net == FG_NET_D, "net must be FG_NET_G or FG_NET_D");
  return pair_get_adam_state(c, c->n32->net, net, m, v, t);
}
int fg_set_bn_state(fg_ctx* c, const float* src) {
  ENTER(c);
  return pair_set_bn_state(c, c->n32->net, src);
}
int fg_get_bn_state(fg_ctx* c, float* dst) {
  ENTER(c);
  return pair_get_bn_state(c, c->n32->net, dst);
}

int fg_G_forward(fg_ctx* c, const float* noise, int B, int training, float* images_out) {
  ENTER(c);
  FG_REQUIRE(noise && B >= 1 && B <= c->maxB, "fg_G_forward: bad arguments (B=%d, max %d)", B, c->maxB);
  c->n32->net.G_pack = -1;
  return gan_G_forward(*c->n32, noise, B, training != 0, images_out);
}
int fg_G_backward(fg_ctx* c, const float* d_images, float* d_noise) {
  ENTER(c);
  FG_REQUIRE(d_images, "fg_G_backward: d_images is null");
  return gan_G_backward(*c->n32, d_images, d_noise);
}
int fg_D_forward(fg_ctx* c, const float* images, int B, int training, const float* masks, uint64_t seed, float* out) {
  ENTER(c);
  FG_REQUIRE(images && B >= 1 && B <= c->maxB, "fg_D_forward: bad arguments (B=%d, max %d)", B, c->maxB);
  c->n32->net.D_pack = -1;
  return gan_D_forward(*c->n32, images, B, training != 0, masks, seed, out);
}
int fg_D_backward(fg_ctx* c, const float* d_out, int want_wgrad, float* d_images) {
  ENTER(c);
  FG_REQUIRE(d_out, "fg_D_backward: d_out is null");
  return gan_D_backward(*c->n32, d_out, want_wgrad != 0, d_images);
}
int fg_bce_forward(fg_ctx* c, const float* x, const float* t, int n, float* loss_out) {
  ENTER(c);
  FG_REQUIRE(x && t && loss_out && n > 0 && n <= c->maxB, "fg_bce_forward: bad arguments");
  const float *xd, *td;
  FG_TRY(fg_to_dev(c, x, n, c->n32->img[0], &xd));
  FG_TRY(fg_to_dev(c, t, n, c->n32->img[1], &td));
  FG_TRY(k_bce_fwd(c, xd, td, n, c->n32->z[0]));
  return fg_to_user(c, loss_out, c->n32->z[0], 1);
}
int fg_bce_backward(fg_ctx* c, const float* x, const float* t, int n, float* dx) {
  ENTER(c);
  FG_REQUIRE(x && t && dx && n > 0 && n <= c->maxB, "fg_bce_backward: bad arguments");
  const float *xd, *td;
  FG_TRY(fg_to_dev(c, x, n, c->n32->img[0], &xd));
  FG_TRY(fg_to_dev(c, t, n, c->n32->img[1], &td));
  FG_TRY(k_bce_bwd(c, xd, td, n, c->n32->z[0]));
  return fg_to_user(c, dx, c->n32->z[0], n);
}
int fg_optim_step(fg_ctx* c, int net, const fg_hyper* h, float grad_scale) {
  ENTER(c);
  FG_REQUIRE(h && (net == FG_NET_G || net == FG_NET_D), "fg_optim_step: bad arguments");
  FG_TRY(k_optim_prep(c, c->n32->net.dstats, net, h));
  return pair_optim(c, c->n32->net, net, h, grad_scale);
}

int fg_train_step(fg_ctx* c, const fg_hyper* h, int B, const float* real, const float* noise_D, const float* noise_G,
                  const float* masks_D, const float* masks_G, uint64_t seed, fg_step_stats* stats) {
  return train_step_iters(c, "fg_train_step", h, B, 1, 1, real, noise_D, noise_G, masks_D, masks_G, seed, stats);
}
int fg_train_step_iters(fg_ctx* c, const fg_hyper* h, int B, int d_iters, int g_iters, const float* real,
                        const float* noise_D, const float* noise_G, const float* masks_D, const float* masks_G, uint64_t seed,
                        fg_step_stats* stats) {
  return train_step_iters(c, "fg_train_step_iters", h, B, d_iters, g_iters, real, noise_D, noise_G, masks_D, masks_G, seed,
                          stats);
}
int fg_train_step_dataset(fg_ctx* c, fg_dataset* d, const fg_hyper* h, int B, uint64_t seed, fg_step_stats* stats) {
  return train_step_dataset_iters(c, d, "fg_train_step_dataset", h, B, 1, 1, seed, stats);
}
int fg_train_step_dataset_iters(fg_ctx* c, fg_dataset* d, const fg_hyper* h, int B, int d_iters, int g_iters, uint64_t seed,
                                fg_step_stats* stats) {
  return train_step_dataset_iters(c, d, "fg_train_step_dataset_iters", h, B, d_iters, g_iters, seed, stats);
}

int fg_sample(fg_ctx* c, const float* noise, int N, int chunk, float* images_out) {
  ENTER(c);
  FG_REQUIRE(noise && images_out && N >= 1 && chunk >= 1 && chunk <= c->maxB, "fg_sample: bad arguments (chunk %d, max %d)",
             chunk, c->maxB);
  Net32* n = c->n32;
  const bool out_dev = fg_is_dev(images_out);
  const size_t img = (size_t)c->C * 1024;
  n->net.G_pack = -1;
  for (int s = 0; s < N; s += chunk) {
    const int b = std::min(chunk, N - s);
    const float* nd;
    FG_TRY(fg_to_dev(c, noise + (size_t)s * kNoiseDim, (size_t)b * kNoiseDim, n->z[0], &nd));
    FG_TRY(gen_forward(n->env, n->G, n->net, nd, b, true));
    float* dst = images_out + (size_t)s * img;
    if (out_dev) {
      FG_TRY(k_nhwc_to_nchw(c, n->G.y, dst, b, c->C, 1024));
    } else {
      FG_TRY(k_nhwc_to_nchw(c, n->G.y, n->img[0], b, c->C, 1024));
      FG_CUDA(cudaMemcpyAsync(dst, n->img[0], b * img * sizeof(float), cudaMemcpyDeviceToHost, c->stream));
      if (s + chunk < N) FG_CUDA(cudaStreamSynchronize(c->stream));
    }
  }
  if (!out_dev) FG_CUDA(cudaStreamSynchronize(c->stream));
  return FG_OK;
}

int64_t fg_debug_tensor(fg_ctx* c, const char* name, float* dst, int64_t max_elems) {
  if (!c || !name) return -1;
  return gan_debug_tensor(*c->n32, "fg_debug_tensor", name, dst, max_elems);
}

}
```

### face_generator_b200/csrc/ups_gan.cu

```cuda
#include "ups_gan.h"

namespace {
struct GanStep final : StepNets {
  UpsGan& n;
  GanD& D;
  const float *real, *noiseD, *noiseG;
  GanStep(UpsGan& n, const fg_hyper* h, int B, const float* real, const float* noiseD, const float* noiseG)
      : StepNets(n.c, n.net, h, B, n.D->logit, n.D->out, n.D->dlogit, n.D->masks, n.d.mask, true, n.d.overlap), n(n),
        D(*n.D), real(real), noiseD(noiseD), noiseG(noiseG) {}
  int g_forward(int j, bool d_iter) override {
    const int rows = d_iter ? B / 2 : B;
    return gen_forward(n.env, n.G, n.net, (d_iter ? noiseD : noiseG) + (size_t)j * rows * kNoiseDim, rows, true);
  }
  int d_input(int j) override {
    const int Bh = B / 2, HW = n.G.S * n.G.S;
    const size_t img = (size_t)c->C * HW;
    FG_TRY(k_nchw_to_nhwc(c, real + (size_t)j * Bh * img, D.x, Bh, c->C, HW));
    FG_CUDA(cudaMemcpyAsync(D.x + Bh * img, n.G.y, sizeof(float) * Bh * img, cudaMemcpyDeviceToDevice, c->stream));
    return FG_OK;
  }
  int draw_masks(int kind, const uint64_t* root) override { return D.draw_masks(B, kind, h, root); }
  int d_forward(bool on_g) override { return D.forward(on_g ? n.G.y : D.x, B, true, h); }
  int d_backward(bool want_wgrad, bool want_dx) override { return D.backward(want_wgrad, want_dx); }
  int g_backward() override { return gen_backward(n.env, n.G, n.net, D.dx, nullptr); }
};
}

int gan_alloc(UpsGan& n, fg_ctx* c, const GanDesc& d, std::unique_ptr<GanD> D, float* io) {
  n.c = c;
  n.d = d;
  n.D = std::move(D);
  n.D->n = &n;
  ConvLEnv& e = n.env;
  e.c = c;
  e.maxB = c->maxB;
  e.allocs = &n.allocs;
  FG_TRY(pair_alloc(c, n.allocs, n.net, make_g_layout(c->C, d.g.side).total, n.D->layout(c->C), true));
  FG_TRY(n.D->alloc());
  FG_TRY(gen_alloc(e, n.G, d.g));
  const size_t B = c->maxB, img = B * d.g.side * d.g.side * c->C;
  n.img[0] = io;
  if (!io) FG_TRY(convl_dalloc(e, &n.img[0], img));
  FG_TRY(convl_dalloc(e, &n.img[1], img));
  FG_TRY(convl_dalloc(e, &n.z[0], B * kNoiseDim));
  FG_TRY(convl_dalloc(e, &n.z[1], B * kNoiseDim));
  FG_CUDA(cudaStreamSynchronize(c->stream));
  return FG_OK;
}

void gan_free(UpsGan& n) {
  pair_free(n.net);
  n.D.reset();
  for (void* p : n.allocs) cudaFree(p);
  n.allocs.clear();
}

int gan_pack_D(UpsGan& n, std::initializer_list<ConvL*> layers) {
  if (n.net.D_pack == pack_key(n.c)) return FG_OK;
  for (ConvL* L : layers) FG_TRY(convl_pack(n.c, *L, n.net.PD));
  n.net.D_pack = pack_key(n.c);
  return FG_OK;
}

int gan_train_step_iters(UpsGan& n, const char* what, const fg_hyper* h, int B, int d_iters, int g_iters, const float* real,
                         const float* noise_D, const float* noise_G, const float* masks_D, const float* masks_G, uint64_t seed,
                         fg_step_stats* stats) {
  fg_ctx* c = n.c;
  FG_TRY(step_check(c, what, B, d_iters, g_iters, h && real && noise_D && noise_G));
  const size_t nd = d_iters, ng = g_iters, Bh = B / 2, M = c->maxB, mask = n.d.mask;
  const size_t img = (size_t)c->C * n.G.S * n.G.S;
  IterStage& s = n.iter_stage;
  const float *r, *zd, *zg, *md, *mg;
  FG_TRY(s.in(c, n.allocs, 0, real, nd * Bh * img, nd * M / 2 * img, &r));
  FG_TRY(s.in(c, n.allocs, 1, noise_D, nd * Bh * kNoiseDim, nd * M / 2 * kNoiseDim, &zd));
  FG_TRY(s.in(c, n.allocs, 2, noise_G, ng * B * kNoiseDim, ng * M * kNoiseDim, &zg));
  FG_TRY(s.in(c, n.allocs, 3, masks_D, nd * B * mask, nd * M * mask, &md));
  FG_TRY(s.in(c, n.allocs, 4, masks_G, ng * B * mask, ng * M * mask, &mg));
  GanStep st(n, h, B, r, zd, zg);
  return pair_train_step(st, d_iters, g_iters, md, mg, seed, {r, zd, zg, md, mg, nullptr}, nullptr, stats);
}

int gan_train_step_dataset_iters(UpsGan& n, fg_dataset* d, const char* what, const fg_hyper* h, int B, int d_iters,
                                 int g_iters, uint64_t seed, fg_step_stats* stats) {
  fg_ctx* c = n.c;
  FG_TRY(step_check(c, what, B, d_iters, g_iters, h, d, true));
  const int Bh = B / 2, S = n.G.S;
  const size_t M = c->maxB, img = (size_t)c->C * S * S;
  IterStage& s = n.iter_stage;
  FG_TRY(s.reserve(c, n.allocs, 0, d_iters * M / 2 * img));
  FG_TRY(s.reserve(c, n.allocs, 1, d_iters * M / 2 * kNoiseDim));
  FG_TRY(s.reserve(c, n.allocs, 2, g_iters * M * kNoiseDim));
  float *real = s.p[0], *zd = s.p[1], *zg = s.p[2];
  const std::function<int()> feed = [&]() -> int {
    for (int j = 0; j < d_iters; ++j) {
      FG_TRY(dataset_draw_gather(d, 0, Bh, S, real + (size_t)j * Bh * img, c->seed_dev + j, 4));
      FG_TRY(noise_uniform_dev(c, 1, (int64_t)Bh * kNoiseDim, zd + (size_t)j * Bh * kNoiseDim, c->seed_dev + j, 4));
    }
    for (int j = 0; j < g_iters; ++j)
      FG_TRY(noise_uniform_dev(c, 2, (int64_t)B * kNoiseDim, zg + (size_t)j * B * kNoiseDim, c->seed_dev + j, 4));
    return FG_OK;
  };
  GanStep st(n, h, B, real, zd, zg);
  return pair_train_step(st, d_iters, g_iters, nullptr, nullptr, seed, {real, zd, zg, nullptr, nullptr, d}, &feed, stats);
}

int gan_G_forward(UpsGan& n, const float* noise, int B, bool training, float* images_out) {
  fg_ctx* c = n.c;
  const int HW = n.G.S * n.G.S;
  const float* nd;
  FG_TRY(fg_to_dev(c, noise, (size_t)B * kNoiseDim, n.z[0], &nd));
  FG_TRY(gen_forward(n.env, n.G, n.net, nd, B, training));
  if (images_out) {
    FG_TRY(k_nhwc_to_nchw(c, n.G.y, n.img[0], B, c->C, HW));
    FG_TRY(fg_to_user(c, images_out, n.img[0], (size_t)B * c->C * HW));
  }
  return FG_OK;
}

int gan_G_backward(UpsGan& n, const float* d_images, float* d_noise) {
  fg_ctx* c = n.c;
  const int B = n.G.B, HW = n.G.S * n.G.S;
  const float* dd;
  FG_TRY(fg_to_dev(c, d_images, (size_t)B * c->C * HW, n.img[0], &dd));
  FG_TRY(k_nchw_to_nhwc(c, dd, n.img[1], B, c->C, HW));
  float* dn = nullptr;
  if (d_noise) dn = fg_is_dev(d_noise) ? d_noise : n.z[1];
  FG_TRY(gen_backward(n.env, n.G, n.net, n.img[1], dn));
  if (d_noise && dn != d_noise) FG_TRY(fg_to_user(c, d_noise, dn, (size_t)B * kNoiseDim));
  return FG_OK;
}

int gan_D_forward(UpsGan& n, const float* images, int B, bool training, const float* masks, uint64_t seed, float* out) {
  fg_ctx* c = n.c;
  GanD& D = *n.D;
  const int HW = n.G.S * n.G.S;
  fg_hyper h;
  fg_hyper_default(&h);
  const float* xd;
  FG_TRY(fg_to_dev(c, images, (size_t)B * c->C * HW, n.img[0], &xd));
  FG_TRY(k_nchw_to_nhwc(c, xd, D.x, B, c->C, HW));
  if (training) {
    if (masks) {
      FG_CUDA(cudaMemcpyAsync(D.masks, masks, sizeof(float) * B * n.d.mask, cudaMemcpyDefault, c->stream));
    } else {
      FG_TRY(D.draw_masks(B, seed, &h, nullptr));
    }
  }
  FG_TRY(D.forward(D.x, B, training, &h));
  FG_TRY(k_sigmoid_fwd(c, D.logit, D.out, B));
  if (out) FG_TRY(fg_to_user(c, out, D.out, B));
  return FG_OK;
}

int gan_D_backward(UpsGan& n, const float* d_out, bool want_wgrad, float* d_images) {
  fg_ctx* c = n.c;
  GanD& D = *n.D;
  const int B = D.B, HW = n.G.S * n.G.S;
  const float* dd;
  FG_TRY(fg_to_dev(c, d_out, B, n.z[0], &dd));
  FG_TRY(k_sigmoid_grad_mul(c, dd, D.out, D.dlogit, B));
  FG_TRY(D.backward(want_wgrad, d_images != nullptr));
  if (d_images) {
    FG_TRY(k_nhwc_to_nchw(c, D.dx, n.img[0], B, c->C, HW));
    FG_TRY(fg_to_user(c, d_images, n.img[0], (size_t)B * c->C * HW));
  }
  return FG_OK;
}

int64_t gan_debug_tensor(UpsGan& n, const char* what, const char* name, float* dst, int64_t max_elems) {
  cudaSetDevice(n.c->device);
  std::vector<DebugTensor> ents;
  n.D->debug_rows(ents);
  pair_keep_rows(n.net, ents);
  gen_debug_rows(n.G, ents);
  return debug_tensor_copy(n.c, what, ents.data(), ents.size(), name, dst, max_elems);
}
```

Measured before the change: 37010.

## Fuse generator BN2+PReLU apply into final conv forward and wgrad input loads

When the last generator conv runs on the edge reduce kernel, BatchNorm and PReLU are applied on the fly to the raw pre-BN activations it loads. This removes the separate bn_prelu_apply pass and the h2 write/read through HBM. The conv wgrad kernel likewise recomputes the normalised input from z2 rather than reading h2. h2 is written out only when debug_keep or the public forward API asks for it. The cost is extra per-element arithmetic, and a halved pixels-per-lane tile for the single-output-channel variant, which may lower throughput.

```diff
diff --git a/face_generator_b200/csrc/convl.cu b/face_generator_b200/csrc/convl.cu
--- a/face_generator_b200/csrc/convl.cu
+++ b/face_generator_b200/csrc/convl.cu
@@ -118,8 +118,14 @@
   return FG_OK;
 }
 
-int convl_fwd(ConvLEnv& e, ConvL& L, const float* in, const float* P, float* out, int B) {
-  fg_ctx* c = e.c;
+bool convl_bn_input(const fg_ctx* c, const ConvL& L) {
+  const ConvGeom g = L.geom(1);
+  return c->edge_impl && k_edge_eligible(g) && g.Cout <= 4 && k_small_eligible(g) && !L.pad_out && !tc_f(c, L, 1);
+}
+
+int convl_fwd(ConvLEnv& e, ConvL& L, const float* in, const float* P, float* out, int B, const BnPrelu& xf, float* xout) {
+  fg_ctx* c = e.c;
+  FG_REQUIRE(!xf.mean || convl_bn_input(c, L), "convl_fwd: no BatchNorm-input kernel for this layer");
   const ConvGeom g = L.geom(B);
   const float* bias = L.bp ? L.bp : P + L.b_off;
   const bool h = L.packed_f16;
@@ -145,12 +151,13 @@
     return tc_conv_fwd(c, L.x.hi, L.x.lo, L.Wf_hi, L.Wf_lo, bias, out, gk, 0, nullptr, nullptr, h, os);
   }
   ScopedTimer t(c, L.tf);
-  if (c->edge_impl && k_edge_eligible(g)) return k_conv_edge(c, in, L.Wp, bias, out, g);
+  if (c->edge_impl && k_edge_eligible(g)) return k_conv_edge(c, in, L.Wp, bias, out, g, xf, xout);
   return k_small_eligible(g) ? k_conv_small(c, in, L.Wp, bias, out, g) : k_conv_simt(c, in, L.Wp, bias, out, g);
 }
 
-int convl_bwd(ConvLEnv& e, ConvL& L, const float* in, const float* dy, float* G, float* din, int B) {
-  fg_ctx* c = e.c;
+int convl_bwd(ConvLEnv& e, ConvL& L, const float* in, const float* dy, float* G, float* din, int B, const BnPrelu& xf) {
+  fg_ctx* c = e.c;
+  FG_REQUIRE(!xf.mean || convl_bn_input(c, L), "convl_bwd: no BatchNorm-input kernel for this layer");
   const ConvGeom g = L.geom(B), gd = L.geom_d(B);
   const bool w_tc = G && tc_w(c, L, B), d_tc = din && tc_d(c, L, B);
   const bool h = L.packed_f16;
@@ -188,7 +195,7 @@
     {
       ScopedTimer t(c, L.tw);
       if (w_tc) FG_TRY(tc_conv_wgrad(c, L.x.hi, L.x.lo, e.dy.hi, e.dy.lo, e.ws + koff, L.geom_k(B), h, osy, osx));
-      else if (k_small_eligible(g)) FG_TRY(k_wgrad_small(c, in, dy, e.ws, g));
+      else if (k_small_eligible(g)) FG_TRY(k_wgrad_small(c, in, dy, e.ws, g, xf));
       else FG_TRY(k_wgrad_simt(c, in, dy, e.ws, g));
     }
     if (koff)
diff --git a/face_generator_b200/csrc/convl.h b/face_generator_b200/csrc/convl.h
--- a/face_generator_b200/csrc/convl.h
+++ b/face_generator_b200/csrc/convl.h
@@ -31,8 +31,10 @@
 bool convl_tc_fwd(const fg_ctx* c, const ConvL& L);
 bool convl_tc_bwd(const fg_ctx* c, const ConvL& L);
 int convl_pack(fg_ctx* c, ConvL& L, const float* P);
-int convl_fwd(ConvLEnv& e, ConvL& L, const float* in, const float* P, float* out, int B);
-int convl_bwd(ConvLEnv& e, ConvL& L, const float* in, const float* dy, float* G, float* din, int B);
+bool convl_bn_input(const fg_ctx* c, const ConvL& L);
+int convl_fwd(ConvLEnv& e, ConvL& L, const float* in, const float* P, float* out, int B, const BnPrelu& xf = {},
+              float* xout = nullptr);
+int convl_bwd(ConvLEnv& e, ConvL& L, const float* in, const float* dy, float* G, float* din, int B, const BnPrelu& xf = {});
 
 bool upsl_tc(const fg_ctx* c, const UpsL& U);
 int upsl_alloc(ConvLEnv& e, UpsL& U);
@@ -42,6 +44,6 @@
 
 int gen_alloc(ConvLEnv& e, UpsGen& G, const GenDesc& d);
 int gen_pack(fg_ctx* c, UpsGen& G, NetPair& p);
-int gen_forward(ConvLEnv& e, UpsGen& G, NetPair& p, const float* noise, int B, bool training);
+int gen_forward(ConvLEnv& e, UpsGen& G, NetPair& p, const float* noise, int B, bool training, bool keep_h2);
 int gen_backward(ConvLEnv& e, UpsGen& G, NetPair& p, const float* dy, float* dnoise);
 void gen_debug_rows(const UpsGen& G, std::vector<DebugTensor>& rows);
diff --git a/face_generator_b200/csrc/fg_internal.h b/face_generator_b200/csrc/fg_internal.h
--- a/face_generator_b200/csrc/fg_internal.h
+++ b/face_generator_b200/csrc/fg_internal.h
@@ -181,9 +181,9 @@
   float *bn_mean[2] = {nullptr, nullptr}, *bn_istd[2] = {nullptr, nullptr}, *bn_mg = nullptr;
   int B = 0;
   bool train = true, valid = false;
+  bool c3_bn = false;
   std::deque<std::string> names;
-  const char *t_bn2_finalize = nullptr, *t_bn2_stats = nullptr, *t_bn2_apply = nullptr, *t_bn2_bwd_reduce = nullptr,
-             *t_bn2_bwd_apply = nullptr;
+  const char *t_bn2_finalize = nullptr, *t_bn2_stats = nullptr, *t_bn2_bwd_reduce = nullptr, *t_bn2_bwd_apply = nullptr;
 };
 
 struct TimerRec {
@@ -345,12 +345,17 @@
 
 int k_conv_simt(fg_ctx* c, const float* in, const float* Wp, const float* bias, float* out, ConvGeom g);
 int k_wgrad_simt(fg_ctx* c, const float* in, const float* dY, float* dWp, ConvGeom g);
+struct BnPrelu {
+  const float *mean = nullptr, *istd = nullptr, *gamma = nullptr, *beta = nullptr, *slope = nullptr;
+};
+
 bool k_small_eligible(const ConvGeom& g);
 int k_conv_small(fg_ctx* c, const float* in, const float* Wp, const float* bias, float* out, ConvGeom g);
-int k_wgrad_small(fg_ctx* c, const float* in, const float* dY, float* dWp, ConvGeom g);
+int k_wgrad_small(fg_ctx* c, const float* in, const float* dY, float* dWp, ConvGeom g, const BnPrelu& xf = {});
 
 bool k_edge_eligible(const ConvGeom& g);
-int k_conv_edge(fg_ctx* c, const float* in, const float* Wp, const float* bias, float* out, ConvGeom g);
+int k_conv_edge(fg_ctx* c, const float* in, const float* Wp, const float* bias, float* out, ConvGeom g,
+                const BnPrelu& xf = {}, float* xout = nullptr);
 
 inline int red_check(fg_ctx* c, int64_t rows, int64_t n) {
   if (rows * n > (int64_t)c->red_ws_elems) {
diff --git a/face_generator_b200/csrc/gen.cu b/face_generator_b200/csrc/gen.cu
--- a/face_generator_b200/csrc/gen.cu
+++ b/face_generator_b200/csrc/gen.cu
@@ -68,7 +68,6 @@
   }
   G.t_bn2_finalize = timer("G.bn2.finalize");
   G.t_bn2_stats = timer("hbm.G.bn2.stats");
-  G.t_bn2_apply = timer("hbm.G.bn2.apply");
   G.t_bn2_bwd_reduce = timer("hbm.G.bn2.bwd_reduce");
   G.t_bn2_bwd_apply = timer("hbm.G.bn2.bwd_apply");
   const size_t B = e.maxB, n0 = L1.Cout, n1 = (size_t)256 * (S / 2) * (S / 2), n2 = (size_t)128 * S * S, n3 = (size_t)C * S * S;
@@ -110,9 +109,12 @@
   }
   return k_bn_finalize(c, c->bn_acc, G.bn_mean[i], G.bn_istd[i], rm, rv, P, Cc);
 }
-}
-
-int gen_forward(ConvLEnv& e, UpsGen& G, NetPair& p, const float* noise, int B, bool training) {
+BnPrelu bn2_input(const UpsGen& G, const float* P) {
+  return BnPrelu{G.bn_mean[1], G.bn_istd[1], P + G.gl.g2, P + G.gl.be2, P + G.gl.a3};
+}
+}
+
+int gen_forward(ConvLEnv& e, UpsGen& G, NetPair& p, const float* noise, int B, bool training, bool keep_h2) {
   fg_ctx* c = e.c;
   FG_REQUIRE(B >= 1 && B <= e.maxB, "G forward: batch %d out of range [1,%d]", B, e.maxB);
   FG_TRY(gen_pack(c, G, p));
@@ -143,11 +145,13 @@
   parts = training ? 1 : 0;
   FG_TRY(upsl_fwd(e, C2, G.h1, P, G.z2, B, &parts));
   FG_TRY(bn_stats(c, G, p, 1, G.z2, B, training, parts, G.t_bn2_finalize, G.t_bn2_stats));
-  {
-    ScopedTimer tm(c, G.t_bn2_apply);
+  G.c3_bn = convl_bn_input(c, G.GC3);
+  if (G.c3_bn) {
+    FG_TRY(convl_fwd(e, G.GC3, G.z2, P, G.z3, B, bn2_input(G, P), keep_h2 ? G.h2 : nullptr));
+  } else {
     FG_TRY(k_bn_prelu_apply(c, G.z2, G.bn_mean[1], G.bn_istd[1], P + L.g2, P + L.be2, P + L.a3, G.h2, (int64_t)B * S * S, 128));
-  }
-  FG_TRY(convl_fwd(e, G.GC3, G.h2, P, G.z3, B));
+    FG_TRY(convl_fwd(e, G.GC3, G.h2, P, G.z3, B));
+  }
   FG_TRY(k_sigmoid_fwd(c, G.z3, G.y, (int64_t)B * S * S * G.C));
   G.valid = true;
   return FG_OK;
@@ -165,7 +169,8 @@
   const int B = G.B, S = G.S, h = S / 2;
   FG_TRY(G.pairs.reset(c));
   FG_TRY(k_sigmoid_bwd(c, dy, G.y, G.dz3, (int64_t)B * S * S * G.C));
-  FG_TRY(convl_bwd(e, G.GC3, G.h2, G.dz3, g, G.dfull, B));
+  if (G.c3_bn) FG_TRY(convl_bwd(e, G.GC3, G.z2, G.dz3, g, G.dfull, B, bn2_input(G, P)));
+  else FG_TRY(convl_bwd(e, G.GC3, G.h2, G.dz3, g, G.dfull, B));
   {
     ScopedTimer tm(c, G.t_bn2_bwd_reduce);
     FG_TRY(k_bn_prelu_bwd_reduce(c, G.dfull, G.z2, G.bn_mean[1], G.bn_istd[1], P + L.g2, P + L.be2, P + L.a3, c->bn_acc,
diff --git a/face_generator_b200/csrc/k_bn_prelu.cuh b/face_generator_b200/csrc/k_bn_prelu.cuh
--- /dev/null
+++ b/face_generator_b200/csrc/k_bn_prelu.cuh
@@ -0,0 +1,9 @@
+#pragma once
+
+__device__ __forceinline__ float bn_affine(float z, float mean, float istd, float gamma, float beta) {
+  return gamma * ((z - mean) * istd) + beta;
+}
+__device__ __forceinline__ float prelu(float u, float a) { return u > 0.f ? u : a * u; }
+__device__ __forceinline__ float bn_prelu(float z, float mean, float istd, float gamma, float beta, float a) {
+  return prelu(bn_affine(z, mean, istd, gamma, beta), a);
+}
diff --git a/face_generator_b200/csrc/k_conv_edge.cu b/face_generator_b200/csrc/k_conv_edge.cu
--- a/face_generator_b200/csrc/k_conv_edge.cu
+++ b/face_generator_b200/csrc/k_conv_edge.cu
@@ -3,6 +3,7 @@
 #include <algorithm>
 
 #include "fg_internal.h"
+#include "k_bn_prelu.cuh"
 #include "k_conv_tc.h"
 
 namespace {
@@ -49,12 +50,12 @@
 template <int VEC>
 constexpr uint32_t red_tile_bytes() { return (kRedRows + 2) * (kW + 2) * 32 * VEC * 4; }
 
-template <int NS, int VEC>
+template <int NS, int VEC, bool BN>
 __global__ void __launch_bounds__(256, 1) conv_reduce_kernel(const __grid_constant__ CUtensorMap tmap, const float* __restrict__ Wp,
                                                              const float* __restrict__ bias, float* __restrict__ out, int H,
-                                                             int nunits) {
+                                                             int nunits, const BnPrelu xf, float* __restrict__ xout) {
   constexpr int C = 32 * VEC;
-  constexpr int PX = NS == 1 ? 16 : 4;
+  constexpr int PX = NS == 1 ? (BN ? 8 : 16) : 4;
   constexpr uint32_t kTile = red_tile_bytes<VEC>();
   extern __shared__ uint8_t smem_raw[];
   uint8_t* smem = reinterpret_cast<uint8_t*>((reinterpret_cast<uintptr_t>(smem_raw) + 127) & ~(uintptr_t)127);
@@ -81,6 +82,17 @@
     for (int n = 0; n < NS; ++n)
 #pragma unroll
       for (int j = 0; j < VEC; ++j) w[t][n][j] = Wp[(t * NS + n) * C + lane * VEC + j];
+  float bm[VEC], bs[VEC], bg[VEC], bb[VEC], ba = 0.f;
+#pragma unroll
+  for (int j = 0; j < VEC; ++j) bm[j] = bs[j] = bg[j] = bb[j] = 0.f;
+  if (BN) {
+#pragma unroll
+    for (int j = 0; j < VEC; ++j) {
+      const int ch = lane * VEC + j;
+      bm[j] = xf.mean[ch]; bs[j] = xf.istd[ch]; bg[j] = xf.gamma[ch]; bb[j] = xf.beta[ch];
+    }
+    ba = *xf.slope;
+  }
   float bv = 0.f;
   if (bias && (lane & 15) < PX * NS) bv = bias[(lane & 15) % NS];
   const int row = warp >> 1, xh = (warp & 1) * 16;
@@ -111,6 +123,16 @@
           } else {
             const float2 q = lds64(ad);
             v[dy][0] = q.x; v[dy][1 % VEC] = q.y;
+          }
+          if (BN) {
+            const bool pix = (unsigned)(y + dy - 1) < (unsigned)H && (unsigned)(x0 + j - 1) < (unsigned)kW;
+#pragma unroll
+            for (int k = 0; k < VEC; ++k) v[dy][k] = pix ? bn_prelu(v[dy][k], bm[k], bs[k], bg[k], bb[k], ba) : 0.f;
+            if (dy == 1 && j >= 1 && j <= PX && xout) {
+              float* hp = xout + ((size_t)(b * H + y) * kW + x0 + j - 1) * C + lane * VEC;
+              if (VEC == 4) *reinterpret_cast<float4*>(hp) = make_float4(v[1][0], v[1][1 % VEC], v[1][2 % VEC], v[1][3 % VEC]);
+              else *reinterpret_cast<float2*>(hp) = make_float2(v[1][0], v[1][1 % VEC]);
+            }
           }
         }
 #pragma unroll
@@ -230,19 +252,21 @@
   }
 }
 
-template <int NS, int VEC>
-int launch_reduce(fg_ctx* c, const float* in, const float* Wp, const float* bias, float* out, const ConvGeom& g) {
+template <int NS, int VEC, bool BN = false>
+int launch_reduce(fg_ctx* c, const float* in, const float* Wp, const float* bias, float* out, const ConvGeom& g,
+                  const BnPrelu& xf = {}, float* xout = nullptr) {
   CUtensorMap tmap;
   FG_TRY(tc_encode_nhwc_box(&tmap, in, 32 * VEC, g.W, g.H, g.B, 32 * VEC, kW + 2, kRedRows + 2, 1));
   const int nunits = g.B * (g.H / kRedRows);
   const size_t smem = 2 * (size_t)red_tile_bytes<VEC>() + 64 + 128;
   static bool attr_done = false;
   if (!attr_done) {
-    FG_CUDA(cudaFuncSetAttribute(conv_reduce_kernel<NS, VEC>, cudaFuncAttributeMaxDynamicSharedMemorySize, (int)smem));
+    FG_CUDA(cudaFuncSetAttribute(conv_reduce_kernel<NS, VEC, BN>, cudaFuncAttributeMaxDynamicSharedMemorySize, (int)smem));
     attr_done = true;
   }
   note_conv(c, FG_KERNEL_EDGE_REDUCE, NS, VEC, 0, 1);
-  conv_reduce_kernel<NS, VEC><<<std::min(nunits, c->sm_count), 256, smem, c->stream>>>(tmap, Wp, bias, out, g.H, nunits);
+  conv_reduce_kernel<NS, VEC, BN><<<std::min(nunits, c->sm_count), 256, smem, c->stream>>>(tmap, Wp, bias, out, g.H, nunits,
+                                                                                          xf, xout);
   LAUNCH_CHECK(c);
   return FG_OK;
 }
@@ -263,7 +287,14 @@
   return reduce || expand;
 }
 
-int k_conv_edge(fg_ctx* c, const float* in, const float* Wp, const float* bias, float* out, ConvGeom g) {
+int k_conv_edge(fg_ctx* c, const float* in, const float* Wp, const float* bias, float* out, ConvGeom g, const BnPrelu& xf,
+                float* xout) {
+  if (xf.mean) {
+    if (g.Cin == 128 && g.Cout == 3) return launch_reduce<3, 4, true>(c, in, Wp, bias, out, g, xf, xout);
+    if (g.Cin == 128 && g.Cout == 1) return launch_reduce<1, 4, true>(c, in, Wp, bias, out, g, xf, xout);
+    fg_set_error("k_conv_edge: BatchNorm input for %d -> %d", g.Cin, g.Cout);
+    return FG_ERR_UNSUPPORTED;
+  }
   if (g.Cout <= 3) {
     if (g.Cout == 3 && g.Cin == 128) return launch_reduce<3, 4>(c, in, Wp, bias, out, g);
     if (g.Cout == 3 && g.Cin == 64) return launch_reduce<3, 2>(c, in, Wp, bias, out, g);
diff --git a/face_generator_b200/csrc/k_conv_small.cu b/face_generator_b200/csrc/k_conv_small.cu
--- a/face_generator_b200/csrc/k_conv_small.cu
+++ b/face_generator_b200/csrc/k_conv_small.cu
@@ -1,4 +1,5 @@
 #include "fg_internal.h"
+#include "k_bn_prelu.cuh"
 
 namespace {
 constexpr int kMaxSmallW = 36 * 128;
@@ -109,14 +110,16 @@
   }
 }
 
-template <int CS, int XS>
+template <int CS, int XS, bool BN = false>
 __global__ void __launch_bounds__(128) wgrad_smallbig_kernel(const float* __restrict__ big, const float* __restrict__ small,
                                                              float* __restrict__ part, int B, int H, int W, int Cb,
-                                                             int rows_per_block) {
+                                                             int rows_per_block, const BnPrelu xf = {}) {
   __shared__ float4 sm[3][68];
   const int lanes = 128 / Cb;
   const int cb = threadIdx.x % Cb, pl = threadIdx.x / Cb;
   const int x_begin = pl * XS;
+  float bm = 0.f, bs = 0.f, bg = 0.f, bb = 0.f, ba = 0.f;
+  if (BN) bm = xf.mean[cb], bs = xf.istd[cb], bg = xf.gamma[cb], bb = xf.beta[cb], ba = *xf.slope;
   float acc[9][CS];
 #pragma unroll
   for (int t = 0; t < 9; ++t)
@@ -144,7 +147,7 @@
     const float* bp = big + ((size_t)r * W + x_begin) * Cb + cb;
     float bv[XS];
 #pragma unroll
-    for (int i = 0; i < XS; ++i) bv[i] = bp[(size_t)i * Cb];
+    for (int i = 0; i < XS; ++i) bv[i] = BN ? bn_prelu(bp[(size_t)i * Cb], bm, bs, bg, bb, ba) : bp[(size_t)i * Cb];
     float4 w0[3], w1[3], w2[3];
 #pragma unroll
     for (int rr = 0; rr < 3; ++rr) {
@@ -243,7 +246,7 @@
   return FG_OK;
 }
 
-int k_wgrad_small(fg_ctx* c, const float* in, const float* dY, float* dWp, ConvGeom g) {
+int k_wgrad_small(fg_ctx* c, const float* in, const float* dY, float* dWp, ConvGeom g, const BnPrelu& xf) {
   const bool small_out = g.Cout <= 4;
   const float* big = small_out ? in : dY;
   const float* small = small_out ? dY : in;
@@ -265,11 +268,20 @@
     else if (xs == 16) WG(CS_, 16); \
     else WG(CS_, 32);            \
   } while (0)
-  switch (Cs) {
-    case 1: WGX(1); break;
-    case 2: WGX(2); break;
-    case 3: WGX(3); break;
-    default: WGX(4); break;
+  if (xf.mean) {
+    if (!(small_out && Cb == 128 && xs == 32 && (Cs == 1 || Cs == 3))) {
+      fg_set_error("k_wgrad_small: BatchNorm input for %d -> %d at width %d", g.Cin, g.Cout, g.W);
+      return FG_ERR_UNSUPPORTED;
+    }
+    if (Cs == 3) wgrad_smallbig_kernel<3, 32, true><<<nblocks, 128, 0, c->stream>>>(big, small, c->small_ws, g.B, g.H, g.W, Cb, rpb, xf);
+    else wgrad_smallbig_kernel<1, 32, true><<<nblocks, 128, 0, c->stream>>>(big, small, c->small_ws, g.B, g.H, g.W, Cb, rpb, xf);
+  } else {
+    switch (Cs) {
+      case 1: WGX(1); break;
+      case 2: WGX(2); break;
+      case 3: WGX(3); break;
+      default: WGX(4); break;
+    }
   }
 #undef WGX
 #undef WG
diff --git a/face_generator_b200/csrc/k_elem.cu b/face_generator_b200/csrc/k_elem.cu
--- a/face_generator_b200/csrc/k_elem.cu
+++ b/face_generator_b200/csrc/k_elem.cu
@@ -2,6 +2,7 @@
 
 #include "convl.h"
 #include "fg_internal.h"
+#include "k_bn_prelu.cuh"
 #include "k_f16split.cuh"
 #include "k_ordered.cuh"
 
@@ -390,15 +391,15 @@
     const float4 g = make_float4(gamma[ch], gamma[ch + 1], gamma[ch + 2], gamma[ch + 3]);
     const float4 b = make_float4(beta[ch], beta[ch + 1], beta[ch + 2], beta[ch + 3]);
     float4 o;
-    o.x = g.x * ((v.x - m.x) * s.x) + b.x;
-    o.y = g.y * ((v.y - m.y) * s.y) + b.y;
-    o.z = g.z * ((v.z - m.z) * s.z) + b.z;
-    o.w = g.w * ((v.w - m.w) * s.w) + b.w;
+    o.x = bn_affine(v.x, m.x, s.x, g.x, b.x);
+    o.y = bn_affine(v.y, m.y, s.y, g.y, b.y);
+    o.z = bn_affine(v.z, m.z, s.z, g.z, b.z);
+    o.w = bn_affine(v.w, m.w, s.w, g.w, b.w);
     if (act) {
-      o.x = o.x > 0.f ? o.x : a * o.x;
-      o.y = o.y > 0.f ? o.y : a * o.y;
-      o.z = o.z > 0.f ? o.z : a * o.z;
-      o.w = o.w > 0.f ? o.w : a * o.w;
+      o.x = prelu(o.x, a);
+      o.y = prelu(o.y, a);
+      o.z = prelu(o.z, a);
+      o.w = prelu(o.w, a);
     }
     if (h) h4[i] = o;
     am = amax4(am, o.x, o.y, o.z, o.w);
@@ -423,8 +424,8 @@
   const float a = act ? *slope : 1.f;
   for (int64_t i = blockIdx.x * (int64_t)blockDim.x + threadIdx.x; i < n; i += (int64_t)gridDim.x * blockDim.x) {
     const int ch = (int)(i % C);
-    float o = gamma[ch] * ((z[i] - mean[ch]) * istd[ch]) + beta[ch];
-    if (act) o = o > 0.f ? o : a * o;
+    float o = bn_affine(z[i], mean[ch], istd[ch], gamma[ch], beta[ch]);
+    if (act) o = prelu(o, a);
     h[i] = o;
   }
 }
diff --git a/face_generator_b200/csrc/nets.cu b/face_generator_b200/csrc/nets.cu
--- a/face_generator_b200/csrc/nets.cu
+++ b/face_generator_b200/csrc/nets.cu
@@ -444,7 +444,7 @@
     const int b = std::min(chunk, N - s);
     const float* nd;
     FG_TRY(fg_to_dev(c, noise + (size_t)s * kNoiseDim, (size_t)b * kNoiseDim, n->z[0], &nd));
-    FG_TRY(gen_forward(n->env, n->G, n->net, nd, b, true));
+    FG_TRY(gen_forward(n->env, n->G, n->net, nd, b, true, false));
     float* dst = images_out + (size_t)s * img;
     if (out_dev) {
       FG_TRY(k_nhwc_to_nchw(c, n->G.y, dst, b, c->C, 1024));
diff --git a/face_generator_b200/csrc/ups_gan.cu b/face_generator_b200/csrc/ups_gan.cu
--- a/face_generator_b200/csrc/ups_gan.cu
+++ b/face_generator_b200/csrc/ups_gan.cu
@@ -10,7 +10,8 @@
         D(*n.D), real(real), noiseD(noiseD), noiseG(noiseG) {}
   int g_forward(int j, bool d_iter) override {
     const int rows = d_iter ? B / 2 : B;
-    return gen_forward(n.env, n.G, n.net, (d_iter ? noiseD : noiseG) + (size_t)j * rows * kNoiseDim, rows, true);
+    return gen_forward(n.env, n.G, n.net, (d_iter ? noiseD : noiseG) + (size_t)j * rows * kNoiseDim, rows, true,
+                       c->debug_keep);
   }
   int d_input(int j) override {
     const int Bh = B / 2, HW = n.G.S * n.G.S;
@@ -109,7 +110,7 @@
   const int HW = n.G.S * n.G.S;
   const float* nd;
   FG_TRY(fg_to_dev(c, noise, (size_t)B * kNoiseDim, n.z[0], &nd));
-  FG_TRY(gen_forward(n.env, n.G, n.net, nd, B, training));
+  FG_TRY(gen_forward(n.env, n.G, n.net, nd, B, training, true));
   if (images_out) {
     FG_TRY(k_nhwc_to_nchw(c, n.G.y, n.img[0], B, c->C, HW));
     FG_TRY(fg_to_user(c, images_out, n.img[0], (size_t)B * c->C * HW));
diff --git a/profiles/edge_fusion.py b/profiles/edge_fusion.py
--- /dev/null
+++ b/profiles/edge_fusion.py
@@ -0,0 +1,114 @@
+import argparse
+import json
+import os
+import subprocess
+import sys
+
+import numpy as np
+
+ROOT = os.path.join(os.path.dirname(os.path.abspath(__file__)), "..")
+sys.path.insert(0, ROOT)
+
+TIMERS = ["G.C3.fwd", "G.C3.wgrad", "G.C3.dgrad", "hbm.G.bn2.stats", "hbm.G.bn2.apply", "hbm.G.bn2.bwd_reduce",
+          "hbm.G.bn2.bwd_apply", "D.C1.fwd", "D.C1.wgrad", "D.C1.dgrad", "G.", "D."]
+
+
+def card():
+    q = "name,power.limit,clocks.sm,clocks.max.sm"
+    try:
+        out = subprocess.run(["nvidia-smi", "-i", "0", "--query-gpu=" + q, "--format=csv,noheader"], capture_output=True,
+                             text=True, timeout=30).stdout.strip()
+    except Exception as e:
+        out = "nvidia-smi unavailable: %s" % e
+    return out
+
+
+def synth_inputs(B, C, seed):
+    rng = np.random.default_rng(seed)
+    f = lambda a: np.ascontiguousarray(a, np.float32)
+    return (f(rng.random((B // 2, C, 32, 32))), f(rng.uniform(-1, 1, (B // 2, 100))), f(rng.uniform(-1, 1, (B, 100))))
+
+
+def one(args):
+    from face_generator_b200.lib import load_library
+    load_library(os.path.abspath(args.lib))
+    import face_generator_b200 as fg
+    from face_generator_b200 import layouts as LY
+    from face_generator_b200.lib import NET_D, NET_G
+    B, C = args.batch, 3
+    ctx = fg.Context(0, max_batch=B, channels=C)
+    rng = np.random.default_rng(1)
+    ctx.set_params(NET_G, LY.trained_like_init(LY.G_layout(C), rng))
+    ctx.set_params(NET_D, LY.trained_like_init(LY.D_layout(C), rng, 1.4))
+    hyper = fg.hyper_default()
+    real, nD, nG = (ctx.dev_array(a) for a in synth_inputs(B, C, 100))
+    seed = [0]
+
+    def step():
+        seed[0] += 1
+        ctx.train_step(hyper, B, real, nD, nG, None, None, seed[0], want_stats=False)
+
+    for _ in range(args.warmup):
+        step()
+    ctx.sync()
+    l0 = ctx.launches()
+    ctx.event_record(0)
+    for _ in range(args.steps):
+        step()
+    ctx.event_record(1)
+    ctx.sync()
+    ms = ctx.event_elapsed_ms(0, 1) / args.steps
+    launches = (ctx.launches() - l0) / args.steps
+    ctx.timing_enable(True)
+    nprof = 5
+    for _ in range(nprof):
+        step()
+    ctx.sync()
+    kern = {}
+    for name in TIMERS:
+        t, n = ctx.timing_get(name)
+        kern[name] = {"ms": round(t / nprof, 4), "launches": n // nprof}
+    ctx.timing_enable(False)
+    ctx.close()
+    print(json.dumps({"lib": args.lib, "ms_per_step": round(ms, 4), "images_per_s": round(B / (ms / 1e3), 1),
+                      "launches_per_step": launches, "kernels_ms_per_step": kern, "card": card()}))
+
+
+def compare(args):
+    res = {lib: [] for lib in args.libs}
+    print(json.dumps({"card_before": card()}))
+    for r in range(args.rounds):
+        for lib in args.libs:
+            cmd = [sys.executable, os.path.abspath(__file__), "one", "--lib", lib, "--steps", str(args.steps),
+                   "--warmup", str(args.warmup), "--batch", str(args.batch)]
+            out = subprocess.run(cmd, check=True, capture_output=True, text=True, cwd=ROOT).stdout
+            line = [ln for ln in out.splitlines() if ln.startswith("{")][-1]
+            print(line, flush=True)
+            res[lib].append(json.loads(line))
+    for lib, rows in res.items():
+        ms = [x["ms_per_step"] for x in rows]
+        ips = [x["images_per_s"] for x in rows]
+        kern = {k: round(float(np.median([x["kernels_ms_per_step"][k]["ms"] for x in rows])), 4) for k in TIMERS}
+        lau = {k: rows[0]["kernels_ms_per_step"][k]["launches"] for k in TIMERS}
+        print(json.dumps({"summary": lib, "ms_per_step": [min(ms), float(np.median(ms)), max(ms)],
+                          "images_per_s": [min(ips), float(np.median(ips)), max(ips)],
+                          "launches_per_step": rows[0]["launches_per_step"], "kernel_ms_median": kern,
+                          "kernel_launches_per_step": lau}))
+    print(json.dumps({"card_after": card()}))
+
+
+def main():
+    ap = argparse.ArgumentParser()
+    ap.add_argument("mode", choices=["one", "compare"])
+    ap.add_argument("--lib", default=os.path.join(ROOT, "face_generator_b200", "libfg_b200.so"))
+    ap.add_argument("--libs", nargs="+", default=[])
+    ap.add_argument("--rounds", type=int, default=5)
+    ap.add_argument("--steps", type=int, default=60)
+    ap.add_argument("--warmup", type=int, default=10)
+    ap.add_argument("--batch", type=int, default=256)
+    args = ap.parse_args()
+    (one if args.mode == "one" else compare)(args)
+
+
+if __name__ == "__main__":
+    main()
```

New measurement: 37510, median of 6. 1.01x the previous value.
